# sanazkaviani/3d-latent-diffusion-model

Hardware: AMD Instinct MI355X
Metric: UNet denoising steps/sec (bf16, 1x4x24x24x24 latent; whole job = sum over GPUs) (higher is better)
Workload: dtype bf16

## Files before the change

3d-latent-diffusion-model_amd/_lib.py:

```python
from __future__ import annotations

import ctypes as C
import os
import threading

LDM_MAX_LEVELS = 8
_HERE = os.path.dirname(os.path.abspath(__file__))
LIB_PATH = os.environ.get("LDM3D_LIB") or os.path.join(_HERE, "libldm3d.so")


class UNetCfg(C.Structure):
    _fields_ = [("spatial_dims", C.c_int), ("in_channels", C.c_int), ("out_channels", C.c_int),
                ("num_levels", C.c_int),
                ("channels", C.c_int * LDM_MAX_LEVELS), ("attention_levels", C.c_int * LDM_MAX_LEVELS),
                ("num_head_channels", C.c_int * LDM_MAX_LEVELS), ("num_res_blocks", C.c_int * LDM_MAX_LEVELS),
                ("norm_num_groups", C.c_int), ("norm_eps", C.c_float)]


class VaeCfg(C.Structure):
    _fields_ = [("spatial_dims", C.c_int), ("in_channels", C.c_int), ("out_channels", C.c_int),
                ("latent_channels", C.c_int), ("num_levels", C.c_int),
                ("channels", C.c_int * LDM_MAX_LEVELS), ("num_res_blocks", C.c_int * LDM_MAX_LEVELS),
                ("attention_levels", C.c_int * LDM_MAX_LEVELS),
                ("norm_num_groups", C.c_int), ("norm_eps", C.c_float),
# ... 36 lines not shown
    "ldm_adam_step_ema": (C.c_int, [_P, _P, _P, _P, _P, C.c_int64, C.c_float, C.c_float, C.c_float, C.c_float, C.c_float, C.c_int,
                                    C.c_float, C.c_int, _P, C.c_float, _P]),
    "ldm_model_adam_step_ema": (C.c_int, [_P, _P, _P, _P, _P, _P, C.c_float, C.c_float, C.c_float, C.c_float, C.c_float, C.c_int,
                                          C.c_float, C.c_int, _P, C.c_float, _P]),
    "ldm_model_set_graph_mode": (C.c_int, [_P, C.c_int]),
    "ldm_model_set_precision": (C.c_int, [_P, C.c_int]),
    "ldm_model_get_precision": (C.c_int, [_P]),
    "ldm_model_tap_count": (C.c_int, [_P, C.c_char_p, C.c_int, C.c_int, C.c_int, C.c_int]),
    "ldm_model_tap_elems": (C.c_int64, [_P, C.c_char_p, C.c_int, C.c_int, C.c_int, C.c_int]),
    "ldm_model_tap_info": (C.c_int, [_P, C.c_char_p, C.c_int, C.c_int, C.c_int, C.c_int, C.c_int, C.c_char_p, C.c_int,
                                     C.POINTER(C.c_int), C.POINTER(C.c_int64)]),
    "ldm_model_taps_workspace_bytes": (C.c_size_t, [_P, C.c_char_p, C.c_int, C.c_int, C.c_int, C.c_int, C.c_int]),
    "ldm_unet_forward_taps": (C.c_int, [_P, _P, C.c_int, _P, C.c_int, _P, _P, C.c_int, C.c_int, C.c_int, C.c_int, _P, _P,
                                        _P, C.c_size_t, _P]),
    "ldm_vae_encode_taps": (C.c_int, [_P, _P, _P, _P, _P, _P, C.c_int, C.c_int, C.c_int, C.c_int, _P, _P, _P, C.c_size_t, _P]),
    "ldm_vae_decode_taps": (C.c_int, [_P, _P, _P, C.c_int, C.c_int, C.c_int, C.c_int, _P, _P, _P, C.c_size_t, _P]),
    "ldm_vae_encode_workspace_bytes": (C.c_size_t, [_P, C.c_int, C.c_int, C.c_int, C.c_int]),
    "ldm_vae_decode_workspace_bytes": (C.c_size_t, [_P, C.c_int, C.c_int, C.c_int, C.c_int]),
    "ldm_vae_encode": (C.c_int, [_P, _P, _P, _P, _P, _P, C.c_int, C.c_int, C.c_int, C.c_int, _P, C.c_size_t, _P]),
    "ldm_vae_decode": (C.c_int, [_P, _P, _P, C.c_int, C.c_int, C.c_int, C.c_int, _P, C.c_size_t, _P]),
    "ldm_add_noise": (C.c_int, [_P, _P, _P, _P, _P, C.c_int, C.c_int64, _P]),
    "ldm_scheduler_step": (C.c_int, [_P, _P, _P, _P, _P, C.c_int64, C.c_int, C.c_int, _F, C.c_int, _P]),
    "ldm_add_noise_target": (C.c_int, [_P, _P, _P, _P, _P, _P, C.c_int, C.c_int64, C.c_int, _P]),
    "ldm_scale": (C.c_int, [_P, _P, C.c_int64, C.c_float, _P]),
    "ldm_sampler_create": (C.c_int, [_P, C.c_int, C.c_int, C.c_int, C.c_int, C.c_uint64, C.POINTER(_P)]),
    "ldm_sampler_create_pndm": (C.c_int, [_P, C.c_int, C.c_int, C.POINTER(_P)]),
    "ldm_sampler_state_bytes": (C.c_size_t, [_P, C.c_int64]),
    "ldm_sampler_bind_state": (C.c_int, [_P, _P, C.c_size_t, C.c_int64]),
    "ldm_pndm_step": (C.c_int, [_P] * 9 + [C.c_int64, C.c_int, _F, _P]),
    "ldm_sampler_destroy": (None, [_P]),
    "ldm_sampler_reset": (C.c_int, [_P, _P, C.c_int, _P]),
    "ldm_sampler_step": (C.c_int, [_P, _P, _P, _P, C.c_int64, _P, C.c_int, _P]),
    "ldm_sampler_noise": (C.c_int, [_P, C.c_int, _P, C.c_int64, _P]),
    "ldm_unet_denoise_step": (C.c_int, [_P, _P, _P, C.c_int, _P, C.c_int, _P, _P, C.c_int, C.c_int, C.c_int, C.c_int,
                                        _P, C.c_size_t, _P]),
    "ldm_window_grid_create": (C.c_int, [_P, _P, _P, _P, _P, _P, C.POINTER(_P)]),
    "ldm_window_grid_destroy": (None, [_P]),
    "ldm_window_gather": (C.c_int, [_P, _P, _P, C.c_int, _P]),
    "ldm_window_blend": (C.c_int, [_P, _P, _P, C.c_int, _P]),
    "ldm_unet_denoise_step_windows": (C.c_int, [_P, _P, _P, _P, C.c_int, _P, C.c_int, _P, _P, _P, C.c_int, _P, C.c_size_t, _P]),
    "ldm_op_conv3d": (C.c_int, [_P, C.c_int, _P, C.c_int, _P, _P, _P, C.c_int, _P, C.c_int, _P, _P, _P, C.c_int, _P, _P, _P,
                                C.c_int, C.c_int, C.c_int, C.c_int, C.c_int, C.c_int, C.c_int, C.c_int, C.c_int, C.c_int,
                                C.c_int, C.c_int, _P, C.c_size_t, _P]),
    "ldm_op_weight_flip_transpose": (C.c_int, [_P, _P, C.c_int, C.c_int, C.c_int, C.c_int, _P]),
    "ldm_op_conv3d_wgrad": (C.c_int, [_P, C.c_int, _P, C.c_int, _P, C.c_int, C.c_int, C.c_int, C.c_int, C.c_int, C.c_int,
                                      C.c_int, C.c_int, C.c_int, C.c_int, C.c_int, _P]),
    "ldm_op_group_norm_bwd_scratch_bytes": (C.c_size_t, [C.c_int, C.c_int, C.c_int, C.c_int]),
    "ldm_op_group_norm_bwd": (C.c_int, [_P, _P, C.c_int, _P, C.c_int, _P, _P, C.c_int, C.c_float, C.c_int, _P, _P, _P, _P, _P, _P,
                                        C.c_int, C.c_int, _P, C.c_size_t, _P]),
    "ldm_op_scale_intensity_percentiles_scratch_bytes": (C.c_size_t, [C.c_int]),
    "ldm_op_scale_intensity_percentiles": (C.c_int, [_P, _P, C.c_int, C.c_int64, C.c_float, C.c_float, C.c_float, C.c_float, _P, C.c_size_t, _P]),
    "ldm_op_image_metrics_scratch_bytes": (C.c_size_t, [C.c_int] * 6),
    "ldm_op_image_metrics": (C.c_int, [_P, C.POINTER(C.c_int64), _P, C.POINTER(C.c_int64)] + [C.c_int] * 5 + [_F, C.c_int, C.c_float, C.c_float,
                                       C.c_float, _P, _P, _P, C.c_size_t, _P]),
    "ldm_op_im2col": (C.c_int, [_P, _P] + [C.c_int] * 10 + [_P]),
    "ldm_op_col2im": (C.c_int, [_P, _P] + [C.c_int] * 10 + [_P]),
    "ldm_op_leaky_relu": (C.c_int, [_P, _P, C.c_int64, C.c_float, _P]),
    "ldm_op_leaky_relu_bwd": (C.c_int, [_P, _P, _P, C.c_int64, C.c_float, _P]),
    "ldm_op_pack_ncdhw": (C.c_int, [_P, _P, C.c_int, C.c_int, C.c_int, C.c_int64, _P]),
    "ldm_op_unpack_ndhwc": (C.c_int, [_P, _P, C.c_int, C.c_int, C.c_int, C.c_int64, _P]),
    "ldm_op_conv3d_gn_scratch_bytes": (C.c_size_t, [C.c_int, C.c_int, C.c_int, C.c_int, C.c_int, C.c_int]),
    "ldm_op_conv3d_gn": (C.c_int, [_P, C.c_int, _P, _P, _P, _P, C.c_int, C.c_float, C.c_int, _P, _P, C.c_int, C.c_int, C.c_int, C.c_int,
                                   C.c_int, C.c_int, C.c_int, C.c_int, _P, C.c_size_t, _P]),
    "ldm_op_conv3d_fin_gn_scratch_bytes": (C.c_size_t, [C.c_int, C.c_int, C.c_int, C.c_int, C.c_int, C.c_int]),
    "ldm_op_conv3d_fin_gn": (C.c_int, [_P, C.c_int, _P, _P, _P, C.c_int, _P, _P, _P, C.c_int, C.c_float, C.c_int, _P, _P,
                                       C.c_int, C.c_int, C.c_int, C.c_int, C.c_int, C.c_int, C.c_int, C.c_int, _P, C.c_size_t, _P]),
    "ldm_op_group_norm_scratch_bytes": (C.c_size_t, [C.c_int, C.c_int, C.c_int]),
    "ldm_op_group_norm": (C.c_int, [_P, C.c_int, _P, C.c_int, _P, _P, C.c_int, C.c_float, C.c_int, _P, C.c_int, C.c_int,
                                    _P, C.c_size_t, _P]),
    "ldm_op_attention": (C.c_int, [_P, _P, C.c_int, C.c_int, C.c_int, _P]),
    "ldm_op_attention_hd": (C.c_int, [_P, _P, _P, C.c_int, C.c_int, C.c_int, C.c_int, _P]),
    "ldm_op_attention_bwd_hd": (C.c_int, [_P, _P, _P, _P, _P, _P, C.c_int, C.c_int, C.c_int, C.c_int, _P]),
    "ldm_op_attention_train": (C.c_int, [_P, _P, _P, C.c_int, C.c_int, C.c_int, _P]),
    "ldm_op_attention_bwd": (C.c_int, [_P, _P, _P, _P, _P, _P, C.c_int, C.c_int, C.c_int, _P]),
    "ldm_profile_start": (C.c_int, [C.c_int, C.c_int, C.c_int, C.c_int]),
    "ldm_profile_detail": (C.c_int, [C.POINTER(C.c_double), C.POINTER(C.c_double), C.c_int]),
    "ldm_profile_stop": (C.c_int, [C.POINTER(C.c_double)]),
# ... 109 lines not shown
```

3d-latent-diffusion-model_amd/csrc/conv_thin.h:

```cpp
#pragma once
#include "common.h"

struct ThinParams {
    const bf16_t* x; const bf16_t* w;
    const float* bias; float* out;
    int N, D, H, W, Cin, CoutPad, CoutReal;
    int td, th, tw;
    int x3_c;
};

constexpr int THIN_TD = 4, THIN_TH = 4, THIN_TW = 16;
constexpr int THIN_HD = THIN_TD + 2, THIN_HH = THIN_TH + 2, THIN_HW = THIN_TW + 2;
constexpr int THIN_HV = THIN_HD * THIN_HH * THIN_HW;
constexpr int THIN_CK = 32, THIN_RB = THIN_CK * 2, THIN_NC = THIN_RB / 16;
constexpr int THIN_LDS_X = THIN_HV * THIN_RB, THIN_LDS_W = 27 * 4 * THIN_RB;
constexpr int THIN_LDS = THIN_LDS_X + THIN_LDS_W;

__global__ __launch_bounds__(256) void conv3_thin_kernel(const ThinParams p) {
#if defined(__HIP_DEVICE_COMPILE__)
    extern __shared__ __attribute__((aligned(16))) char smem[];
    char* sx = smem; char* sw = smem + THIN_LDS_X;
    const int tid = threadIdx.x, lane = tid & 63, wave = tid >> 6, fr = lane & 15, fg = lane >> 4;
    int b = blockIdx.x;
    const int bw = b % p.tw; b /= p.tw; const int bh = b % p.th; b /= p.th; const int bd = b % p.td; const int n = b / p.td;
    const int d0 = bd * THIN_TD, h0 = bh * THIN_TH, w0 = bw * THIN_TW;
    const size_t xn = (size_t)n * p.D * p.H * p.W;
    const int xstride = p.x3_c ? 2 * p.x3_c : p.Cin;
    const int wm = fr < 4 ? 2 * fr : fr < 12 ? 2 * (fr - 4) + 1 : 2 * (fr - 8);
    f32x4 acc[4];
#pragma unroll
    for (int t = 0; t < 4; ++t) acc[t] = (f32x4){0.f, 0.f, 0.f, 0.f};
    const u32x4 zero = {0u, 0u, 0u, 0u};
    for (int c0 = 0; c0 < p.Cin; c0 += THIN_CK) {
        __syncthreads();
        const int xc0 = (p.x3_c && c0 >= p.x3_c) ? c0 - p.x3_c : c0;
        constexpr int NIT = (THIN_HV * THIN_NC + 255) / 256;
        u32x4 hv_v[NIT];
#pragma unroll
        for (int k = 0; k < NIT; ++k) {
            const int e = tid + k * 256;
            const int hv = e / THIN_NC, c16 = e % THIN_NC;
            const int wx = hv % THIN_HW, r = hv / THIN_HW, hy = r % THIN_HH, dz = r / THIN_HH;
            const int gd = d0 - 1 + dz, gh = h0 - 1 + hy, gw = w0 - 1 + wx;
            hv_v[k] = zero;
            if (e < THIN_HV * THIN_NC && (unsigned)gd < (unsigned)p.D && (unsigned)gh < (unsigned)p.H && (unsigned)gw < (unsigned)p.W)
                hv_v[k] = *reinterpret_cast<const u32x4*>(p.x + (xn + ((size_t)gd * p.H + gh) * p.W + gw) * xstride + xc0 + c16 * 8);
        }
#pragma unroll
        for (int k = 0; k < NIT; ++k) {
            const int e = tid + k * 256;
            const int hv = e / THIN_NC, c16 = e % THIN_NC;
            if (e < THIN_HV * THIN_NC) *reinterpret_cast<u32x4*>(sx + hv * THIN_RB + ((c16 ^ ((hv >> 2) & (THIN_NC - 1))) << 4)) = hv_v[k];
        }
        for (int e = tid; e < 27 * 4 * THIN_NC; e += 256) {
            const int c16 = e % THIN_NC, row = (e / THIN_NC) & 3, tap = e / (4 * THIN_NC);
            u32x4 v = zero;
            if (row < p.CoutReal) v = *reinterpret_cast<const u32x4*>(p.w + ((size_t)tap * p.CoutPad + row) * p.Cin + c0 + c16 * 8);
            *reinterpret_cast<u32x4*>(sw + (tap * 4 + row) * THIN_RB + ((c16 ^ row) << 4)) = v;
        }
        __syncthreads();
#pragma unroll 1
        for (int tap = 0; tap < 27; ++tap) {
            const int kd = tap / 9, kh = (tap / 3) % 3, kw = tap % 3;
            u32x4 wv = zero;
            if (fr < 4) wv = *reinterpret_cast<const u32x4*>(sw + (tap * 4 + fr) * THIN_RB + ((fg ^ fr) << 4));
            const bf16x8 wf = *reinterpret_cast<const bf16x8*>(&wv);
#pragma unroll
            for (int t = 0; t < 4; ++t) {
                const int hv = ((wave + kd) * THIN_HH + (t + kh)) * THIN_HW + wm + kw;
                const bf16x8 xf = *reinterpret_cast<const bf16x8*>(sx + hv * THIN_RB + ((fg ^ ((hv >> 2) & (THIN_NC - 1))) << 4));
                acc[t] = __builtin_amdgcn_mfma_f32_16x16x32_bf16(wf, xf, acc[t], 0, 0, 0);
            }
        }
    }
    if (fg != 0) return;
    const int gd = d0 + wave, gw = w0 + wm;
    if (gd >= p.D || gw >= p.W) return;
    const size_t dhw = (size_t)p.D * p.H * p.W;
#pragma unroll
    for (int t = 0; t < 4; ++t) {
        const int gh = h0 + t;
        if (gh >= p.H) continue;
        const size_t sp = ((size_t)gd * p.H + gh) * p.W + gw;
#pragma unroll
        for (int r = 0; r < 4; ++r)
            if (r < p.CoutReal) p.out[((size_t)n * p.CoutReal + r) * dhw + sp] = acc[t][r] + (p.bias ? p.bias[r] : 0.f);
    }
#endif
}
```

3d-latent-diffusion-model_amd/csrc/gemm_wg.h:

```cpp
#pragma once
#include "conv_cube.h"
#include "gemm_light.h"

struct WgGnParams {
    const float* slabs;
    const float* gamma; const float* beta;
    int nrb, groups, DHW; float eps;
};

__device__ __forceinline__ void wg_copies_landed_barrier() {
    asm volatile("s_waitcnt vmcnt(0)" ::: "memory");
    __builtin_amdgcn_s_barrier();
    asm volatile("" ::: "memory");
}

template <int MT, int NWV, bool GN>
__global__ __launch_bounds__(64 * NWV) void gemm_wg_kernel(const LightParams p, const int cout_pad, const WgGnParams g) {
#if defined(__HIP_DEVICE_COMPILE__)
    extern __shared__ __attribute__((aligned(16))) char smem[];
    typedef __attribute__((address_space(3))) void* lds_ptr_t;
    constexpr int NT = 2, R = 16 * MT, NW = 32 * NWV;
    const int tid = threadIdx.x, lane = tid & 63, fr = lane & 15, fg = lane >> 4;
    const int wave = __builtin_amdgcn_readfirstlane(tid >> 6);
    const int mtile = blockIdx.x % p.mtiles, ntile = blockIdx.x / p.mtiles;
    const int m0 = mtile * R, n0 = ntile * NW;
    const int nkb = p.K >> 7;
    const unsigned row2 = (unsigned)p.K * 2u;
    const int xbase = nkb * NW * 256;

    constexpr int T = 64 * NWV;
    const int C = p.K;
    int ns0 = 0, ns1 = 0;
    float4 t[16]; float gm[4], bt[4];
    float* const ab = reinterpret_cast<float*>(smem + nkb * (NW + R) * 256);
    double* const csum = reinterpret_cast<double*>(ab + 4 * C);
    float* const gstat = reinterpret_cast<float*>(csum + 2 * C);
    auto slab_loads = [&](const int smp, const int pp) {
        const float* base = g.slabs + ((size_t)smp * g.nrb * C + 2 * pp) * 2;
#pragma unroll
        for (int k = 0; k < 16; ++k) {
            int bb = k; const bool ok = bb < g.nrb; if (!ok) bb = g.nrb - 1;
            t[k] = *reinterpret_cast<const float4*>(base + (size_t)bb * C * 2);
            if (!ok) t[k] = make_float4(0.f, 0.f, 0.f, 0.f);
        }
    };
    if constexpr (GN) {
        ns0 = m0 / g.DHW;
        int ml = m0 + R - 1; if (ml > p.M - 1) ml = p.M - 1;
        ns1 = ml / g.DHW;
        if (tid < (C >> 1)) slab_loads(ns0, tid);
#pragma unroll
        for (int j = 0; j < 4; ++j) {
            const int c = tid + j * T;
            gm[j] = c < C ? g.gamma[c] : 0.f; bt[j] = c < C ? g.beta[c] : 0.f;
        }
    }

    {
        __amdgpu_buffer_rsrc_t rs_w = __builtin_amdgcn_make_buffer_rsrc((void*)p.w, 0, (int)((unsigned)cout_pad * row2), 0x00020000);
        for (int u = wave; u < nkb * (NW / 4); u += NWV) {
            const int kb = u / (NW / 4), lr = 4 * (u % (NW / 4)) + (lane >> 4), f = lr & 15;
            const int co = n0 + (lr & ~31) + 8 * (f >> 2) + 4 * ((lr >> 4) & 1) + (f & 3);
            const unsigned vo = (unsigned)co * row2 + (unsigned)kb * 256u + (unsigned)((lane & 15) ^ f) * 16u;
            __builtin_amdgcn_raw_ptr_buffer_load_lds(rs_w, (lds_ptr_t)(smem + u * 1024), 16, vo, 0, 0, 0);
        }
        __amdgpu_buffer_rsrc_t rs_x = __builtin_amdgcn_make_buffer_rsrc((void*)p.x, 0, (int)((unsigned)p.M * row2), 0x00020000);
        for (int u = wave; u < nkb * (R / 4); u += NWV) {
            const int kb = u / (R / 4), lr = 4 * (u % (R / 4)) + (lane >> 4);
            const unsigned vo = (unsigned)(m0 + lr) * row2 + (unsigned)kb * 256u + (unsigned)((lane & 15) ^ (lr & 15)) * 16u;
            __builtin_amdgcn_raw_ptr_buffer_load_lds(rs_x, (lds_ptr_t)(smem + xbase + u * 1024), 16, vo, 0, 0, 0);
        }
    }
    const int n0w = n0 + 32 * wave;
    const int wrow = (32 * wave + fr) * 256, xrow = xbase + fr * 256;
    f32x4 acc[NT][MT];
#pragma unroll
    for (int a = 0; a < NT; ++a)
#pragma unroll
        for (int b = 0; b < MT; ++b) acc[a][b] = (f32x4){0.f, 0.f, 0.f, 0.f};
    if constexpr (GN) {
        const int cpg = C / g.groups;
        for (int smp = ns0; smp <= ns1; ++smp) {
            for (int pp = tid; pp < (C >> 1); pp += T) {
                if (smp != ns0 || pp != tid) slab_loads(smp, pp);
                double s0 = 0.0, q0 = 0.0, s1 = 0.0, q1 = 0.0;
#pragma unroll
                for (int k = 0; k < 8; ++k) {
                    float4 a = make_float4(0.f, 0.f, 0.f, 0.f);
                    a.x += t[k].x; a.y += t[k].y; a.z += t[k].z; a.w += t[k].w;
                    a.x += t[k + 8].x; a.y += t[k + 8].y; a.z += t[k + 8].z; a.w += t[k + 8].w;
                    s0 += (double)a.x; q0 += (double)a.y; s1 += (double)a.z; q1 += (double)a.w;
                }
                csum[4 * pp] = s0; csum[4 * pp + 1] = q0; csum[4 * pp + 2] = s1; csum[4 * pp + 3] = q1;
            }
            cube_barrier();
            if (tid < g.groups) {
                double s = 0.0, q = 0.0;
                for (int k = 0; k < cpg; ++k) { s += csum[(tid * cpg + k) * 2]; q += csum[(tid * cpg + k) * 2 + 1]; }
                const double cnt = (double)cpg * (double)g.DHW;
                const double mean = s / cnt;
                double var = q / cnt - mean * mean; if (var < 0.0) var = 0.0;
                const float rstd = (float)(1.0 / sqrt(var + (double)g.eps));
                gstat[2 * tid] = (float)mean; gstat[2 * tid + 1] = rstd;
            }
// ... 47 lines not shown
        _Pragma("unroll") for (int mt = 0; mt < MT; ++mt) XF[mt] = *reinterpret_cast<const bf16x8*>(xp_ + mt * 4096); \
    } while (0)
#define GW_MFMA(WF, XF) do {                                                                          \
        _Pragma("unroll") for (int nt = 0; nt < NT; ++nt)                                             \
            _Pragma("unroll") for (int mt = 0; mt < MT; ++mt)                                         \
                acc[nt][mt] = __builtin_amdgcn_mfma_f32_16x16x32_bf16(WF[nt], XF[mt], acc[nt][mt], 0, 0, 0); \
    } while (0)
    GW_LOAD(wa, xa, 0);
    for (int s = 0; s < nsteps; s += 2) {
        GW_LOAD(wb, xb, s + 1);
        GW_MFMA(wa, xa);
        GW_LOAD(wa, xa, s + 2);
        GW_MFMA(wb, xb);
    }
#undef GW_LOAD
#undef GW_MFMA
    light_epilogue<MT, NT>(p, acc, mtile, m0, n0w, fr, fg);
#endif
}

static inline bool gemm_wg_ok(bool single_source, int K, long M) {
    return ldm_knob("LDM_GEMM_WG", 1) != 0 && single_source && K % 128 == 0 && K >= 128 && K <= 512 && M * (long)K * 2 < (1L << 31);
}
static inline int gemm_wg_gn_lds(int K, int groups) { return 32 * K + 8 * groups; }
static inline int gemm_wg_rows(int big) { return big ? 64 : 32; }
static inline int gemm_wg_couts(int big, int K) { return big && K <= 384 ? 128 : 64; }
static inline bool gemm_wg_gn_shape_ok(int K, long DHW, int groups, int nrb, int big) {
    return K >= 256 && groups >= 1 && groups <= 128 && K % groups == 0 && (K / groups) % 2 == 0 && K / groups <= 64 && nrb >= 1 && nrb <= 16 &&
           DHW >= gemm_wg_rows(big) && (gemm_wg_rows(big) + gemm_wg_couts(big, K)) * 2 * K + gemm_wg_gn_lds(K, groups) <= 160 * 1024;
}
static inline bool gemm_wg_gn_ok(int K, long DHW, int groups, int nrb, int big) {
    return ldm_knob("LDM_GEMM_WG_GN", 0) != 0 && gemm_wg_gn_shape_ok(K, DHW, groups, nrb, big);
}
template <int MT, int NWV, bool GN>
static inline hipError_t launch_gemm_wg_t(const LightParams& p, int cout_pad, const WgGnParams& g, hipStream_t s) {
    constexpr int kmax = (16 * MT + 32 * NWV) * 2 * 512 <= 160 * 1024 ? 512 : 384;
    const int lds = (16 * MT + 32 * NWV) * 2 * p.K + (GN ? gemm_wg_gn_lds(p.K, g.groups) : 0);
    if (p.K > kmax || lds > 160 * 1024) return hipErrorInvalidValue;
    static bool attr_tab[32] = {}; bool& attr_set = attr_flag(attr_tab);
    if (!attr_set) {
        hipError_t e = hipFuncSetAttribute(reinterpret_cast<const void*>(&gemm_wg_kernel<MT, NWV, GN>), hipFuncAttributeMaxDynamicSharedMemorySize,
                                           GN ? 160 * 1024 : (16 * MT + 32 * NWV) * 2 * kmax);
        if (e != hipSuccess) return e;
        attr_set = true;
    }
    hipLaunchKernelGGL((gemm_wg_kernel<MT, NWV, GN>), dim3(p.mtiles * ((cout_pad + 32 * NWV - 1) / (32 * NWV))), dim3(64 * NWV), lds, s, p, cout_pad, g);
    return hipGetLastError();
}
static inline hipError_t launch_gemm_wg(const LightParams& p0, int cout_pad, int big, hipStream_t s, const WgGnParams* gn = nullptr) {
    LightParams p = p0;
    const WgGnParams g = gn ? *gn : WgGnParams{};
    if (big) {
        p.mtiles = (p.M + 63) / 64;
        if (p.K <= 384) return gn ? launch_gemm_wg_t<4, 4, true>(p, cout_pad, g, s) : launch_gemm_wg_t<4, 4, false>(p, cout_pad, g, s);
        return gn ? launch_gemm_wg_t<4, 2, true>(p, cout_pad, g, s) : launch_gemm_wg_t<4, 2, false>(p, cout_pad, g, s);
    }
    p.mtiles = (p.M + 31) / 32;
    return gn ? launch_gemm_wg_t<2, 2, true>(p, cout_pad, g, s) : launch_gemm_wg_t<2, 2, false>(p, cout_pad, g, s);
}
static inline hipError_t launch_gemm_1x1(const LightParams& p, int cout_pad, int big, int wg, hipStream_t s) {
    return wg ? launch_gemm_wg(p, cout_pad, big, s) : launch_gemm_light(p, cout_pad, big, s);
}
```

3d-latent-diffusion-model_amd/csrc/ldm3d.hip:

```cpp
#include <hip/hip_runtime.h>
#include <dlfcn.h>
#include <math.h>
#include <stdarg.h>
#include <stdio.h>
#include <stdlib.h>
#include <string.h>

#include <algorithm>
#include <atomic>
#include <map>
#include <memory>
#include <string>
#include <type_traits>
#include <vector>

#include "../../include/ldm3d.h"
#include "attention.h"
#include "conv_igemm.h"
#include "conv_halo.h"
#include "conv_cube.h"
#include "conv_plane.h"
#ifdef LDM_EXPERIMENTS
#include "conv_halo_pp.h"
#include "conv_halo_rw.h"
// ... 99 lines not shown
struct Ref { int base = BASE_NULL; size_t off = 0; };
static inline Ref ws_ref(size_t off) { Ref r; r.base = BASE_WS; r.off = off; return r; }
static inline Ref w_ref(size_t off) { Ref r; r.base = BASE_W; r.off = off; return r; }
static inline Ref io_ref(int i) { Ref r; r.base = BASE_IO0 + i; r.off = 0; return r; }
static inline Ref w32_ref(size_t off) { Ref r; r.base = BASE_W32; r.off = 2 * off; return r; }

struct Act {
    size_t off = 0; int C = 0; int N = 0, D = 0, H = 0, W = 0; bool valid = false;
    size_t stats_off = 0; bool has_stats = false;
    int stats_nrb = 0;
    int esz = 2;
    bool hl = false;
    size_t cs_off = 0; int cs_rows = 0;
    size_t bytes() const { return (size_t)N * D * H * W * C * esz; }
    long rows() const { return (long)N * D * H * W; }
};

enum OpKind { OP_PACK, OP_CONV, OP_FINALIZE, OP_GN_STATS, OP_GN_FINALIZE, OP_GN_PREP, OP_GN_APPLY, OP_ATTN, OP_SINUSOID,
              OP_GEMV, OP_VAE_HEADS, OP_GN_FUSED,
              OP_WT , OP_WT_BATCH, OP_WGRAD, OP_EXPORT , OP_EXPORT_BATCH, OP_COLSUM, OP_GNB, OP_ATTN_BWD, OP_ADD, OP_SUMPOOL, OP_LIN_DX, OP_LIN_DW, OP_VAE_HEADS_BWD,
              OP_GEMM_LIGHT,
              OP_COLSUM_BATCH,
              OP_IM2COL,
              OP_PACK32, OP_CONV32, OP_FIN32, OP_GN_STATS32, OP_GN_APPLY32, OP_ATTN32, OP_GEMV32,
              OP_TAP,
              OP_BUCKET, OP_BUCKET_JOIN,
              OP_UPS_SPLIT32,
              OP_CONV_THIN,
              OP_FIN_GN,
              OP_GEMM_LIGHT32,
              OP_CONV_BLOCK,
              OP_TEMB_ROW };

struct ConvCfg { int wgm, wgn, bk, splitk; int halo = 0, mtps = 0, qps = 0; int slab_lg = 0; int cube = 0; int th = 0, big = 0; int plane = 0; int wg = 0; };

struct ConvRec {
    Ref xa, xb, w; int ca, cb;
    Ref x1a, x1b, w1; int c1a, c1b;
    int N, Din, Hin, Win, Dout, Hout, Wout;
    int k, stride, pad, M;
    int couts, cout_pad, cout_real;
    int nchunk0, nchunk1, mtiles, ntiles;
    bool ups, exact;
    bool phase;
    bool x3;
    bool ep32_ndhwc, ep32_ncdhw;
    Ref bias, bias2, temb, residual; int temb_stride;
    Ref out; int f32_out;
    Ref partial, stats;
    int stats_nrb, stats_rows;
    Ref gamma, beta, gn_out; int gn_groups, gn_silu, gn_lg; float gn_eps;
    Ref gn_stats; int gn_nrb;
};

struct GnRec {
    Ref xa, xb; int ca, cb, N, DHW;
    Ref gamma, beta; int groups; float eps; bool silu;
    Ref stats_a, stats_b; int nrb_a, nrb_b;
    Ref partial; int nslab, rows_per_slab;
    Ref ab, mr;
    Ref out; bool out_hl;
    int rows_per_block, chunks;
    Ref dy, gsum, dgamma_n, dbeta_n;
    Ref cs; bool leaves_colsums;
    Ref acc_a, acc_b, dxa, dxb;
    int dgamma_flat, dbeta_flat;
    bool fp32;
// ... 12 lines not shown
struct LayoutRec {
    Ref a, b, dst;
    int N, c_real, c_stored, D, H, W, DHW;
    bool internal;
    int esz, mode, ups;
};

struct AttnRec {
    Ref qkv, out, lse;
    Ref d_o, delta, dqkv;
    int B, N, C, heads, d; float scale;
    bool x3, fp32;
};

struct LinRec {
    Ref w, bias, x, y;
    Ref dy, x_pre, dx, dW, db, part;
    int B, I, O, x_stride, y_stride, dy_stride;
    int silu, nz; bool fp32;
};

struct ElemRec {
    Ref a, b, out; int n;
    Ref ml, noise, mu, sigma, z;
    Ref dz, g_mu, g_sigma, dy; int c_dz;
    int N, D, H, W, C, L, DHW;
    bool fp32;
};

struct RangeRec { int first, end, count; bool fp32; };

struct Op {
    OpKind kind;
    ConvCfg cc;
    ConvRec cv;
    GnRec gn;
    WgradRec wg;
    LayoutRec lay;
    AttnRec at;
    LinRec lin;
    ElemRec el;
    RangeRec rg;
};

struct Pool {
    struct Blk { size_t off, size; };
    std::vector<Blk> free_list;
    std::map<size_t, size_t> live;
    size_t top = 0, high = 0;
    size_t alloc(size_t bytes) {
        bytes = rup_sz(bytes, 256);
        for (size_t k = 0; k < free_list.size(); ++k)
            if (free_list[k].size >= bytes) {
                size_t off = free_list[k].off;
                if (free_list[k].size == bytes) free_list.erase(free_list.begin() + k);
                else { free_list[k].off += bytes; free_list[k].size -= bytes; }
                live[off] = bytes;
                return off;
            }
        size_t off = top; top += bytes; high = std::max(high, top); live[off] = bytes;
        return off;
    }
    void release(size_t off) {
        auto it = live.find(off); if (it == live.end()) return;
        Blk b{off, it->second}; live.erase(it);
        free_list.push_back(b);
// ... 6 lines not shown
            top = free_list.back().off; free_list.pop_back();
        }
    }
};

struct DevTable {
    void* descs = nullptr; int2* map = nullptr; int nblocks = 0;
    std::vector<char> h_descs, h_map;
    ~DevTable() { if (descs) (void)hipFree(descs); if (map) (void)hipFree(map); }
    template <class D> int upload(const std::vector<D>& d, const std::vector<int2>& m) {
        if (d.empty()) return 0;
        h_descs.assign((const char*)d.data(), (const char*)(d.data() + d.size()));
        h_map.assign((const char*)m.data(), (const char*)(m.data() + m.size()));
        nblocks = (int)m.size();
        return 0;
    }
    int ready() {
        if (descs || h_descs.empty()) return 0;
        if (hipMalloc(&descs, h_descs.size()) != hipSuccess || hipMalloc((void**)&map, h_map.size()) != hipSuccess) return -1;
        if (hipMemcpy(descs, h_descs.data(), h_descs.size(), hipMemcpyHostToDevice) != hipSuccess) return -1;
        if (hipMemcpy(map, h_map.data(), h_map.size(), hipMemcpyHostToDevice) != hipSuccess) return -1;
        return 0;
    }
};

struct TapInfo { std::string name; int dims[5]; size_t off; };

struct Plan {
    std::vector<Op> ops;
    std::vector<TapInfo> taps; size_t tap_elems = 0;
    size_t ws_bytes = 0;
    size_t bwd_begin = 0;
    bool train = false;
    mutable DevTable wt_tab, exp_tab, cs_tab;
};

enum PackKind { PK_CONV_W, PK_VEC_F32, PK_LINEAR_W };
struct ParamDesc {
    std::string name; std::vector<int64_t> shape;
    PackKind kind; size_t dst_off;
    int k = 1, cout = 0, cin = 0, cout_pad = 0, cin_s = 0, row_off = 0;
    int64_t flat_off = 0;
    bool loaded = false;
};

struct ConvW { size_t w_off = 0; size_t b_off = 0; int cout = 0, cout_pad = 0, cin_s = 0, k = 1; bool has = false;
               size_t wp_off = 0;
               size_t x3_off = (size_t)-1;
               size_t x3p_off = (size_t)-1; };
struct GnW { size_t g_off = 0, b_off = 0; int C = 0; };
struct LinW { size_t w_off = 0, b_off = 0; int in = 0, out = 0; };

struct ldm_comm;
struct GradSyncState {
    ldm_comm* comm = nullptr; hipStream_t stream = nullptr;
    std::vector<hipEvent_t> ev;
    size_t used = 0; std::vector<int64_t> elems;
    int wire = 0;
    void* stage = nullptr; size_t stage_bytes = 0;
    int pending = 0;
};
static int grad_sync_begin(GradSyncState& g, hipStream_t s);
static int grad_sync_bucket(GradSyncState& g, float* buf, int64_t count, hipStream_t s);
static int grad_sync_join(GradSyncState& g, hipStream_t s);
struct ldm_model {
    int type = 0;
// ... 141 lines not shown
    int tap_mode = 0;
    void tap(const std::string& name, Act& h, int c_real) {
        if (!tap_mode) return;
        TapInfo t; t.name = name; t.dims[0] = h.N; t.dims[1] = c_real; t.dims[2] = h.D; t.dims[3] = h.H; t.dims[4] = h.W; t.off = plan->tap_elems;
        plan->tap_elems += (size_t)h.N * c_real * h.D * h.H * h.W;
        Op o{}; o.kind = OP_TAP; LayoutRec& l = o.lay; l.a = ws_ref(h.off);
        l.dst.base = BASE_TAPO; l.dst.off = t.off * 4; l.b.base = BASE_TAPI; l.b.off = t.off * 4;
        l.N = h.N; l.c_real = c_real; l.c_stored = h.C; l.DHW = h.D * h.H * h.W; l.esz = h.esz; l.mode = tap_mode;
        plan->ops.push_back(o);
        plan->taps.push_back(t);
        if (tap_mode == 2 && h.has_stats) { pool.release(h.stats_off); h.has_stats = false; }
    }
    void pack(Ref src_a, Ref src_b, const Act& dst, int c_real, bool internal) {
        Op o{}; o.kind = hp ? OP_PACK32 : OP_PACK; LayoutRec& l = o.lay; l.a = src_a; l.b = src_b; l.dst = ws_ref(dst.off);
        l.N = dst.N; l.c_real = c_real; l.c_stored = dst.C; l.DHW = dst.D * dst.H * dst.W; l.internal = internal;
        plan->ops.push_back(o);
    }
    void free_act(Act& a) {
        if (train) return;
        if (a.valid) { pool.release(a.off); if (a.has_stats) pool.release(a.stats_off); }
        a.valid = false; a.has_stats = false;
    }
    bool train = false, recording = false;

    struct ConvArgs {
        Act xa, xb;
        const ConvW* w = nullptr;
        int k = 3, stride = 1, pad = 1, ups = 0;
        int Do = 0, Ho = 0, Wo = 0;
        Act g1a, g1b; const ConvW* w1 = nullptr;
        Ref temb; int temb_stride = 0;
        Act residual;
        bool f32_out = false; Ref out_ref; int cout_real = 0;
        bool want_stats = true;
        Ref w_over; bool no_bias = false; int exact = 0;
        int temb_row = -1;
        int f32_tag = 0;
        const GnW* pre_gn = nullptr; int pre_groups = 0, pre_nrb = 0; float pre_eps = 0.f;
    };
    struct Tape {
        int kind = 0;
        ConvArgs c; Act out; bool leaf_input = false;
        const GnW* g = nullptr; Act xa, xb; size_t ab_off = 0, mr_off = 0; int groups = 0; bool silu = false;
        Act qkv, o; size_t lse_off = 0; int head_ch = 64;
    };
    std::vector<Tape> tape;

    static bool halo_enabled() { return ldm_knob("LDM_CONV_HALO", 1) != 0; }
    static int tall_mode() { return ldm_xknob("LDM_HALO_TALL", 2); }
    static bool light_enabled() { return ldm_knob("LDM_GEMM_LIGHT", 1) != 0; }
    static bool two_wg_enabled() { return ldm_knob("LDM_IGEMM_2WG", 1) != 0; }
    static bool phase_enabled() { return ldm_knob("LDM_CONV_PHASE", 1) != 0; }
    static bool halo_skip_enabled() { static const int v = ldm_knob("LDM_HALO_SKIP", 1); return v != 0; }
    static bool halo_skip_split_enabled() { static const int v = ldm_knob("LDM_HALO_SKIP_SPLIT", 1); return v != 0; }
    static bool cube_enabled() { return ldm_knob("LDM_CONV_CUBE", 1) != 0; }
    static bool cube_ok(int D, int H, int W, int cin0, int c1a, int c1b, int cout_pad) {
        return cube_enabled() && D >= 1 && H >= 1 && W >= 1 && D <= CUBE_EDGE && H <= CUBE_EDGE && W <= CUBE_EDGE && cin0 % 64 == 0 && cin0 >= 128 &&
               c1a % 64 == 0 && c1b % 64 == 0 && cout_pad % 16 == 0;
    }
    static ConvCfg cube_cfg(int cin0) { ConvCfg c{2, 2, 64, cin0 / 64}; c.cube = 1; return c; }
    static bool plane_enabled() { return ldm_knob("LDM_CONV_PLANE", 1) != 0; }
    static int plane_max_cin() { return (int)ldm_knob("LDM_CONV_PLANE_MAX_CIN", 256); }
    static bool plane_ok(int D, int H, int W, int cin0, int c1a, int c1b, int cout_pad) {
        return plane_enabled() && D >= 1 && H >= 1 && W >= 1 && D <= PLANE_EDGE && H <= PLANE_EDGE && W <= PLANE_EDGE &&
               (D > CUBE_EDGE || H > CUBE_EDGE || W > CUBE_EDGE) && cin0 % 64 == 0 && cin0 >= 128 && cin0 <= plane_max_cin() &&
               c1a % 64 == 0 && c1b % 64 == 0 && cout_pad % 16 == 0;
// ... 47 lines not shown
            for (int sk : splits) {
                if (sk > 1 && Q / sk < 3) break;
                const int qps = (Q + sk - 1) / sk, skr = (Q + qps - 1) / qps;
                const long nwg = tiles * skr;
                const double rounds = ceil((double)nwg / 256.0);
                double t = rounds * (3.0 * qps * c_step + 2500.0 + ((steps1 + skr - 1) / skr) * 1.6 * c_step + (steps1 && skr > 1 ? 800.0 : 0.0));
                if (skr > 1) t += 6000.0 + (double)M * cout_pad * 4.0 * skr * 2.0 / 2500.0;
                if (steps1 && skr > 1 && !halo_skip_split_enabled()) continue;
                if (tall_mode() == 2 && cout_pad % 128 == 0) t = 1e31;
                if (tall_mode() == 3 && skr == 1 && best.halo == 1 && best.splitk == 1) t = 0.0;
                if (t < best_t) { best_t = t; best = ConvCfg{4, 1, 64, skr}; best.halo = 2; best.mtps = mtps; best.qps = qps; }
            }
        }
        return best;
    }

    static ConvRec conv_rec(const ConvArgs& a, int k, int stride, int pad, long M, int cout_real) {
        ConvRec c{}; c.N = a.xa.N; c.Din = a.xa.D; c.Hin = a.xa.H; c.Win = a.xa.W; c.Dout = a.Do; c.Hout = a.Ho; c.Wout = a.Wo;
        c.k = k; c.stride = stride; c.pad = pad; c.M = (int)M; c.couts = rup(a.w->cout, 32); c.cout_pad = a.w->cout_pad; c.cout_real = cout_real;
        return c;
    }
    static void conv_epilogue(ConvRec& c, const ConvArgs& a, const Act& out) {
        c.bias = a.no_bias ? Ref() : w_ref(a.w->b_off); c.temb = a.temb; c.temb_stride = a.temb_stride;
        c.residual = a.residual.valid ? ws_ref(a.residual.off) : Ref();
        c.out = a.f32_out ? a.out_ref : ws_ref(out.off); c.f32_out = a.f32_out ? 1 : 0;
    }
    static void conv_sources(ConvRec& c, const ConvArgs& a) {
        c.xa = ws_ref(a.xa.off); c.xb = a.xb.valid ? ws_ref(a.xb.off) : Ref(); c.ca = a.xa.C; c.cb = a.xb.valid ? a.xb.C : 0;
    }
    void record_conv(const ConvArgs& a, const Act& out) { if (recording) { Tape t; t.kind = 0; t.c = a; t.out = out; tape.push_back(t); } }
    static long thin_tiles(const ConvArgs& a) {
        return (long)a.xa.N * ((a.Do + THIN_TD - 1) / THIN_TD) * ((a.Ho + THIN_TH - 1) / THIN_TH) * ((a.Wo + THIN_TW - 1) / THIN_TW);
    }
    void emit_thin(const ConvArgs& a, long M, Ref w, int cout_real, bool x3) {
        Op op{}; op.kind = OP_CONV_THIN;
        ConvRec& c = op.cv; c = conv_rec(a, 3, 1, 1, M, cout_real); conv_epilogue(c, a, Act());
        c.xa = ws_ref(a.xa.off); c.ca = x3 ? 2 * a.xa.C : a.xa.C; c.x3 = x3; c.w = w;
        plan->ops.push_back(op);
    }
    Act emit_light(OpKind kind, const ConvArgs& a, long M, Ref w, int big, bool want_stats) {
        const int N = a.xa.N, rows = big ? 64 : 32;
        Op op{}; op.kind = kind; op.cc.big = big;
        ConvRec& c = op.cv; c = conv_rec(a, a.k, a.stride, a.pad, M, a.w->cout);
        op.cc.wg = kind == OP_GEMM_LIGHT && gemm_wg_ok(!a.xb.valid, a.xa.C + (a.xb.valid ? a.xb.C : 0), M);
        if (a.pre_gn) {
            op.cc.wg = 2; c.gamma = w_ref(a.pre_gn->g_off); c.beta = w_ref(a.pre_gn->b_off); c.gn_groups = a.pre_groups; c.gn_eps = a.pre_eps;
            c.gn_stats = ws_ref(a.xa.stats_off); c.gn_nrb = a.pre_nrb;
        }
        Act out = new_act(N, a.Do, a.Ho, a.Wo, c.couts);
        const long dhwo = (long)a.Do * a.Ho * a.Wo;
        if (want_stats && (N == 1 || dhwo % rows == 0)) {
            out.stats_off = pool.alloc((size_t)((M + rows - 1) / rows) * c.couts * 2 * 4); out.has_stats = true;
            out.stats_nrb = (int)(N == 1 ? (M + rows - 1) / rows : dhwo / rows);
        }
        conv_epilogue(c, a, out); conv_sources(c, a); c.w = w; c.stats = out.has_stats ? ws_ref(out.stats_off) : Ref();
        plan->ops.push_back(op);
        record_conv(a, out);
        return out;
    }
    Act emit_conv_block(const ConvArgs& a, long M, int th, int tiles) {
        const int N = a.xa.N;
        Op op{}; op.kind = OP_CONV_BLOCK; op.cc.th = th;
        ConvRec& c = op.cv; c = conv_rec(a, 3, 1, 1, M, a.w->cout);
        Act out = new_act(N, a.Do, a.Ho, a.Wo, c.couts);
        if (a.want_stats) { out.stats_off = pool.alloc((size_t)N * tiles * c.couts * 2 * 4); out.has_stats = true; out.stats_nrb = tiles; }
        conv_epilogue(c, a, out); conv_sources(c, a);
        c.w = a.w_over.base != BASE_NULL ? a.w_over : w_ref(a.w->w_off); c.stats = out.has_stats ? ws_ref(out.stats_off) : Ref();
        plan->ops.push_back(op);
        record_conv(a, out);
        return out;
// ... 136 lines not shown
        if (sk > 1) { partial_bytes = std::max(partial_bytes, (size_t)sk * M * w.cout_pad * 4); partial_fixups.push_back(plan->ops.size()); }
        plan->ops.push_back(op);
        if (sk > 1) { Op f = op; f.kind = OP_FIN32; fin32_stats(f, out, a, N, a.Do * a.Ho * a.Wo, couts); partial_fixups.push_back(plan->ops.size()); plan->ops.push_back(f); }
        record_conv(a, out);
        return out;
    }

    Act conv(const ConvArgs& a, std::string tag = "") {
        if (hp) return conv32(a, tag);
        const ConvW& w = *a.w;
        const int cin0 = a.xa.C + (a.xb.valid ? a.xb.C : 0);
        int bk = 64;
        if (a.xa.C % 64 || (a.xb.valid && a.xb.C % 64)) bk = 32;
        int cin1 = 0;
        if (a.w1) {
            cin1 = a.g1a.C + (a.g1b.valid ? a.g1b.C : 0);
            if (a.g1a.C % 64 || (a.g1b.valid && a.g1b.C % 64)) bk = 32;
        }
        if (cin0 != w.cin_s || (a.w1 && cin1 != a.w1->cin_s) || cin0 % 32 || cin1 % 32) {
            err = "conv " + tag + ": channel bookkeeping mismatch"; return Act();
        }
        const int N = a.xa.N;
        const long M = (long)N * a.Do * a.Ho * a.Wo;
        {
            const long rows0 = (long)N * a.xa.D * a.xa.H * a.xa.W;
            const long big = std::max(std::max(rows0 * a.xa.C, a.xb.valid ? rows0 * a.xb.C : 0L),
                                      a.w1 ? std::max(M * a.g1a.C, a.g1b.valid ? M * a.g1b.C : 0L) : 0L) * 2;
            if (big >= (1L << 32)) { err = "conv " + tag + ": a source tensor exceeds 4 GiB (split the batch)"; return Act(); }
        }
        {
            static const int thin = ldm_knob("LDM_CONV_THIN", 1);
            static const long thin_min = ldm_knob("LDM_CONV_THIN_MIN", 512L);
            const int cr = a.cout_real ? a.cout_real : w.cout;
            if (thin && a.f32_out && a.k == 3 && a.stride == 1 && a.pad == 1 && !a.ups && !a.exact && !a.xb.valid && !a.w1 &&
                a.temb.base == BASE_NULL && !a.residual.valid && a.w_over.base == BASE_NULL && cr <= 4 && cin0 % 32 == 0 && cin0 <= 128 &&
                a.xa.D == a.Do && a.xa.H == a.Ho && a.xa.W == a.Wo &&
                thin_tiles(a) >= thin_min) {
                emit_thin(a, M, w_ref(w.w_off), cr, false);
                record_conv(a, Act());
                return Act();
            }
        }
        const bool phase = a.ups == 1 && !a.exact && a.k == 3 && a.stride == 1 && a.pad == 1 && !train && !a.xb.valid && !a.w1 &&
                           a.w_over.base == BASE_NULL && w.wp_off != 0 && phase_enabled() &&
                           a.Do == 2 * a.xa.D && a.Ho == 2 * a.xa.H && a.Wo == 2 * a.xa.W;
        if (gemm_light_ok(a.k, a.stride, a.ups, cin0, !a.w1, !a.f32_out && a.temb.base == BASE_NULL) && light_enabled() &&
            a.xa.D == a.Do && a.xa.H == a.Ho && a.xa.W == a.Wo && M * (long)cin0 * 2 < (1L << 31))
            return emit_light(OP_GEMM_LIGHT, a, M, a.w_over.base != BASE_NULL ? a.w_over : w_ref(w.w_off), gemm_light_big(M, w.cout_pad), a.want_stats);
        if (a.pre_gn) { err = "conv " + tag + ": a GroupNorm prologue needs the light GEMM"; return Act(); }
        if (conv_block_enabled() && a.k == 3 && a.stride == 1 && a.pad == 1 && a.ups == 0 && !a.exact && !a.xb.valid && !a.w1 && !a.f32_out &&
            w.cout_pad == 64 && rup(w.cout, 32) == 64 && cin0 <= conv_block_max_cin() &&
            a.xa.D == a.Do && a.xa.H == a.Ho && a.xa.W == a.Wo) {
            const int TH = conv_block_th();
            const int td = (a.Do + BLK_TD - 1) / BLK_TD, th = (a.Ho + TH - 1) / TH, tw = (a.Wo + BLK_TW - 1) / BLK_TW;
            static const long min_blocks = ldm_knob("LDM_CONV_BLOCK_MIN", 512L);
            if ((long)N * td * th * tw >= min_blocks) return emit_conv_block(a, M, TH, td * th * tw);
        }
        if (conv_block128_enabled() && a.k == 3 && a.stride == 1 && a.pad == 1 && a.ups == 0 && !a.exact && !a.xb.valid && !a.w1 && !a.f32_out &&
            w.cout_pad == 128 && rup(w.cout, 32) == 128 && cin0 <= conv_block128_max_cin() && a.xa.D == a.Do && a.xa.H == a.Ho && a.xa.W == a.Wo) {
            const int td = (a.Do + BLK_TD - 1) / BLK_TD, th = (a.Ho + 7) / 8, tw = (a.Wo + BLK_TW - 1) / BLK_TW;
            static const long min_blocks = ldm_knob("LDM_CONV_BLOCK128_MIN", 192L);
            static const long max_blocks = ldm_xknob("LDM_CONV_BLOCK128_MAX", 0L);
            const long tiles128 = (long)N * td * th * tw;
            if (tiles128 >= min_blocks && tiles128 <= (max_blocks > 0 ? max_blocks : (long)device_cus())) return emit_conv_block(a, M, 8, td * th * tw);
        }
        const int taps = phase ? 8 : a.k * a.k * a.k;
        const bool halo_ok = a.k == 3 && a.stride == 1 && a.pad == 1 && a.ups == 0 && !a.exact && !a.xb.valid && (!a.w1 || (halo_skip_enabled() && bk == 64)) &&
                             a.xa.D == a.Do && a.xa.H == a.Ho && a.xa.W == a.Wo;
        int nchunk0 = cin0 / bk, nchunk1 = cin1 / bk;
        int steps0 = taps * nchunk0, steps1 = nchunk1;
// ... 133 lines not shown
            return out;
        }
        if (fused) push_ab(OP_GN_PREP, rec);
        else {
            const int rows_par = std::max(1, 256 / (C / 8));
            static const bool gn32_fold = (ldm_knob("LDM_GN32_FOLD", 1) != 0);
            const bool fold32 = hp && !train && gn32_fold && C / groups <= 64;
            int nslab = std::min((DHW + rows_par - 1) / rows_par, std::max(1, (fold32 ? 256 : 512) / N));
            int rps = (DHW + nslab - 1) / nslab;
            nslab = (DHW + rps - 1) / rps;
            gnpart_bytes = std::max(gnpart_bytes, (size_t)N * nslab * C * 2 * 4);
            rec.nslab = nslab; rec.rows_per_slab = rps;
            gnpart_fixups.push_back(plan->ops.size()); push(hp ? OP_GN_STATS32 : OP_GN_STATS, rec);
            gnpart_fixups.push_back(plan->ops.size());
            if (fold32) { Act out = fold_apply32(); push(OP_GN_APPLY32, rec); return out; }
            push_ab(OP_GN_FINALIZE, rec);
        }
        Act out = new_act(N, xa.D, xa.H, xa.W, C);
        GnRec ap = gn_rec(xa, xb); ap.silu = silu; ap.ab = rec.ab; ap.out = ws_ref(out.off);
        push_ab(hp ? OP_GN_APPLY32 : OP_GN_APPLY, ap);
        record(out);
        return out;
    }

    static bool im2col_enabled() { return ldm_knob("LDM_CONV_IM2COL", 1) != 0; }
    Act conv_in_im2col(const std::string& name, Ref r0, Ref r1, int N, int D, int H, int W, int cin, bool internal) {
        auto it = m->convs.find(name + ".im2col");
        if (train || hp || it == m->convs.end() || !im2col_enabled() || !light_enabled()) return Act();
        const ConvW& wi = it->second;
        Act pm = new_act(N, D, H, W, wi.cin_s);
        Op o{}; o.kind = OP_IM2COL; LayoutRec& l = o.lay; l.a = r0; l.b = r1; l.dst = ws_ref(pm.off);
        l.N = N; l.c_real = cin; l.c_stored = wi.cin_s; l.D = D; l.H = H; l.W = W; l.internal = internal;
        plan->ops.push_back(o);
        ConvArgs a; a.xa = pm; a.w = &wi; a.k = 1; a.pad = 0; a.Do = D; a.Ho = H; a.Wo = W;
        Act out = conv(a, name + ".im2col");
        free_act(pm);
        return out;
    }

    Act conv3(const std::string& name, const Act& x, int stride = 1, int pad = 1, int ups = 0) {
        ConvArgs a; a.xa = x; a.w = &m->convs.at(name); a.k = 3; a.stride = stride; a.pad = pad; a.ups = ups;
        const int Du = x.D << ups, Hu = x.H << ups, Wu = x.W << ups;
        if (stride == 1) { a.Do = Du; a.Ho = Hu; a.Wo = Wu; }
        else if (pad == 1) { a.Do = (Du + 2 - 3) / 2 + 1; a.Ho = (Hu + 2 - 3) / 2 + 1; a.Wo = (Wu + 2 - 3) / 2 + 1; }
        else { a.Do = (Du + 1 - 3) / 2 + 1; a.Ho = (Hu + 1 - 3) / 2 + 1; a.Wo = (Wu + 1 - 3) / 2 + 1; }
        return conv(a, name);
    }

    Act resblock(const std::string& p, const Act& xa, const Act& xb, int cout, int groups, float eps,
                 const std::string& skip_name, bool with_temb, const GnW* next_gn = nullptr) {
        const int cin = xa.C + (xb.valid ? xb.C : 0);
        Act sk;
        if (cin != cout && hp) {
            ConvArgs cs; cs.xa = xa; cs.xb = xb; cs.w = &m->convs.at(p + skip_name); cs.k = 1; cs.pad = 0;
            cs.Do = xa.D; cs.Ho = xa.H; cs.Wo = xa.W; cs.want_stats = false;
            sk = conv(cs, p + skip_name);
            if (!sk.valid) return Act();
        }
        Act h0 = gn_apply(m->gns.at(p + ".norm1"), xa, xb, groups, eps, true, &m->convs.at(p + ".conv1"));
        if (!h0.valid) return Act();
        ConvArgs c1; c1.xa = h0; c1.w = &m->convs.at(p + ".conv1"); c1.Do = xa.D; c1.Ho = xa.H; c1.Wo = xa.W;
        if (with_temb) {
            c1.temb = ws_ref(temb_all_off + (size_t)m->tproj_row.at(p) * 4); c1.temb_stride = tproj_stride;
            c1.temb_row = m->tproj_row.at(p);
        }
        Act h1 = conv(c1, p + ".conv1");
        free_act(h0);
        if (!h1.valid) return Act();
        Act h2;
// ... 389 lines not shown
        const int lvl = L - 1 - i;
        int prev = oc; oc = ch[lvl];
        const int ic = ch[std::max(lvl - 1, 0)];
        const int nres = c.num_res_blocks[lvl] + 1;
        for (int j = 0; j < nres; ++j) {
            const int skip_c = (j == nres - 1) ? ic : oc;
            const int rin = (j == 0) ? prev : oc;
            char p[96]; snprintf(p, sizeof p, "up_blocks.%d.resnets.%d", i, j);
            reg_res(p, rin + skip_c, oc);
            if (c.attention_levels[lvl] && !collect) { snprintf(p, sizeof p, "up_blocks.%d.attentions.%d", i, j); m->reg_attn(p, oc); }
        }
        if (i != L - 1 && !collect) { char p[96]; snprintf(p, sizeof p, "up_blocks.%d.upsampler.postconv", i); m->reg_conv(p, oc, oc, oc, 3, true); }
    }
    if (!collect) { m->reg_gn("out.0", ch[0]); m->reg_conv("out.2", ch[0], ch[0], c.out_channels, 3); }
    };
    walk();
    m->reg_linear("time_embed.0", ch[0], temb);
    m->reg_linear("time_embed.2", temb, temb);
    int rows = 0; for (auto& t : tprojs) rows += t.second;
    m->tproj_rows = rows;
    m->tproj_w_off = m->arena_alloc((size_t)rows * temb * 2);
    m->tproj_b_off = m->arena_alloc((size_t)rows * 4);
    int r = 0;
    for (auto& t : tprojs) {
        m->tproj_row[t.first] = r;
        m->reg_linear_at(t.first + ".time_emb_proj", temb, t.second, m->tproj_w_off + (size_t)r * temb * 2, m->tproj_b_off + (size_t)r * 4);
        r += t.second;
    }
    collect = false;
    walk();
    return 0;
}

static int unet_build(ldm_model* m, int B, int D, int H, int W, Plan* plan, bool train, bool hp = false, int tap_mode = 0, bool temb_table = false) {
    const ldm_unet_cfg& c = m->ucfg;
    const int L = c.num_levels; const int* ch = c.channels;
    const int temb = ch[0] * 4, G = c.norm_num_groups; const float eps = c.norm_eps;
    if (train && tap_mode) return fail(LDM_ERR_UNSUPPORTED, "debug taps are inference-only");
    Builder b; b.m = m; b.plan = plan; b.train = train; b.recording = train; b.hp = hp; b.tap_mode = tap_mode;
    const size_t sin_off = b.pool.alloc((size_t)B * ch[0] * 4);
    const size_t e1_off = b.pool.alloc((size_t)B * temb * 4);
    const size_t e2_off = b.pool.alloc((size_t)B * temb * 4);
    b.tproj_stride = m->tproj_rows;
    b.temb_all_off = b.pool.alloc(((size_t)B * m->tproj_rows + 256) * 4);
    const LinW& l0 = m->lins.at("time_embed.0"); const LinW& l2 = m->lins.at("time_embed.2");
    if (temb_table && !train) {
        Op o{}; o.kind = OP_TEMB_ROW; o.lin.y = ws_ref(b.temb_all_off); o.lin.O = m->tproj_rows; o.lin.B = B; plan->ops.push_back(o);
    } else {
    { Op o{}; o.kind = OP_SINUSOID; o.lin.x = io_ref(2); o.lin.y = ws_ref(sin_off); o.lin.B = B; o.lin.O = ch[0];
      plan->ops.push_back(o); }
    auto gemv = [&](size_t w_off, size_t b_off, size_t x_off, size_t y_off, int I, int O, int xs, int ys, int silu) {
        Op o{}; o.kind = hp ? OP_GEMV32 : OP_GEMV; LinRec& l = o.lin;
        l.w = hp ? w32_ref(w_off) : w_ref(w_off); l.bias = w_ref(b_off); l.x = ws_ref(x_off); l.y = ws_ref(y_off);
        l.I = I; l.O = O; l.x_stride = xs; l.y_stride = ys; l.silu = silu; l.B = B; plan->ops.push_back(o);
    };
    gemv(l0.w_off, l0.b_off, sin_off, e1_off, ch[0], temb, ch[0], temb, 0);
    gemv(l2.w_off, l2.b_off, e1_off, e2_off, temb, temb, temb, temb, 1);
    gemv(m->tproj_w_off, m->tproj_b_off, e2_off, b.temb_all_off, temb, m->tproj_rows, temb, m->tproj_rows, 1);
    }

    const int cin_s = rup(c.in_channels, 32);
    Act h = b.conv_in_im2col("conv_in", io_ref(0), io_ref(1), B, D, H, W, c.in_channels, false);
    if (!h.valid) {
        if (!b.err.empty()) return fail(LDM_ERR_UNSUPPORTED, "%s", b.err.c_str());
        Act xin = b.new_act(B, D, H, W, cin_s);
        b.pack(io_ref(0), io_ref(1), xin, c.in_channels, false);
        h = b.conv3("conv_in", xin);
// ... 47 lines not shown
    for (int i = 0; i < L; ++i) {
        const int lvl = L - 1 - i;
        for (int j = 0; j < c.num_res_blocks[lvl] + 1; ++j) {
            Act s = skips.back(); skips.pop_back();
            snprintf(p, sizeof p, "up_blocks.%d.resnets.%d", i, j);
            char pa[96]; snprintf(pa, sizeof pa, "up_blocks.%d.attentions.%d.norm", i, j);
            Act hn = b.resblock(p, h, s, ch[lvl], G, eps, ".skip_connection", true, c.attention_levels[lvl] ? &m->gns.at(pa) : nullptr);
            b.free_act(h); b.free_act(s);
            if (!hn.valid) return fail(LDM_ERR_UNSUPPORTED, "%s", b.err.c_str());
            b.tap(p, hn, ch[lvl]);
            if (c.attention_levels[lvl]) {
                snprintf(p, sizeof p, "up_blocks.%d.attentions.%d", i, j);
                Act ha = b.attention(p, hn, c.num_head_channels[lvl], G, eps);
                b.free_act(hn);
                if (!ha.valid) return fail(LDM_ERR_UNSUPPORTED, "%s", b.err.c_str());
                hn = ha;
                b.tap(p, hn, ch[lvl]);
            }
            h = hn;
        }
        if (i != L - 1) {
            snprintf(p, sizeof p, "up_blocks.%d.upsampler.postconv", i);
            Act hu = b.conv3(p, h, 1, 1, 1);
            b.free_act(h);
            if (!hu.valid) return fail(LDM_ERR_UNSUPPORTED, "%s", b.err.c_str());
            b.tap(p, hu, ch[lvl]);
            h = hu;
        }
    }
    Act hn = b.gn_apply(m->gns.at("out.0"), h, Act(), G, eps, true, &m->convs.at("out.2"));
    b.free_act(h);
    if (!hn.valid) return fail(LDM_ERR_UNSUPPORTED, "%s", b.err.c_str());
    Builder::ConvArgs oa; oa.xa = hn; oa.w = &m->convs.at("out.2"); oa.Do = D; oa.Ho = H; oa.Wo = W;
    oa.f32_out = true; oa.out_ref = io_ref(3); oa.cout_real = c.out_channels;
    b.conv(oa, "out.2");
    if (!b.err.empty()) return fail(LDM_ERR_UNSUPPORTED, "%s", b.err.c_str());
    if (train) {
        plan->train = true; plan->bwd_begin = plan->ops.size();
        b.recording = false;
        const int rows = m->tproj_rows;
        b.dtemb_off = b.pool.alloc(((size_t)B * rows + 256) * 4);
        { Op o{}; o.kind = OP_WT_BATCH; o.rg.fp32 = hp; plan->ops.push_back(o); }
        const int cos_ = rup(c.out_channels, 32);
        Act dout = b.new_act(B, D, H, W, cos_);
        b.pack(io_ref(0), Ref(), dout, c.out_channels, false);
        b.bucket_hi = b.done_from = m->flat_total;
        b.tail_reserved = m->params[m->pindex.at("conv_in.conv.weight")].flat_off;
        if (!b.backward_all(dout)) return fail(LDM_ERR_UNSUPPORTED, "%s", b.err.c_str());
        b.flush_colsums();
        const Ref dtemb = ws_ref(b.dtemb_off);
        b.dw_off = b.pool.alloc((size_t)rows * temb * 4); b.vec_off = b.pool.alloc((size_t)rows * 4);
        b.emit_lin_dw(dtemb, ws_ref(e2_off), ws_ref(b.dw_off), ws_ref(b.vec_off), B, temb, rows, rows, temb, 1);
        for (const ParamDesc& d : m->params) {
            if (d.kind == PK_LINEAR_W && d.dst_off >= m->tproj_w_off && d.dst_off < m->tproj_w_off + (size_t)rows * temb * 2)
                b.emit_export(b.dw_off, 1, rows, temb, (int)((d.dst_off - m->tproj_w_off) / ((size_t)temb * 2)), 0, d.cout, d.cin, d.flat_off);
            if (d.kind == PK_VEC_F32 && d.dst_off >= m->tproj_b_off && d.dst_off < m->tproj_b_off + (size_t)rows * 4)
                b.emit_export(b.vec_off, 1, 1, 0, 0, (int)((d.dst_off - m->tproj_b_off) / 4), 1, d.cout, d.flat_off);
        }
        const size_t de2 = b.pool.alloc((size_t)B * temb * 4), de1 = b.pool.alloc((size_t)B * temb * 4);
        b.emit_lin_dx(hp ? w32_ref(m->tproj_w_off) : w_ref(m->tproj_w_off), dtemb, ws_ref(e2_off), ws_ref(de2), B, temb, rows, rows, temb, 1);
        auto P = [&](const char* n) { return m->params[m->pindex.at(n)].flat_off; };
        b.emit_lin_dw(ws_ref(de2), ws_ref(e1_off), Builder::grad_ref(P("time_embed.2.weight")), Builder::grad_ref(P("time_embed.2.bias")),
                      B, temb, temb, temb, temb, 1);
        b.emit_lin_dx(hp ? w32_ref(l2.w_off) : w_ref(l2.w_off), ws_ref(de2), ws_ref(e1_off), ws_ref(de1), B, temb, temb, temb, temb, 1);
        b.emit_lin_dw(ws_ref(de1), ws_ref(sin_off), Builder::grad_ref(P("time_embed.0.weight")), Builder::grad_ref(P("time_embed.0.bias")),
                      B, ch[0], temb, temb, ch[0], 0);
        if (!b.err.empty()) return fail(LDM_ERR_UNSUPPORTED, "%s", b.err.c_str());
// ... 611 lines not shown
    p.CoutS = c.couts; p.CoutPad = c.cout_pad; p.CoutReal = c.cout_real; p.nchunk = c.nchunk0; p.steps = c.k * c.k * c.k * c.nchunk0;
    p.splitk = o.cc.splitk; p.steps_per_split = (p.steps + p.splitk - 1) / p.splitk; p.mtiles = c.mtiles; p.ntiles = c.ntiles;
    p.bias = (const float*)rp(bs, c.bias); p.temb = (const float*)rp(bs, c.temb); p.temb_stride = c.temb_stride; p.residual = (const float*)rp(bs, c.residual);
    if (c.f32_out) p.out_ncdhw = (float*)rp(bs, c.out); else p.out = (float*)rp(bs, c.out);
    p.partial = (float*)rp(bs, c.partial);
    if (c.stats_nrb > 0) { p.stats = (float*)rp(bs, c.stats); p.stats_nrb = c.stats_nrb; p.stats_rows = c.stats_rows; }
    return p;
}
static FinalizeParams finalize_params(const ConvParams& p) {
    FinalizeParams f{}; f.partial = p.partial; f.splitk = p.splitk; f.M = p.M; f.CoutPad = p.CoutPad; f.CoutS = p.CoutS; f.CoutReal = p.CoutReal;
    f.DHWo = p.Dout * p.Hout * p.Wout; f.bias = p.bias; f.bias2 = p.bias2; f.temb = p.temb; f.temb_stride = p.temb_stride; f.residual = p.residual;
    f.out = p.out; f.out_f32 = p.out_f32; f.stats = p.stats;
    return f;
}
template <class P> static P wgrad_params(const WgradRec& w, const Bases& bs) {
    P p{}; p.dy = (decltype(p.dy))rp(bs, w.dy); p.cdy = w.cdy; p.x = (decltype(p.x))rp(bs, w.x); p.cx = w.cx;
    p.dw = (float*)rp(bs, w.dw); p.Cout = w.Cout; p.Cin = w.Cin; p.dw_ld = w.dw_ld; p.dw_ci_off = w.dw_ci_off;
    p.N = w.N; p.Din = w.Din; p.Hin = w.Hin; p.Win = w.Win; p.Dout = w.Dout; p.Hout = w.Hout; p.Wout = w.Wout;
    p.ksize = w.ksize; p.stride = w.stride; p.pad = w.pad; p.ups = w.ups; p.M = w.M;
    p.co_tiles = (p.Cout + 127) / 128; p.ci_tiles = (p.Cin + 127) / 128; p.ksplit = w.ksplit;
    p.slab_stride = (long)w.ksize * w.ksize * w.ksize * w.rows_total * w.dw_ld;
    return p;
}
template <class P> static P attn_params(const AttnRec& a, const Bases& bs) {
    P p{}; p.qkv = (decltype(p.qkv))rp(bs, a.qkv); p.out = (decltype(p.out))rp(bs, a.out); p.lse = (float*)rp(bs, a.lse);
    p.B = a.B; p.N = a.N; p.C = a.C; p.heads = a.heads; p.d = a.d; p.scale = a.scale;
    return p;
}
template <class P> static P attn_bwd_params(const AttnRec& a, const Bases& bs) {
    P p{}; p.qkv = (decltype(p.qkv))rp(bs, a.qkv); p.o = (decltype(p.o))rp(bs, a.out); p.d_o = (decltype(p.d_o))rp(bs, a.d_o);
    p.lse = (const float*)rp(bs, a.lse); p.delta = (float*)rp(bs, a.delta); p.dqkv = (decltype(p.dqkv))rp(bs, a.dqkv);
    p.B = a.B; p.N = a.N; p.C = a.C; p.d = a.d; p.heads = a.heads; p.scale = a.scale;
    return p;
}

struct PlanTrace { bool on = false; std::string path; PlanTrace() { const char* e = getenv("LDM_PLAN_TRACE"); if (e && *e) { on = true; path = e; } } };
static PlanTrace g_plan_trace;
struct LaneCtx { GradSyncState* sync = nullptr; };

static int run_plan(const Plan& plan, const Bases& bs, const int* rt, hipStream_t s, size_t begin = 0, size_t end = (size_t)-1,
                    LaneCtx lanes = LaneCtx()) {
    if (end > plan.ops.size()) end = plan.ops.size();
    const char* trace_path = g_plan_trace.on ? g_plan_trace.path.c_str() : nullptr;
    std::vector<hipEvent_t> tev;
    if (trace_path) { tev.resize(end - begin + 1); for (auto& e : tev) HIP_TRY(hipEventCreate(&e)); }
    struct TraceDone {
        const Plan& plan; size_t begin, end; std::vector<hipEvent_t>& ev; hipStream_t s; const char* path;
        ~TraceDone() {
            if (ev.empty()) return;
            (void)hipEventRecord(ev.back(), s); (void)hipEventSynchronize(ev.back());
            FILE* f = fopen(path, "a");
            for (size_t oi = begin; oi < end && f; ++oi) {
                const Op& o = plan.ops[oi]; float ms = 0.f; (void)hipEventElapsedTime(&ms, ev[oi - begin], ev[oi - begin + 1]);
                fprintf(f, "%zu,%zu,%d,%.3f", plan.ops.size(), oi, (int)o.kind, ms * 1e3f);
                const ConvRec& c = o.cv;
                if (o.kind == OP_CONV || o.kind == OP_FINALIZE)
                    fprintf(f, ",M=%d k=%d s=%d ups=%d cin=%d+%d(x%d) cin1=%d couts=%d cfg=%dx%dx%d splitk=%d halo=%d mtps=%d qps=%d cube=%d", c.M, c.k, c.stride,
                            c.ups | c.exact << 1 | c.phase << 2 | c.x3 << 3 | c.ep32_ndhwc << 4 | c.ep32_ncdhw << 5, c.ca, c.cb, c.nchunk0, c.c1a + c.c1b, c.couts,
                            o.cc.wgm, o.cc.wgn, o.cc.bk, o.cc.splitk, o.cc.plane ? 6 : o.cc.halo, o.cc.mtps, o.cc.qps, o.cc.cube);
                else {
                    const GnRec& g = o.gn; const WgradRec& w = o.wg; const LayoutRec& l = o.lay; const AttnRec& at = o.at;
                    const LinRec& li = o.lin; const ElemRec& el = o.el; const RangeRec& r = o.rg;
                    int v[6] = {};
                    auto six = [&](int a, int b, int c2, int d, int e, int h) { v[0] = a; v[1] = b; v[2] = c2; v[3] = d; v[4] = e; v[5] = h; };
                    switch (o.kind) {
                        case OP_FIN_GN: six(c.gn_groups, c.gn_silu, c.gn_lg, c.c1b, c.N, c.Din); break;
// ... 10 lines not shown
                        case OP_COLSUM: six(g.N, g.nslab, g.ca, g.over_n, g.count, g.out_stride); break;
                        case OP_GNB: six(g.ca, g.cb, g.groups, g.DHW, g.N, g.silu); break;
                        case OP_WGRAD: six(w.cdy, w.cx, w.Cout, w.Cin, w.dw_ld, w.dw_ci_off); break;
                        case OP_PACK: case OP_PACK32: six(l.N, l.c_real, l.c_stored, l.DHW, l.internal, 0); break;
                        case OP_IM2COL: six(l.N, l.c_real, l.c_stored, l.D, l.H, l.W); break;
                        case OP_UPS_SPLIT32: six(l.N, l.c_stored, l.D, l.H, l.W, l.ups); break;
                        case OP_TAP: six(l.N, l.c_real, l.c_stored, l.DHW, l.esz, l.mode); break;
                        case OP_ATTN: case OP_ATTN32: six(at.B, at.N, at.C, at.heads, at.d, at.x3); break;
                        case OP_ATTN_BWD: six(at.B, at.N, at.C, at.d, at.fp32, 0); break;
                        case OP_SINUSOID: six(li.B, li.O, 0, 0, 0, 0); break;
                        case OP_TEMB_ROW: six(li.O, li.B, 0, 0, 0, 0); break;
                        case OP_GEMV: case OP_GEMV32: six(li.I, li.O, li.x_stride, li.y_stride, li.silu, li.B); break;
                        case OP_LIN_DX: case OP_LIN_DW: six(li.B, li.I, li.O, li.dy_stride, li.x_stride, li.silu); break;
                        case OP_VAE_HEADS: six(el.N, el.L, el.DHW, 0, 0, 0); break;
                        case OP_VAE_HEADS_BWD: six(el.N, el.L, el.C, el.DHW, el.c_dz, el.fp32); break;
                        case OP_ADD: six(el.n, el.fp32, 0, 0, 0, 0); break;
                        case OP_SUMPOOL: six(el.N, el.D, el.H, el.W, el.C, el.fp32); break;
                        case OP_WT_BATCH: six(r.fp32, 0, 0, 0, 0, 0); break;
                        case OP_COLSUM_BATCH: case OP_EXPORT_BATCH: six(r.first, r.end, 0, 0, 0, 0); break;
                        case OP_BUCKET: six(r.first, r.count, 0, 0, 0, 0); break;
                        case OP_BUCKET_JOIN: case OP_WT: case OP_EXPORT: case OP_CONV: case OP_FINALIZE: break;
                    }
                    fprintf(f, ",i=%d %d %d %d %d %d", v[0], v[1], v[2], v[3], v[4], v[5]);
                }
                fprintf(f, "\n");
            }
            if (f) fclose(f);
            for (auto e : ev) (void)hipEventDestroy(e);
        }
    } trace_done{plan, begin, end, tev, s, trace_path};
    for (size_t oi = begin; oi < end; ++oi) {
        const Op& o = plan.ops[oi];
        if (trace_path) HIP_TRY(hipEventRecord(tev[oi - begin], s));
        switch (o.kind) {
            case OP_PACK: case OP_PACK32: case OP_IM2COL: {
                const LayoutRec& l = o.lay;
                int cx = rt[0], cc = rt[1];
                if (l.internal) { cx = l.c_real; cc = 0; }
                if (cx + cc != l.c_real) return fail(LDM_ERR_BAD_ARG, "x_channels + cond_channels = %d, model expects %d", cx + cc, l.c_real);
                const float* xa = (const float*)rp(bs, l.a); const float* xb = (const float*)rp(bs, l.b);
                const long total = (long)l.N * l.DHW * l.c_stored;
                if (o.kind == OP_PACK)
                    hipLaunchKernelGGL(pack2_ncdhw_kernel, dim3(grid_for(total)), dim3(256), 0, s, xa, cx, xb, cc, (bf16_t*)rp(bs, l.dst), l.N, l.c_stored, l.DHW);
                else if (o.kind == OP_PACK32)
                    hipLaunchKernelGGL(pack2_ncdhw_f32_kernel, dim3(grid_for(total)), dim3(256), 0, s, xa, cx, xb, cc, (float*)rp(bs, l.dst), l.N, l.c_stored, l.DHW);
                else
                    hipLaunchKernelGGL(pack_im2col_kernel, dim3(grid_for((long)l.N * l.D * l.H * l.W * (l.c_stored / 8), 256, 16384)), dim3(256), 0, s, xa, cx,
                                       xb, cc, (bf16_t*)rp(bs, l.dst), l.N, l.D, l.H, l.W, l.c_stored);
                break; }
            case OP_CONV_THIN: {
                const ConvRec& c = o.cv;
                ThinParams q{}; q.x = (const bf16_t*)rp(bs, c.xa); q.w = (const bf16_t*)rp(bs, c.w); q.bias = (const float*)rp(bs, c.bias);
                q.out = (float*)rp(bs, c.out); q.N = c.N; q.D = c.Din; q.H = c.Hin; q.W = c.Win; q.CoutPad = c.cout_pad; q.CoutReal = c.cout_real;
                if (c.x3) { q.x3_c = c.ca / 2; q.Cin = 3 * q.x3_c; } else q.Cin = c.ca;
                if (!q.w) return fail(LDM_ERR_NOT_LOADED, "the weight arena is empty");
                q.td = (q.D + THIN_TD - 1) / THIN_TD; q.th = (q.H + THIN_TH - 1) / THIN_TH; q.tw = (q.W + THIN_TW - 1) / THIN_TW;
                static bool attr_tab[32] = {}; bool& attr_set = attr_flag(attr_tab);
                if (!attr_set) { HIP_TRY(hipFuncSetAttribute(reinterpret_cast<const void*>(&conv3_thin_kernel), hipFuncAttributeMaxDynamicSharedMemorySize, THIN_LDS)); attr_set = true; }
                hipLaunchKernelGGL(conv3_thin_kernel, dim3((unsigned)((long)q.N * q.td * q.th * q.tw)), dim3(256), THIN_LDS, s, q);
                break; }
            case OP_CONV_BLOCK: {
                const ConvRec& c = o.cv;
                BlockParams q{}; q.x = (const bf16_t*)rp(bs, c.xa); q.w = (const bf16_t*)rp(bs, c.w); q.bias = (const float*)rp(bs, c.bias);
                q.temb = (const float*)rp(bs, c.temb); q.temb_stride = c.temb_stride; q.residual = (const bf16_t*)rp(bs, c.residual); q.out = (bf16_t*)rp(bs, c.out);
                q.stats = (float*)rp(bs, c.stats); q.N = c.N; q.D = c.Dout; q.H = c.Hout; q.W = c.Wout; q.Cin = c.ca;
                if (!q.w) return fail(LDM_ERR_NOT_LOADED, "the weight arena is empty");
                if (c.couts == 128) HIP_TRY(launch_conv_block128(q, s)); else HIP_TRY(launch_conv_block(q, o.cc.th, s));
                break; }
            case OP_UPS_SPLIT32: {
                const LayoutRec& l = o.lay;
                hipLaunchKernelGGL(upsample_split_f32_kernel, dim3(grid_for(((long)l.N * l.D * l.H * l.W << (3 * l.ups)) * (l.c_stored / 4), 256, 4096)), dim3(256), 0, s,
                                   (const float*)rp(bs, l.a), (bf16_t*)rp(bs, l.dst), l.N, l.c_stored, l.D, l.H, l.W, l.ups);
                break; }
            case OP_CONV32: case OP_FIN32: {
                const Conv32Params p = conv32_params(o, bs);
                if (!p.w) return fail(LDM_ERR_NOT_LOADED, "fp32 precision: the fp32 weight arena is empty (re-upload the parameters after ldm_model_set_precision)");
                if (o.kind == OP_CONV32) launch_conv32(p, o.cc.bk == 32, o.cc.wgn * 64, s);
                else launch_fin32(p, s);
                break; }
            case OP_GEMM_LIGHT32: {
                const ConvRec& c = o.cv;
                LightX3Params p{};
                p.x = (const float*)rp(bs, c.xa); p.xb = (const float*)rp(bs, c.xb); p.ca = c.ca;
                p.w = (const float*)rp(bs, c.w);
                if (!p.w) return fail(LDM_ERR_NOT_LOADED, "fp32 precision: the fp32 weight arena is empty (re-upload the parameters after ldm_model_set_precision)");
                p.bias = (const float*)rp(bs, c.bias); p.residual = (const float*)rp(bs, c.residual);
                p.out = (float*)rp(bs, c.out); p.stats = (float*)rp(bs, c.stats);
                p.M = c.M; p.K = c.ca + c.cb; p.CoutS = c.couts;
                HIP_TRY(launch_gemm_light_x3(p, c.cout_pad, o.cc.big, s));
                break; }
            case OP_GN_STATS32: {
                const GnRec& g = o.gn;
// ... 32 lines not shown
                                        (float*)rp(bs, l.y), l.I, l.O, l.x_stride, l.y_stride, l.silu);
                break; }
            case OP_TAP: {
                const LayoutRec& l = o.lay;
                float* dst = (float*)rp(bs, l.dst); const float* src = (const float*)rp(bs, l.b);
                const long total = (long)l.N * l.c_real * l.DHW;
                if (dst) {
                    if (l.esz == 4) hipLaunchKernelGGL(tap_export_kernel<float>, dim3(grid_for(total)), dim3(256), 0, s, (const float*)rp(bs, l.a), dst, l.N, l.c_real, l.c_stored, l.DHW);
                    else hipLaunchKernelGGL(tap_export_kernel<bf16_t>, dim3(grid_for(total)), dim3(256), 0, s, (const bf16_t*)rp(bs, l.a), dst, l.N, l.c_real, l.c_stored, l.DHW);
                }
                if (src && l.mode == 2) {
                    const long tot2 = (long)l.N * l.DHW * l.c_stored;
                    if (l.esz == 4) hipLaunchKernelGGL(pack2_ncdhw_f32_kernel, dim3(grid_for(tot2)), dim3(256), 0, s, src, l.c_real, (const float*)nullptr, 0, (float*)rp(bs, l.a), l.N, l.c_stored, l.DHW);
                    else hipLaunchKernelGGL(pack2_ncdhw_kernel, dim3(grid_for(tot2)), dim3(256), 0, s, src, l.c_real, (const float*)nullptr, 0, (bf16_t*)rp(bs, l.a), l.N, l.c_stored, l.DHW);
                }
                break; }
            case OP_FIN_GN: {
                const ConvRec& c = o.cv;
                FinGnParams q{}; q.f = finalize_params(conv_params(o, bs));
                q.gamma = (const float*)rp(bs, c.gamma); q.beta = (const float*)rp(bs, c.beta); q.y = (bf16_t*)rp(bs, c.gn_out);
                q.groups = c.gn_groups; q.silu = c.gn_silu; q.lg = c.gn_lg; q.eps = c.gn_eps;
                HIP_TRY(launch_fin_gn(q, c.N, wt_stores(), s));
                break; }
            case OP_CONV: case OP_FINALIZE: {
                const ConvParams p = conv_params(o, bs);
                if (o.kind == OP_CONV) { LDM_TRY(launch_conv(p, o.cc, s)); }
                else launch_finalize(finalize_params(p), wt_stores(), s);
                break; }
            case OP_GEMM_LIGHT: {
                const ConvRec& c = o.cv;
                LightParams p{}; p.x = (const bf16_t*)rp(bs, c.xa); p.w = (const bf16_t*)rp(bs, c.w); p.bias = (const float*)rp(bs, c.bias);
                p.residual = (const bf16_t*)rp(bs, c.residual); p.out = (bf16_t*)rp(bs, c.out); p.stats = (float*)rp(bs, c.stats);
                p.M = c.M; p.K = c.ca + c.cb; p.CoutS = c.couts; p.xb = (const bf16_t*)rp(bs, c.xb); p.ca = c.ca;
                if (o.cc.wg == 2) {
                    WgGnParams g{}; g.slabs = (const float*)rp(bs, c.gn_stats); g.gamma = (const float*)rp(bs, c.gamma); g.beta = (const float*)rp(bs, c.beta);
                    g.nrb = c.gn_nrb; g.groups = c.gn_groups; g.DHW = c.Dout * c.Hout * c.Wout; g.eps = c.gn_eps;
                    HIP_TRY(launch_gemm_wg(p, c.cout_pad, o.cc.big, s, &g));
                } else
                    HIP_TRY(launch_gemm_1x1(p, c.cout_pad, o.cc.big, o.cc.wg, s));
                break; }
            case OP_GN_STATS: {
                const GnRec& g = o.gn;
                GnStatsParams p{}; p.xa = (const bf16_t*)rp(bs, g.xa); p.xb = (const bf16_t*)rp(bs, g.xb); p.ca = g.ca; p.cb = g.cb;
                p.DHW = g.DHW; p.nslab = g.nslab; p.rows_per_slab = g.rows_per_slab; p.partial = (float*)rp(bs, g.partial);
                hipLaunchKernelGGL(gn_stats_kernel, dim3(g.nslab, g.N), dim3(256), 0, s, p);
                break; }
            case OP_GN_FINALIZE: {
                const GnRec& g = o.gn;
                GnFinalizeParams p{}; p.partial = (const float*)rp(bs, g.partial); p.nslab = g.nslab; p.C = p.Creal = g.ca + g.cb; p.groups = g.groups;
                p.DHW = g.DHW; p.eps = g.eps; p.gamma = (const float*)rp(bs, g.gamma); p.beta = (const float*)rp(bs, g.beta);
                p.ab = (float*)rp(bs, g.ab); p.mr = (float*)rp(bs, g.mr);
                hipLaunchKernelGGL(gn_finalize_kernel, dim3(g.groups, g.N), dim3(256), 0, s, p);
                break; }
            case OP_GN_PREP: {
                const GnRec& g = o.gn;
                GnPrepParams p{}; p.sa = (const float*)rp(bs, g.stats_a); p.sb = (const float*)rp(bs, g.stats_b); p.ca = g.ca; p.cb = g.cb;
                p.nrb_a = g.nrb_a; p.nrb_b = g.nrb_b; p.groups = g.groups; p.DHW = g.DHW; p.eps = g.eps;
                p.gamma = (const float*)rp(bs, g.gamma); p.beta = (const float*)rp(bs, g.beta); p.ab = (float*)rp(bs, g.ab); p.mr = (float*)rp(bs, g.mr);
                hipLaunchKernelGGL(gn_prep_kernel, dim3(g.groups, g.N), dim3(256), 0, s, p);
                break; }
            case OP_GN_FUSED: {
                const GnRec& g = o.gn;
                GnFusedParams p{}; p.xa = (const bf16_t*)rp(bs, g.xa); p.xb = (const bf16_t*)rp(bs, g.xb); p.ca = g.ca; p.cb = g.cb;
                p.sa = (const float*)rp(bs, g.stats_a); p.sb = (const float*)rp(bs, g.stats_b); p.nrb_a = g.nrb_a; p.nrb_b = g.nrb_b;
                p.groups = g.groups; p.DHW = g.DHW; p.N = g.N; p.silu = g.silu; p.rows_per_block = g.rows_per_block; p.eps = g.eps;
                p.gamma = (const float*)rp(bs, g.gamma); p.beta = (const float*)rp(bs, g.beta); p.out = (bf16_t*)rp(bs, g.out);
                p.ab = (float*)rp(bs, g.ab); p.mr = (float*)rp(bs, g.mr); p.xcd_rows = xcd_rows_mode();
// ... 280 lines not shown
}

static int ensure_derived(ldm_model* m, hipStream_t s) {
    if (!m->derived_dirty) return 0;
    for (const auto& iw : m->im2col_ws)
        hipLaunchKernelGGL(im2col_weights_kernel, dim3((unsigned)((iw.cout_pad * iw.Kp + 255) / 256)), dim3(256), 0, s,
                           (const bf16_t*)(m->arena + iw.w_off), (bf16_t*)(m->arena + iw.wi_off), iw.cout_pad, iw.cin_s, iw.cin, iw.Kp);
    for (const auto& pw : m->phase_ws) {
        const long vecs = (long)pw.cout_pad * pw.cin_s / 8;
        hipLaunchKernelGGL(phase_weights_kernel, dim3((unsigned)((vecs + 255) / 256), 64), dim3(256), 0, s,
                           (const bf16_t*)(m->arena + pw.w_off), (bf16_t*)(m->arena + pw.wp_off), pw.cout_pad, pw.cin_s);
    }
    if (m->precision == 1 && m->arena32)
        for (const auto& xw : m->x3p_ws)
            hipLaunchKernelGGL(x3_phase_weights_kernel, dim3((unsigned)(((long)xw.cout_pad * xw.cin_s / 4 + 255) / 256), 64), dim3(256), 0, s,
                               (const float*)(m->arena32 + 2 * xw.w_off), (bf16_t*)(m->arena32 + 2 * m->arena_bytes + xw.x3p_off), xw.cout_pad, xw.cin_s);
    if (m->precision == 1 && m->arena32)
        for (const auto& xw : m->x3_ws)
            hipLaunchKernelGGL(x3_weights_kernel, dim3(grid_for(xw.rows * (xw.cin_s / 4), 256, 2048)), dim3(256), 0, s,
                               (const float*)(m->arena32 + 2 * xw.w_off), (bf16_t*)(m->arena32 + 2 * m->arena_bytes + xw.x3_off), xw.rows, xw.cin_s);
    HIP_TRY(hipGetLastError());
    m->derived_dirty = false;
    return 0;
}

static int get_plan(ldm_model* m, const char* kind, int B, int D, int H, int W, std::shared_ptr<Plan>* out, int tap_mode = 0) {
    if (B < 1 || D < 1 || H < 1 || W < 1 || D > 255 * 8 || H > 255 * 8 || W > 255 * 8) return fail(LDM_ERR_BAD_ARG, "bad shape");
    const bool train = kind[0] == 't';
    const bool hp = m->precision == 1;
    char key[96]; snprintf(key, sizeof key, "%s:%d:%d:%d:%d:p%d:t%d", kind, B, D, H, W, hp ? 1 : 0, tap_mode);
    auto it = m->plans.find(key);
    if (it != m->plans.end()) { *out = it->second; return 0; }
    std::shared_ptr<Plan> p(new Plan());
    if (m->type == 0) LDM_TRY(unet_build(m, B, D, H, W, p.get(), train, hp, tap_mode, strcmp(kind, "unet_tab") == 0));
    else if (train) LDM_TRY(vae_build_train(m, B, D, H, W, p.get(), hp));
    else if (kind[0] == 'e') LDM_TRY(vae_build_encode(m, B, D, H, W, p.get(), hp, tap_mode));
    else LDM_TRY(vae_build_decode(m, B, D, H, W, p.get(), hp, tap_mode));
    m->plans[key] = p; *out = p;
    return 0;
}

static int check_ready(ldm_model* m, const void* ws, size_t ws_bytes, const Plan& p) {
    if (m->loaded_count != (int)m->params.size()) {
        for (auto& d : m->params) if (!d.loaded)
            return fail(LDM_ERR_NOT_LOADED, "parameter '%s' (and %d others) not uploaded", d.name.c_str(),
                        (int)m->params.size() - m->loaded_count - 1);
    }
    if (!ws || ws_bytes < p.ws_bytes) return fail(LDM_ERR_WORKSPACE, "workspace too small: need %zu bytes, got %zu", p.ws_bytes, ws_bytes);
    if (((uintptr_t)ws) & 255) return fail(LDM_ERR_BAD_ARG, "workspace must be 256-byte aligned");
    if (p.wt_tab.ready() || p.exp_tab.ready() || p.cs_tab.ready()) return fail(LDM_ERR_HIP, "descriptor table upload failed");
    return 0;
}

size_t ldm_unet_workspace_bytes(ldm_model* m, int B, int D, int H, int W) {
    if (!m || m->type != 0) { fail(LDM_ERR_BAD_ARG, "not a UNet handle"); return 0; }
    std::shared_ptr<Plan> p; if (get_plan(m, "unet", B, D, H, W, &p)) return 0;
    return p->ws_bytes;
}

static std::atomic<uint64_t> g_sampler_uid{0};
struct ldm_sampler {
    float* coef = nullptr; SamplerState* st = nullptr; int n_steps = 0, kind = 0, clip = 1, pred = PRED_EPSILON; unsigned seed_lo = 0, seed_hi = 0;
    uint64_t uid = ++g_sampler_uid;
    float* state = nullptr; int64_t state_n = 0;
    std::vector<float> ts;
};
enum { SAMPLER_DDPM = 0, SAMPLER_DDIM = 1, SAMPLER_PNDM = 2 };
extern "C++" template <bool SAMPLE = true, class Launch>
static void with_pred(int pred, Launch&& launch) {
    if constexpr (SAMPLE) if (pred == PRED_SAMPLE) return launch(std::integral_constant<int, PRED_SAMPLE>{});
    if (pred == PRED_V) return launch(std::integral_constant<int, PRED_V>{});
    launch(std::integral_constant<int, PRED_EPSILON>{});
}
static int pndm_check_state(const ldm_sampler* sp, int64_t n) {
    if (sp->kind != SAMPLER_PNDM) return 0;
    if (!sp->state) return fail(LDM_ERR_BAD_ARG, "PNDM sampler without a state buffer: call ldm_sampler_bind_state first");
    if (sp->state_n != n) return fail(LDM_ERR_BAD_ARG, "PNDM sampler: the state buffer is bound for %lld elements, the step has %lld",
                                      (long long)sp->state_n, (long long)n);
    return 0;
}
static int sampler_launch(ldm_sampler* sp, const float* eps, float* x, float* x0_out, int64_t n, float* tbuf, int B, hipStream_t s) {
    if (sp->kind == SAMPLER_PNDM) {
        if (x0_out) return fail(LDM_ERR_BAD_ARG, "PNDM has no x0_hat: x0_out must be NULL");
        LDM_TRY(pndm_check_state(sp, n));
        PndmParams p{}; p.coef = sp->coef; p.st = sp->st; p.n_steps = sp->n_steps; p.m = eps; p.x = x; p.state = sp->state; p.n = (long)n;
        p.tbuf = tbuf; p.B = B;
        const dim3 grid(grid_for((n + 3) / 4, 256, 1024));
        with_pred<false>(sp->pred, [&](auto P) { hipLaunchKernelGGL(pndm_sampler_step_kernel<P()>, grid, dim3(256), 0, s, p); });
        return 0;
    }
    SamplerParams p{}; p.coef = sp->coef; p.st = sp->st; p.n_steps = sp->n_steps; p.kind = sp->kind; p.clip = sp->clip;
    p.seed_lo = sp->seed_lo; p.seed_hi = sp->seed_hi; p.eps = eps; p.x = x; p.x0_out = x0_out; p.n = (long)n; p.tbuf = tbuf; p.B = B;
    const dim3 grid(grid_for((n + 3) / 4, 256, 1024));
    with_pred(sp->pred, [&](auto P) { hipLaunchKernelGGL(sampler_step_kernel<P()>, grid, dim3(256), 0, s, p); });
    return 0;
}

static bool temb_table_enabled() { static const int v = ldm_knob("LDM_TEMB_TABLE", 1); return v != 0; }
static int ensure_temb_table(ldm_model* m, const ldm_sampler* sp, hipStream_t s) {
    if (m->temb_tab_valid && m->temb_tab_prec == m->precision && m->temb_tab_ts == sp->ts) return 0;
    const int n = sp->n_steps, rows = m->tproj_rows, c0 = m->ucfg.channels[0], temb = 4 * c0;
    const bool hp = m->precision == 1;
    if (hp && !m->arena32) return fail(LDM_ERR_NOT_LOADED, "fp32 precision: the fp32 weight arena is empty");
    const size_t need = (size_t)n * rows * 4;
    if (need > m->temb_tab_cap) {
        HIP_TRY(hipDeviceSynchronize());
        for (auto& g : m->graphs) if (g.exec) (void)hipGraphExecDestroy(g.exec);
        m->graphs.clear();
        if (m->temb_tab) (void)hipFree(m->temb_tab);
        m->temb_tab = nullptr; m->temb_tab_cap = 0;
        HIP_TRY(hipMalloc((void**)&m->temb_tab, need));
        m->temb_tab_cap = need;
    }
    float* tmp = nullptr;
    HIP_TRY(hipMalloc((void**)&tmp, (size_t)n * (1 + c0 + 2 * temb) * 4));
    float* d_t = tmp; float* d_sin = tmp + n; float* d_e1 = d_sin + (size_t)n * c0; float* d_e2 = d_e1 + (size_t)n * temb;
    hipError_t e = hipMemcpyAsync(d_t, sp->ts.data(), (size_t)n * 4, hipMemcpyHostToDevice, s);
    if (e == hipSuccess) {
        const LinW& l0 = m->lins.at("time_embed.0"); const LinW& l2 = m->lins.at("time_embed.2");
        hipLaunchKernelGGL(temb_sinusoid_kernel, dim3(grid_for((long)n * c0)), dim3(256), 0, s, (const float*)d_t, d_sin, n, c0);
        auto gemv = [&](size_t w_off, size_t b_off, const float* xin, float* y, int I, int O, int silu) {
            if (hp) hipLaunchKernelGGL(gemv_f32_kernel, dim3((O + 3) / 4, n), dim3(256), 0, s, (const float*)(m->arena32 + 2 * w_off),
                                       (const float*)(m->arena + b_off), xin, y, I, O, I, O, silu);
            else hipLaunchKernelGGL(gemv_bf16_kernel, dim3((O + 3) / 4, n), dim3(256), 0, s, (const bf16_t*)(m->arena + w_off),
                                    (const float*)(m->arena + b_off), xin, y, I, O, I, O, silu);
// ... 25 lines not shown
        if (g.plan == probe.plan && g.plan2 == probe.plan2 && !memcmp(g.ptr, probe.ptr, sizeof g.ptr) && g.rt[0] == probe.rt[0] &&
            g.rt[1] == probe.rt[1] && g.sampler_uid == probe.sampler_uid && g.grid_uid == probe.grid_uid && g.chunk == probe.chunk &&
            g.sampler_state == probe.sampler_state) { ge = &g; break; }
    if (!ge) {
        if (m->graphs.size() >= 16) {
            if (m->graphs.front().exec) (void)hipGraphExecDestroy(m->graphs.front().exec);
            m->graphs.erase(m->graphs.begin());
        }
        ldm_model::GraphEntry g = probe; g.seen = 0; g.exec = nullptr;
        m->graphs.push_back(g); ge = &m->graphs.back();
    }
    if (ge->exec) { HIP_TRY(hipGraphLaunch(ge->exec, stream)); return 0; }
    if (ge->seen++ == 0) return run_all(stream);
    hipGraph_t graph = nullptr;
    if (!m->cap_stream) HIP_TRY(hipStreamCreateWithFlags(&m->cap_stream, hipStreamNonBlocking));
    HIP_TRY(hipStreamBeginCapture(m->cap_stream, hipStreamCaptureModeThreadLocal));
    const int rc = run_all(m->cap_stream);
    const hipError_t ec = hipStreamEndCapture(m->cap_stream, &graph);
    if (rc) { if (graph) (void)hipGraphDestroy(graph); return rc; }
    if (ec != hipSuccess || !graph) return fail(LDM_ERR_HIP, "stream capture failed: %s", hipGetErrorString(ec));
    HIP_TRY(hipGraphInstantiate(&ge->exec, graph, nullptr, nullptr, 0));
    (void)hipGraphDestroy(graph);
    HIP_TRY(hipGraphLaunch(ge->exec, stream));
    return 0;
}

static int unet_forward_impl(ldm_model* m, const float* x, int x_channels, const float* cond, int cond_channels,
                             const float* timesteps, float* out, int B, int D, int H, int W,
                             void* workspace, size_t workspace_bytes, void* stream, ldm_sampler* sp, float* x_inout) {
    if (!m || m->type != 0) return fail(LDM_ERR_BAD_ARG, "not a UNet handle");
    if (!x || !timesteps || !out) return fail(LDM_ERR_BAD_ARG, "null tensor argument");
    if (!cond) cond_channels = 0;
    const bool tab = sp != nullptr && temb_table_enabled() && m->tproj_rows % 4 == 0;
    std::shared_ptr<Plan> p; LDM_TRY(get_plan(m, tab ? "unet_tab" : "unet", B, D, H, W, &p));
    LDM_TRY(check_ready(m, workspace, workspace_bytes, *p));
    if (tab) LDM_TRY(ensure_temb_table(m, sp, (hipStream_t)stream));
    Bases bs{}; bs.p[BASE_WS] = (char*)workspace; bs.p[BASE_W] = m->arena; bs.p[BASE_W32] = m->arena32;
    bs.p[BASE_IO0] = (char*)x; bs.p[BASE_IO1] = (char*)cond; bs.p[BASE_IO2] = (char*)timesteps; bs.p[BASE_IO3] = (char*)out;
    if (tab) { bs.p[BASE_TTAB] = (char*)m->temb_tab; bs.p[BASE_SST] = (char*)sp->st; bs.sampler_steps = sp->n_steps; }
    const int rt[2] = {x_channels, cond_channels};
    LDM_TRY(ensure_derived(m, (hipStream_t)stream));
    LaneCtx lanes;
    const int64_t n_out = (int64_t)B * m->ucfg.out_channels * D * H * W;
    auto run_all = [&](hipStream_t s) -> int {
        LDM_TRY(run_plan(*p, bs, rt, s, 0, (size_t)-1, lanes));
        if (sp) LDM_TRY(sampler_launch(sp, out, x_inout, nullptr, n_out, (float*)timesteps, B, s));
        return 0;
    };
    if (!m->graph_mode || g_prof.on || g_plan_trace.on) return run_all((hipStream_t)stream);
    ldm_model::GraphEntry probe{}; probe.plan = p.get();
    const void* key[8] = {x, cond, timesteps, out, workspace, stream, sp, x_inout};
    memcpy(probe.ptr, key, sizeof key); probe.rt[0] = rt[0]; probe.rt[1] = rt[1]; probe.sampler_uid = sp ? sp->uid : 0;
    probe.sampler_state = sp ? sp->state : nullptr;
    return graph_run(m, probe, sp, (hipStream_t)stream, run_all);
}

int ldm_unet_forward(ldm_model* m, const float* x, int x_channels, const float* cond, int cond_channels,
                     const float* timesteps, float* out, int B, int D, int H, int W,
                     void* workspace, size_t workspace_bytes, void* stream) {
    return unet_forward_impl(m, x, x_channels, cond, cond_channels, timesteps, out, B, D, H, W, workspace, workspace_bytes, stream, nullptr, nullptr);
}

static int sampler_alloc(const float* coef_host, int row_len, int n_steps, std::unique_ptr<ldm_sampler>* out) {
    std::unique_ptr<ldm_sampler> sp(new ldm_sampler());
    const size_t bytes = (size_t)n_steps * row_len * 4;
    HIP_TRY(hipMalloc((void**)&sp->coef, bytes));
    HIP_TRY(hipMemcpy(sp->coef, coef_host, bytes, hipMemcpyHostToDevice));
    HIP_TRY(hipMalloc((void**)&sp->st, 256));
    HIP_TRY(hipMemset(sp->st, 0, 256));
    HIP_TRY(hipDeviceSynchronize());
    sp->n_steps = n_steps;
    sp->ts.resize(n_steps); for (int k = 0; k < n_steps; ++k) sp->ts[k] = coef_host[(size_t)k * row_len + 5];
    *out = std::move(sp);
    return 0;
}
int ldm_sampler_create(const float* coef_host, int n_steps, int kind, int pred, int clip, uint64_t seed, ldm_sampler** out) {
    if (!coef_host || n_steps < 1 || kind < 0 || kind > 1 || !out) return fail(LDM_ERR_BAD_ARG, "bad argument");
    if (pred < PRED_EPSILON || pred > PRED_V) return fail(LDM_ERR_BAD_ARG, "unknown prediction type %d (0 epsilon, 1 sample, 2 v_prediction)", pred);
    std::unique_ptr<ldm_sampler> sp; LDM_TRY(sampler_alloc(coef_host, 8, n_steps, &sp));
// ... 24 lines not shown
    sp->kind = SAMPLER_PNDM; sp->pred = pred; sp->clip = 0;
    *out = sp.release();
    return 0;
}
size_t ldm_sampler_state_bytes(const ldm_sampler* sp, int64_t n) {
    if (!sp || n < 0) { fail(LDM_ERR_BAD_ARG, "bad argument"); return 0; }
    return sp->kind == SAMPLER_PNDM ? (size_t)n * 6 * sizeof(float) : 0;
}
int ldm_sampler_bind_state(ldm_sampler* sp, void* state, size_t bytes, int64_t n) {
    if (!sp || !state || n < 0) return fail(LDM_ERR_BAD_ARG, "bad argument");
    if (sp->kind != SAMPLER_PNDM) return fail(LDM_ERR_BAD_ARG, "only a PNDM sampler takes a state buffer");
    if ((uintptr_t)state % sizeof(float)) return fail(LDM_ERR_BAD_ARG, "state buffer not aligned to 4 bytes");
    const size_t need = ldm_sampler_state_bytes(sp, n);
    if (bytes < need) return fail(LDM_ERR_BAD_ARG, "state buffer of %zu bytes, %zu needed for %lld elements", bytes, need, (long long)n);
    sp->state = (float*)state; sp->state_n = n;
    return 0;
}
void ldm_sampler_destroy(ldm_sampler* sp) {
    if (!sp) return;
    if (sp->coef) (void)hipFree(sp->coef);
    if (sp->st) (void)hipFree(sp->st);
    delete sp;
}
int ldm_sampler_reset(ldm_sampler* sp, float* tbuf, int B, void* stream) {
    if (!sp || !tbuf || B < 1) return fail(LDM_ERR_BAD_ARG, "bad argument");
    hipLaunchKernelGGL(sampler_reset_kernel, dim3(1), dim3(64), 0, (hipStream_t)stream, sp->st, (const float*)sp->coef, tbuf, B);
    HIP_TRY(hipGetLastError());
    return 0;
}
int ldm_sampler_step(ldm_sampler* sp, const float* eps, float* x, float* x0_out, int64_t n, float* tbuf, int B, void* stream) {
    if (!sp || !eps || !x || !tbuf || n < 0 || B < 1) return fail(LDM_ERR_BAD_ARG, "bad argument");
    if (sp->kind == SAMPLER_PNDM && eps == x) return fail(LDM_ERR_BAD_ARG, "PNDM: the model output may not alias x");
    LDM_TRY(sampler_launch(sp, eps, x, x0_out, n, tbuf, B, (hipStream_t)stream));
    HIP_TRY(hipGetLastError());
    return 0;
}
int ldm_sampler_noise(const ldm_sampler* sp, int step, float* out, int64_t n, void* stream) {
    if (!sp || !out || n < 0 || step < 0) return fail(LDM_ERR_BAD_ARG, "bad argument");
    hipLaunchKernelGGL(sampler_noise_kernel, dim3(grid_for((n + 3) / 4, 256, 1024)), dim3(256), 0, (hipStream_t)stream, out, (long)n, step, sp->seed_lo, sp->seed_hi);
    HIP_TRY(hipGetLastError());
    return 0;
}
int ldm_unet_denoise_step(ldm_model* m, ldm_sampler* sp, float* x, int x_channels, const float* cond, int cond_channels,
                          float* tbuf, float* eps_scratch, int B, int D, int H, int W,
                          void* workspace, size_t workspace_bytes, void* stream) {
    if (!sp) return fail(LDM_ERR_BAD_ARG, "null sampler");
    if (m && m->type == 0 && x_channels != m->ucfg.out_channels) return fail(LDM_ERR_BAD_ARG, "x must have the UNet's out_channels (%d)", m->ucfg.out_channels);
    LDM_TRY(pndm_check_state(sp, (int64_t)B * x_channels * D * H * W));
    return unet_forward_impl(m, x, x_channels, cond, cond_channels, tbuf, eps_scratch, B, D, H, W, workspace, workspace_bytes, stream, sp, x);
}

static std::atomic<uint64_t> g_grid_uid{0};
struct ldm_window_grid {
    int dims[3] = {0, 0, 0}, roi[3] = {0, 0, 0}, n[3] = {0, 0, 0};
    char* dev = nullptr;
    WinGeom geom{};
    uint64_t uid = ++g_grid_uid;
    int64_t n_windows() const { return (int64_t)n[0] * n[1] * n[2]; }
    int64_t roi_vox() const { return (int64_t)roi[0] * roi[1] * roi[2]; }
    int64_t vox() const { return (int64_t)dims[0] * dims[1] * dims[2]; }
};

int ldm_window_grid_create(const int* dims, const int* roi, const int* n, const int* starts, const float* weights, const int* cover,
                           ldm_window_grid** out) {
    if (!dims || !roi || !n || !starts || !weights || !cover || !out) return fail(LDM_ERR_BAD_ARG, "null argument");
    std::unique_ptr<ldm_window_grid> g(new ldm_window_grid());
// ... 584 lines not shown
}
int ldm_profile_stop(double out[5]) {
    if (!out) return fail(LDM_ERR_BAD_ARG, "null out");
    g_prof.on = false;
    double ms = 0.0, fl = 0.0;
    for (size_t k = 0; k + 1 < g_prof.used + 1 && k < g_prof.used; k += 2) {
        HIP_TRY(hipEventSynchronize(g_prof.ev[k + 1]));
        float t = 0.f; HIP_TRY(hipEventElapsedTime(&t, g_prof.ev[k], g_prof.ev[k + 1]));
        ms += t; fl += g_prof.flops[k / 2];
    }
    out[0] = (double)(g_prof.used / 2); out[1] = ms; out[2] = fl; out[3] = (double)g_prof.launches_all; out[4] = g_prof.flops_all;
    for (auto e : g_prof.ev) (void)hipEventDestroy(e);
    g_prof.ev.clear(); g_prof.used = 0; g_prof.flops.clear();
    return 0;
}
int ldm_model_plan_conv_cfgs(ldm_model* m, const char* kind, int B, int D, int H, int W, int* cfgs, int max_convs) {
    if (!m || !kind) return fail(LDM_ERR_BAD_ARG, "null argument");
    std::shared_ptr<Plan> p; LDM_TRY(get_plan(m, kind, B, D, H, W, &p));
    int n = 0;
    for (const Op& o : p->ops) if (o.kind == OP_CONV) {
        if (cfgs && n < max_convs) { cfgs[4 * n] = o.cc.wgm; cfgs[4 * n + 1] = o.cc.wgn; cfgs[4 * n + 2] = o.cc.bk | ((o.cc.cube ? 5 : o.cc.plane ? 6 : o.cc.halo) << 8); cfgs[4 * n + 3] = o.cc.splitk; }
        ++n;
    } else if (o.kind == OP_CONV_BLOCK) {
        if (cfgs && n < max_convs) { cfgs[4 * n] = 4; cfgs[4 * n + 1] = o.cv.couts == 128 ? 2 : 1; cfgs[4 * n + 2] = 32 | ((o.cv.couts == 128 ? 4 : 3) << 8); cfgs[4 * n + 3] = 1; }
        ++n;
    }
    return n;
}

int ldm_model_plan_launches(ldm_model* m, const char* kind, int B, int D, int H, int W) {
    if (!m || !kind) return fail(LDM_ERR_BAD_ARG, "null argument");
    std::shared_ptr<Plan> p; LDM_TRY(get_plan(m, kind, B, D, H, W, &p));
    int n = 0;
    for (const Op& o : p->ops) if (o.kind != OP_TAP) ++n;
    return n;
}

static char* g_zero_page = nullptr;
static int ensure_zero_page() {
    if (g_zero_page) return 0;
    HIP_TRY(hipMalloc((void**)&g_zero_page, 8192));
    HIP_TRY(hipMemset(g_zero_page, 0, 8192));
    HIP_TRY(hipDeviceSynchronize());
    return 0;
}

int ldm_op_conv3d_block128(const void* x, int cin, const void* w, const float* bias, const float* temb, int temb_stride, const void* residual,
                           void* out, float* stats, int N, int D, int H, int W, void* stream) {
    if (!x || !w || !out || N < 1 || D < 1 || H < 1 || W < 1 || cin < 32 || cin % 32) return fail(LDM_ERR_BAD_ARG, "bad argument");
    if ((long)N * D * H * W * cin * 2 >= (1L << 32)) return fail(LDM_ERR_BAD_ARG, "the input tensor exceeds 4 GiB (split the batch)");
    BlockParams q{}; q.x = (const bf16_t*)x; q.w = (const bf16_t*)w; q.bias = bias; q.temb = temb; q.temb_stride = temb_stride;
    q.residual = (const bf16_t*)residual; q.out = (bf16_t*)out; q.stats = stats; q.N = N; q.D = D; q.H = H; q.W = W; q.Cin = cin;
    HIP_TRY(launch_conv_block128(q, (hipStream_t)stream));
    return 0;
}
int ldm_debug_conv_block_slots(int slots) {
#ifdef LDM_EXPERIMENTS
    const int old = g_block_slots; g_block_slots = slots < 0 ? 0 : slots; return old;
#else
    (void)slots; return -1;
#endif
}
int ldm_op_conv3d_block_stats_rows(int D, int H, int W, int th) {
    if (th != 4 && th != 8) return 0;
    return ((D + BLK_TD - 1) / BLK_TD) * ((H + th - 1) / th) * ((W + BLK_TW - 1) / BLK_TW);
}
int ldm_op_conv3d_block(const void* x, int cin, const void* w, const float* bias, const float* temb, int temb_stride, const void* residual,
                        void* out, float* stats, int N, int D, int H, int W, int th, void* stream) {
    if (!x || !w || !out || N < 1 || D < 1 || H < 1 || W < 1 || cin < 32 || cin % 32 || (th != 4 && th != 8)) return fail(LDM_ERR_BAD_ARG, "bad argument");
    if ((long)N * D * H * W * cin * 2 >= (1L << 32)) return fail(LDM_ERR_BAD_ARG, "the input tensor exceeds 4 GiB (split the batch)");
    BlockParams q{}; q.x = (const bf16_t*)x; q.w = (const bf16_t*)w; q.bias = bias; q.temb = temb; q.temb_stride = temb_stride;
    q.residual = (const bf16_t*)residual; q.out = (bf16_t*)out; q.stats = stats; q.N = N; q.D = D; q.H = H; q.W = W; q.Cin = cin;
    HIP_TRY(launch_conv_block(q, th, (hipStream_t)stream));
    return 0;
}

static int op_conv3d_impl(const void* xa, int ca, const void* xb, int cb, const void* w, const float* bias,
                          const void* x1a, int c1a, const void* x1b, int c1b, const void* w1, const float* bias2,
                          const float* temb, int temb_stride, const void* residual, void* out_bf16, float* out_f32,
                          int N, int Din, int Hin, int Win, int ksize, int stride, int pad, int ups,
                          int cout, int cout_pad, int wgn, int splitk, void* scratch, size_t scratch_bytes, void* stream,
                          float* stats, int* stats_nrb, FinGnParams* fg = nullptr) {
    if (!xa || !w || (!out_bf16 && !out_f32 && !fg)) return fail(LDM_ERR_BAD_ARG, "null tensor argument");
    if (!xb) cb = 0;
    if (!x1a) { c1a = 0; c1b = 0; }
    if (!x1b) c1b = 0;
    const int cin0 = ca + cb, cin1 = c1a + c1b;
    const int cmax = (ksize == 1 && stride == 1 && pad == 0 && ups == 0) ? 65536 : 4096;
    if (ca % 32 || cb % 32 || c1a % 32 || c1b % 32 || cout_pad % 64 || cout > cout_pad || cin0 > cmax || cin1 > 4096)
        return fail(LDM_ERR_BAD_ARG, "channel counts must be multiples of 32 (cout_pad of 64), at most %d per row", cmax);
    if (ksize != 1 && ksize != 3) return fail(LDM_ERR_UNSUPPORTED, "ksize must be 1 or 3");
    int exact = 0;
    if (ups == 2) { ups = 1; exact = 1; }
    if (ups < 0 || ups > 1 || stride < 1 || stride > 2) return fail(LDM_ERR_UNSUPPORTED, "stride 1|2, ups 0|1|2");
    LDM_TRY(ensure_zero_page());
    int bk = 64;
    if (ca % 64 || cb % 64 || c1a % 64 || c1b % 64) bk = 32;
    const int Du = Din << ups, Hu = Hin << ups, Wu = Win << ups;
    const int pad_total = (stride == 2 && pad == 0 && ksize == 3) ? 1 : 2 * pad;
    const int Do = (Du + pad_total - ksize) / stride + 1, Ho = (Hu + pad_total - ksize) / stride + 1,
              Wo = (Wu + pad_total - ksize) / stride + 1;
    const long M = (long)N * Do * Ho * Wo;
    if (M >= (1L << 31) || M < 1) return fail(LDM_ERR_BAD_ARG, "bad output size");
    if (!stats && !wgn && !splitk && out_bf16 && !out_f32 && gemm_light_ok(ksize, stride, ups, cin0, cin1 == 0, !temb && !bias2) &&
        Builder::light_enabled() && M * (long)cin0 * 2 < (1L << 31)) {
        LightParams lp{}; lp.x = (const bf16_t*)xa; lp.w = (const bf16_t*)w; lp.bias = bias; lp.residual = (const bf16_t*)residual;
// ... 236 lines not shown
    hipLaunchKernelGGL(pack2_ncdhw_f32_kernel, dim3(grid_for((long)N * DHW * Cs)), dim3(256), 0, (hipStream_t)stream, x, C, (const float*)nullptr, 0, out, N, Cs, (int)DHW);
    HIP_TRY(hipGetLastError());
    return 0;
}
int ldm_op_unpack_ndhwc_f32(const float* act, float* out, int N, int C, int Cs, int64_t DHW, void* stream) {
    if (!act || !out || N < 1 || C < 1 || C > Cs || DHW < 1 || DHW >= (1L << 31)) return fail(LDM_ERR_BAD_ARG, "bad argument");
    hipLaunchKernelGGL(unpack_ndhwc_kernel<float>, dim3(grid_for((long)N * C * DHW)), dim3(256), 0, (hipStream_t)stream, act, out, N, C, Cs, (int)DHW);
    HIP_TRY(hipGetLastError());
    return 0;
}
int ldm_op_gemm_f32(const float* x, int K, const float* w, const float* bias, float* out, int64_t M, int cout, int cout_pad, int couts, void* stream) {
    if (!x || !w || !out || M < 1 || M >= (1L << 31) || K < 16 || K % 16 || cout < 1 || cout_pad % 64 || cout_pad < cout || couts % 4 || couts < cout || couts > cout_pad)
        return fail(LDM_ERR_BAD_ARG, "bad argument");
    Conv32Params p{}; p.xa = x; p.ca = K; p.w = w; p.N = 1; p.Din = p.Dout = (int)M; p.Hin = p.Win = p.Hout = p.Wout = 1;
    p.ksize = 1; p.stride = 1; p.pad = 0; p.M = (int)M; p.CoutS = couts; p.CoutPad = cout_pad; p.CoutReal = cout;
    p.nchunk = K / 16; p.steps = p.nchunk; p.splitk = 1; p.steps_per_split = p.steps; p.mtiles = (int)((M + 127) / 128);
    p.bias = bias; p.out = out;
    const int bn = cout_pad % 128 == 0 ? 128 : 64;
    p.ntiles = cout_pad / bn;
    launch_conv32(p, false, bn, (hipStream_t)stream);
    HIP_TRY(hipGetLastError());
    return 0;
}
int ldm_op_linear_f32x3(const float* xa, int ca, const float* xb, int cb, const float* w, const float* bias, const float* residual, float* out,
                        float* stats, int64_t M, int cout_pad, int couts, int big, void* stream) {
    if (!xa || !w || !out || M < 1 || ca < 32 || ca % 32 || cb < 0 || cb % 32 || (cb > 0 && !xb) || cout_pad < 32 || cout_pad % 32 || couts < 32 || couts % 32 ||
        couts > cout_pad || M * (int64_t)std::max(ca + cb, cout_pad) * 4 >= (1L << 31) || (big == 1 && cout_pad % 64))
        return fail(LDM_ERR_BAD_ARG, "bad argument");
    LightX3Params p{}; p.x = xa; p.xb = cb > 0 ? xb : nullptr; p.ca = ca; p.w = w; p.bias = bias; p.residual = residual; p.out = out; p.stats = stats;
    p.M = (int)M; p.K = ca + cb; p.CoutS = couts;
    HIP_TRY(launch_gemm_light_x3(p, cout_pad, big < 0 ? gemm_light_x3_big(M, cout_pad) : big, (hipStream_t)stream));
    return 0;
}
int ldm_op_linear_bf16(const void* xa, int ca, const void* xb, int cb, const void* w, const float* bias, const void* residual, void* out,
                       float* stats, int64_t M, int cout_pad, int couts, int big, int kernel,
                       const float* gn_slabs, int gn_nrb, int gn_dhw, const float* gamma, const float* beta, int groups, float eps, int fold,
                       void* scratch, void* stream) {
    const int K = ca + (xb ? cb : 0);
    if (!xa || !w || !out || M < 1 || ca < 32 || ca % 32 || cb < 0 || cb % 32 || (cb > 0 && !xb) || cout_pad < 32 || cout_pad % 32 || couts < 32 || couts % 32 ||
        couts > cout_pad || M * (int64_t)std::max(K, cout_pad) * 2 >= (1L << 31) || (big == 1 && cout_pad % 64) || kernel < -1 || kernel > 1 ||
        !(K % 128 == 0 || K < 128) || K > 2048)
        return fail(LDM_ERR_BAD_ARG, "bad argument");
    const bool one = !xb || cb == 0;
    const bool wg_shape = one && K % 128 == 0 && K >= 128 && K <= 512;
    if (kernel == 1 && !wg_shape) return fail(LDM_ERR_UNSUPPORTED, "gemm_wg_kernel takes one source and K = 128 .. 512 in steps of 128");
    LightParams p{}; p.x = (const bf16_t*)xa; p.xb = one ? nullptr : (const bf16_t*)xb; p.ca = one ? K : ca; p.w = (const bf16_t*)w; p.bias = bias;
    p.residual = (const bf16_t*)residual; p.out = (bf16_t*)out; p.stats = stats; p.M = (int)M; p.K = K; p.CoutS = couts;
    if (big < 0) big = cout_pad % 64 == 0 ? gemm_light_big(M, cout_pad) : 0;
    const int wg = kernel < 0 ? gemm_wg_ok(one, K, M) : kernel;
    if (gn_slabs) {
        if (!one || !gamma || !beta || groups < 1 || K % groups || K % 8 || K / groups > 64 || gn_nrb < 1 || gn_nrb > 512 || gn_dhw < 1 || M % gn_dhw || fold < 0 || fold > 1 ||
            (!fold && !scratch))
            return fail(LDM_ERR_BAD_ARG, "bad GroupNorm argument");
        if (fold) {
            if (!wg || !wg_shape || !gemm_wg_gn_shape_ok(K, gn_dhw, groups, gn_nrb, big))
                return fail(LDM_ERR_UNSUPPORTED, "the GroupNorm prologue needs gemm_wg_kernel, K >= 256, at most 16 slab rows, even groups of at most 64 channels");
            WgGnParams g{}; g.slabs = gn_slabs; g.gamma = gamma; g.beta = beta; g.nrb = gn_nrb; g.groups = groups; g.DHW = gn_dhw; g.eps = eps;
            HIP_TRY(launch_gemm_wg(p, cout_pad, big, (hipStream_t)stream, &g));
            return 0;
        }
        const int N = (int)(M / gn_dhw), slices = (K + 63) / 64;
        int chunks = std::max(1, std::min(512 / (slices * N), (gn_dhw + 31) / 32));
        const int rpb = rup((gn_dhw + chunks - 1) / chunks, 32);
        chunks = (gn_dhw + rpb - 1) / rpb;
        GnFusedParams g{}; g.xa = (const bf16_t*)xa; g.ca = K; g.sa = gn_slabs; g.nrb_a = gn_nrb; g.groups = groups; g.DHW = gn_dhw; g.N = N;
        g.rows_per_block = rpb; g.eps = eps; g.gamma = gamma; g.beta = beta; g.out = (bf16_t*)scratch;
// ... 830 lines not shown
```

3d-latent-diffusion-model_amd/csrc/norm_elem.h:

```cpp
#pragma once
#include "common.h"

struct GnStatsParams {
    const bf16_t* xa; const bf16_t* xb; int ca, cb;
    int DHW; int nslab; int rows_per_slab;
    float* partial;
};

__global__ __launch_bounds__(256) void gn_stats_kernel(const GnStatsParams p) {
    __shared__ float red[256 * 16];
    const int C = p.ca + p.cb;
    const int cvec = C / 8;
    const int n = blockIdx.y, slab = blockIdx.x;
    const int r0 = slab * p.rows_per_slab;
    int r1 = r0 + p.rows_per_slab; if (r1 > p.DHW) r1 = p.DHW;
    float s[8], q[8];
#pragma unroll
    for (int k = 0; k < 8; ++k) { s[k] = 0.f; q[k] = 0.f; }
    const int tid = threadIdx.x;
    const int rows_par = 256 / cvec > 0 ? 256 / cvec : 1;
    if (cvec <= 256) {
        const int cv = tid % cvec, rl = tid / cvec;
        if (rl < rows_par) {
            const int c = cv * 8;
// ... 439 lines not shown
__global__ __launch_bounds__(256) void add_noise_target_kernel(const float* __restrict__ x0, const float* __restrict__ eps,
                                                               const float* __restrict__ sa, const float* __restrict__ sb,
                                                               float* __restrict__ noisy, float* __restrict__ target, long per_sample, int B) {
#pragma clang fp contract(off)
    const long n = per_sample * B;
    for (long i = (long)blockIdx.x * blockDim.x + threadIdx.x; i < n; i += (long)gridDim.x * blockDim.x) {
        const int b = (int)(i / per_sample);
        const float a = sa[b], s = sb[b], xv = x0[i], ev = eps[i];
        if (noisy) noisy[i] = __fmaf_rn(a, xv, s * ev);
        if constexpr (PRED == PRED_EPSILON) target[i] = ev;
        else if constexpr (PRED == PRED_SAMPLE) target[i] = xv;
        else target[i] = __fmaf_rn(a, ev, -(s * xv));
    }
}

__global__ __launch_bounds__(256) void vae_heads_kernel(const float* __restrict__ ml, const float* __restrict__ eps,
                                                        float* __restrict__ mu, float* __restrict__ sigma,
                                                        float* __restrict__ z, int N, int L, int DHW) {
    const long total = (long)N * L * DHW;
    for (long i = (long)blockIdx.x * blockDim.x + threadIdx.x; i < total; i += (long)gridDim.x * blockDim.x) {
        const int n = (int)(i / ((long)L * DHW));
        const long r = i - (long)n * L * DHW;
        const float m = ml[(size_t)n * 2 * L * DHW + r];
        float lv = ml[(size_t)n * 2 * L * DHW + (long)L * DHW + r];
        lv = fminf(fmaxf(lv, -30.f), 20.f);
        const float sg = expf(0.5f * lv);
        if (mu) mu[i] = m;
        if (sigma) sigma[i] = sg;
        if (z) z[i] = m + sg * (eps ? eps[i] : 0.f);
    }
}

struct SamplerState { int k; unsigned done; };
struct SamplerParams {
    const float* coef; SamplerState* st; int n_steps; int kind;
    int clip; unsigned seed_lo, seed_hi;
    const float* eps; float* x; float* x0_out; long n;
    float* tbuf; int B;
};
__device__ __forceinline__ void philox4x32_10(unsigned c0, unsigned c1, unsigned c2, unsigned c3, unsigned k0, unsigned k1, unsigned out[4]) {
#pragma unroll
    for (int r = 0; r < 10; ++r) {
        const unsigned hi0 = __umulhi(0xD2511F53u, c0), lo0 = 0xD2511F53u * c0;
        const unsigned hi1 = __umulhi(0xCD9E8D57u, c2), lo1 = 0xCD9E8D57u * c2;
        const unsigned n0 = hi1 ^ c1 ^ k0, n2 = hi0 ^ c3 ^ k1;
        c0 = n0; c1 = lo1; c2 = n2; c3 = lo0;
        k0 += 0x9E3779B9u; k1 += 0xBB67AE85u;
    }
    out[0] = c0; out[1] = c1; out[2] = c2; out[3] = c3;
}
__device__ __forceinline__ float4 sampler_normal4(unsigned long long quad, unsigned step, unsigned seed_lo, unsigned seed_hi) {
    unsigned r[4];
    philox4x32_10((unsigned)quad, (unsigned)(quad >> 32), step, 0x5eedu, seed_lo, seed_hi, r);
    const float u0 = ((float)(r[0] >> 8) + 1.0f) * (1.0f / 16777216.0f), u1 = (float)(r[1] >> 8) * (1.0f / 16777216.0f);
    const float u2 = ((float)(r[2] >> 8) + 1.0f) * (1.0f / 16777216.0f), u3 = (float)(r[3] >> 8) * (1.0f / 16777216.0f);
    const float ra = sqrtf(-2.0f * logf(u0)), rb = sqrtf(-2.0f * logf(u2));
    float sa, ca, sb, cb;
    sincosf(6.283185307179586f * u1, &sa, &ca); sincosf(6.283185307179586f * u3, &sb, &cb);
    return make_float4(ra * ca, ra * sa, rb * cb, rb * sb);
}
__global__ __launch_bounds__(256) void sampler_noise_kernel(float* __restrict__ out, long n, int step, unsigned seed_lo, unsigned seed_hi) {
    const long nq = (n + 3) / 4;
    for (long q = (long)blockIdx.x * blockDim.x + threadIdx.x; q < nq; q += (long)gridDim.x * blockDim.x) {
        const float4 z = sampler_normal4((unsigned long long)q, (unsigned)step, seed_lo, seed_hi);
        const float zz[4] = {z.x, z.y, z.z, z.w};
        for (int e = 0; e < 4; ++e) if (4 * q + e < n) out[4 * q + e] = zz[e];
    }
}
struct SamplerCoef { float inv_sqrt_a, sqrt_b, c0, c1, sigma, sqrt_a, inv_sqrt_b; };
template <int PRED>
__device__ __forceinline__ SamplerCoef sampler_coef(const float* coef, int k, int n_steps) {
// ... 17 lines not shown
        eh = __fmaf_rn(c.sqrt_a, ee, c.sqrt_b * xe);
    }
    if (clip) x0 = fminf(fmaxf(x0, -1.f), 1.f);
    float pv = c.c0 * x0 + c.c1 * (kind == 0 ? xe : eh);
    if (c.sigma != 0.f) pv = __fmaf_rn(c.sigma, z, pv);
    *x0_out = x0;
    return pv;
}
__device__ __forceinline__ void sampler_advance(SamplerState* st, const float* coef, int n_steps, int k, float* tbuf, int B, int stride = 8) {
    __shared__ int s_last;
    __syncthreads();
    if (threadIdx.x == 0) s_last = (atomicAdd(&st->done, 1u) == gridDim.x - 1) ? 1 : 0;
    __syncthreads();
    if (s_last && threadIdx.x == 0) {
        st->done = 0;
        const int kn = k < n_steps ? k + 1 : k;
        st->k = kn;
        const float tn = coef[(size_t)(kn < n_steps ? kn : n_steps - 1) * stride + 5];
        for (int b = 0; b < B; ++b) tbuf[b] = tn;
    }
}
template <int PRED>
__global__ __launch_bounds__(256) void sampler_step_kernel(const SamplerParams p) {
    KSTAMP_BEGIN(9);
    const int k = p.st->k;
    const bool live = k < p.n_steps;
    const SamplerCoef c = sampler_coef<PRED>(p.coef, k, p.n_steps);
    const long nq = (p.n + 3) / 4;
    if (live)
    for (long q = (long)blockIdx.x * blockDim.x + threadIdx.x; q < nq; q += (long)gridDim.x * blockDim.x) {
        float4 z = make_float4(0.f, 0.f, 0.f, 0.f);
        if (c.sigma != 0.f) z = sampler_normal4((unsigned long long)q, (unsigned)k, p.seed_lo, p.seed_hi);
        const float zz[4] = {z.x, z.y, z.z, z.w};
#pragma unroll
        for (int e = 0; e < 4; ++e) {
            const long i = 4 * q + e;
            if (i >= p.n) break;
            float x0;
            p.x[i] = sampler_update<PRED>(c, p.kind, p.clip, p.x[i], p.eps[i], zz[e], &x0);
            if (p.x0_out) p.x0_out[i] = x0;
        }
    }
    sampler_advance(p.st, p.coef, p.n_steps, k, p.tbuf, p.B);
}
template <int PRED>
__global__ __launch_bounds__(256) void scheduler_step_kernel(const float* __restrict__ m, const float* __restrict__ x,
                                                             const float* __restrict__ z, float* __restrict__ prev,
                                                             float* __restrict__ x0_out, long n, const SamplerCoef c, int kind, int clip) {
    for (long i = (long)blockIdx.x * blockDim.x + threadIdx.x; i < n; i += (long)gridDim.x * blockDim.x) {
        float x0;
        prev[i] = sampler_update<PRED>(c, kind, clip, x[i], m[i], z ? z[i] : 0.f, &x0);
        if (x0_out) x0_out[i] = x0;
    }
}
__global__ void sampler_reset_kernel(SamplerState* st, const float* coef, float* tbuf, int B) {
    if (threadIdx.x == 0 && blockIdx.x == 0) { st->k = 0; st->done = 0; for (int b = 0; b < B; ++b) tbuf[b] = coef[5]; }
}
enum { PNDM_ROW = 16, PNDM_PUSH = 1, PNDM_SAVE = 2, PNDM_USE_SAVED = 4, PNDM_ACC_SET = 8, PNDM_ACC_ADD = 16 };
struct PndmCoef { float cx, ce, sqrt_a, sqrt_b, wm, w1, w2, w3, wacc, am; int flags, head; };
__host__ __device__ __forceinline__ PndmCoef pndm_coef(const float* c) {
    return PndmCoef{c[0], c[1], c[2], c[3], c[6], c[7], c[8], c[9], c[10], c[11], (int)c[4], (int)c[12]};
}
template <int PRED>
__device__ __forceinline__ float pndm_update(const PndmCoef& c, float xs, float m, float h1, float h2, float h3, float acc, float* acc_out) {
#pragma clang fp contract(off)
    static_assert(PRED == PRED_EPSILON || PRED == PRED_V, "PNDM: epsilon or v_prediction");
    float e = c.wm * m;
    if (c.w1 != 0.f) e = __fmaf_rn(c.w1, h1, e);
    if (c.w2 != 0.f) e = __fmaf_rn(c.w2, h2, e);
    if (c.w3 != 0.f) e = __fmaf_rn(c.w3, h3, e);
    if (c.wacc != 0.f) e = __fmaf_rn(c.wacc, acc, e);
    if (c.flags & PNDM_ACC_SET) acc = c.am * m;
// ... 2 lines not shown
    if constexpr (PRED == PRED_V) e = __fmaf_rn(c.sqrt_a, e, c.sqrt_b * xs);
    return __fmaf_rn(c.cx, xs, c.ce * e);
}
struct PndmSlots { const float *h1, *h2, *h3, *saved_in, *acc_in; float *push, *save, *acc_out; };
__device__ __forceinline__ PndmSlots pndm_slots(const PndmCoef& c, float* state, long n) {
    PndmSlots s{};
    if (c.w1 != 0.f) s.h1 = state + (long)((c.head - 1) & 3) * n;
    if (c.w2 != 0.f) s.h2 = state + (long)((c.head - 2) & 3) * n;
    if (c.w3 != 0.f) s.h3 = state + (long)((c.head - 3) & 3) * n;
    if (c.flags & PNDM_USE_SAVED) s.saved_in = state + 4 * n;
    if (c.wacc != 0.f || (c.flags & PNDM_ACC_ADD)) s.acc_in = state + 5 * n;
    if (c.flags & PNDM_PUSH) s.push = state + (long)(c.head & 3) * n;
    if (c.flags & PNDM_SAVE) s.save = state + 4 * n;
    if (c.flags & (PNDM_ACC_SET | PNDM_ACC_ADD)) s.acc_out = state + 5 * n;
    return s;
}
template <int PRED>
__device__ __forceinline__ float pndm_element(const PndmCoef& c, const PndmSlots& s, float* __restrict__ x, float m, long i) {
    const float xe = x[i];
    const float xs = s.saved_in ? s.saved_in[i] : xe;
    float acc;
    const float xn = pndm_update<PRED>(c, xs, m, s.h1 ? s.h1[i] : 0.f, s.h2 ? s.h2[i] : 0.f, s.h3 ? s.h3[i] : 0.f,
                                       s.acc_in ? s.acc_in[i] : 0.f, &acc);
    if (s.push) s.push[i] = m;
    if (s.save) s.save[i] = xe;
    if (s.acc_out) s.acc_out[i] = acc;
    x[i] = xn;
    return xn;
}
struct PndmParams {
    const float* coef; SamplerState* st; int n_steps;
    const float* m; float* x; float* state; long n;
    float* tbuf; int B;
};
template <int PRED>
__global__ __launch_bounds__(256) void pndm_sampler_step_kernel(const PndmParams p) {
    const int k = p.st->k;
    if (k < p.n_steps) {
        const PndmCoef c = pndm_coef(p.coef + (size_t)k * PNDM_ROW);
        const PndmSlots s = pndm_slots(c, p.state, p.n);
        const long nq = (p.n + 3) / 4;
        for (long q = (long)blockIdx.x * blockDim.x + threadIdx.x; q < nq; q += (long)gridDim.x * blockDim.x) {
#pragma unroll
            for (int e = 0; e < 4; ++e) {
                const long i = 4 * q + e;
                if (i >= p.n) break;
                pndm_element<PRED>(c, s, p.x, p.m[i], i);
            }
        }
    }
    sampler_advance(p.st, p.coef, p.n_steps, k, p.tbuf, p.B, PNDM_ROW);
}
template <int PRED>
__global__ __launch_bounds__(256) void pndm_step_kernel(const float* __restrict__ m, const float* __restrict__ x, const float* __restrict__ h1,
                                                        const float* __restrict__ h2, const float* __restrict__ h3,
                                                        const float* __restrict__ saved, const float* acc_in, float* acc_out,
                                                        float* __restrict__ prev, long n, const PndmCoef c) {
    for (long i = (long)blockIdx.x * blockDim.x + threadIdx.x; i < n; i += (long)gridDim.x * blockDim.x) {
        float acc;
        prev[i] = pndm_update<PRED>(c, saved ? saved[i] : x[i], m[i], h1 ? h1[i] : 0.f, h2 ? h2[i] : 0.f, h3 ? h3[i] : 0.f,
                                    acc_in ? acc_in[i] : 0.f, &acc);
        if (acc_out) acc_out[i] = acc;
    }
}
__global__ __launch_bounds__(256) void temb_row_kernel(const float* __restrict__ tab, const SamplerState* __restrict__ st,
                                                       float* __restrict__ out, int rows, int stride, int n_steps) {
    KSTAMP_BEGIN(1);
    int k = st->k; if (k >= n_steps) k = n_steps - 1; if (k < 0) k = 0;
    const int q = blockIdx.x * blockDim.x + threadIdx.x;
    KSTAMP(1);
    if (4 * q < rows)
        *reinterpret_cast<float4*>(out + (size_t)blockIdx.y * stride + 4 * q) = *reinterpret_cast<const float4*>(tab + (size_t)k * rows + 4 * q);
    KSTAMP_DRAIN(2);
}

template <class T> __device__ __forceinline__ float el_ld(const T* p);
template <> __device__ __forceinline__ float el_ld<bf16_t>(const bf16_t* p) { return bf2f(*p); }
template <> __device__ __forceinline__ float el_ld<float>(const float* p) { return *p; }
template <class T> __device__ __forceinline__ void el_st(T* p, float v);
template <> __device__ __forceinline__ void el_st<bf16_t>(bf16_t* p, float v) { *p = f2bf(v); }
// ... 978 lines not shown
```

include/ldm3d.h:

```cpp
#ifndef LDM3D_H
#define LDM3D_H
#include <stddef.h>
#include <stdint.h>

#ifdef __cplusplus
extern "C" {
#endif

#define LDM_MAX_LEVELS 8
#define LDM_ABI_VERSION 1

typedef enum {
    LDM_OK = 0,
    LDM_ERR_BAD_ARG = -1,
    LDM_ERR_UNSUPPORTED = -2,
    LDM_ERR_HIP = -3,
    LDM_ERR_NOT_LOADED = -4,
    LDM_ERR_WORKSPACE = -5,
    LDM_ERR_RCCL = -6
} ldm_status;

typedef struct {
    int spatial_dims;
    int in_channels, out_channels;
// ... 90 lines not shown

size_t ldm_vae_encode_workspace_bytes(ldm_model* m, int B, int D, int H, int W);
size_t ldm_vae_decode_workspace_bytes(ldm_model* m, int B, int d, int h, int w);
int ldm_vae_encode(ldm_model* m, const float* x, const float* eps, float* z_mu, float* z_sigma, float* z,
                   int B, int D, int H, int W, void* workspace, size_t workspace_bytes, void* stream);
int ldm_vae_decode(ldm_model* m, const float* z, float* out, int B, int d, int h, int w,
                   void* workspace, size_t workspace_bytes, void* stream);

int ldm_add_noise(const float* x0, const float* eps, const float* sqrt_a, const float* sqrt_b, float* out,
                  int B, int64_t per_sample, void* stream);
int ldm_scale(const float* x, float* y, int64_t n, float s, void* stream);
int ldm_scheduler_step(const float* model_out, const float* x, const float* noise, float* prev, float* x0_out, int64_t n, int kind, int pred,
                       const float* row, int clip, void* stream);
int ldm_add_noise_target(const float* x0, const float* eps, const float* sqrt_a, const float* sqrt_b, float* noisy, float* target,
                         int B, int64_t per_sample, int pred, void* stream);

typedef struct ldm_sampler ldm_sampler;
int ldm_sampler_create(const float* coef_host, int n_steps, int kind , int pred, int clip, uint64_t seed, ldm_sampler** out);
#define LDM_PNDM_ROW 16
#define LDM_PNDM_PUSH 1
#define LDM_PNDM_SAVE 2
#define LDM_PNDM_USE_SAVED 4
#define LDM_PNDM_ACC_SET 8
#define LDM_PNDM_ACC_ADD 16
int ldm_sampler_create_pndm(const float* coef_host, int n_steps, int pred, ldm_sampler** out);
size_t ldm_sampler_state_bytes(const ldm_sampler* sp, int64_t n);
int ldm_sampler_bind_state(ldm_sampler* sp, void* state, size_t bytes, int64_t n);
int ldm_pndm_step(const float* m, const float* x, const float* h1, const float* h2, const float* h3, const float* saved,
                  const float* acc_in, float* acc_out, float* prev, int64_t n, int pred, const float* row, void* stream);
void ldm_sampler_destroy(ldm_sampler* sp);
int ldm_sampler_reset(ldm_sampler* sp, float* tbuf, int B, void* stream);
int ldm_sampler_step(ldm_sampler* sp, const float* eps, float* x, float* x0_out, int64_t n, float* tbuf, int B, void* stream);
int ldm_sampler_noise(const ldm_sampler* sp, int step, float* out, int64_t n, void* stream);
int ldm_unet_denoise_step(ldm_model* m, ldm_sampler* sp, float* x, int x_channels, const float* cond, int cond_channels,
                          float* tbuf, float* eps_scratch, int B, int D, int H, int W,
                          void* workspace, size_t workspace_bytes, void* stream);

typedef struct ldm_window_grid ldm_window_grid;
int ldm_window_grid_create(const int* dims, const int* roi, const int* n, const int* starts, const float* weights, const int* cover,
                           ldm_window_grid** out);
void ldm_window_grid_destroy(ldm_window_grid* grid);
int ldm_window_gather(const ldm_window_grid* grid, const float* src, float* dst, int C, void* stream);
int ldm_window_blend(const ldm_window_grid* grid, const float* src, float* dst, int C, void* stream);
int ldm_unet_denoise_step_windows(ldm_model* m, ldm_sampler* sp, const ldm_window_grid* grid, float* x, int x_channels,
                                  const float* cond_w, int cond_channels, float* xw, float* eps_w, float* tbuf, int chunk,
                                  void* workspace, size_t workspace_bytes, void* stream);

int ldm_op_conv3d(const void* xa, int ca, const void* xb, int cb, const void* w, const float* bias,
                  const void* x1a, int c1a, const void* x1b, int c1b, const void* w1, const float* bias2,
                  const float* temb, int temb_stride, const void* residual, void* out_bf16, float* out_f32,
                  int N, int Din, int Hin, int Win, int ksize, int stride, int pad, int ups,
                  int cout, int cout_pad, int wgn, int splitk, void* scratch, size_t scratch_bytes, void* stream);
int ldm_op_conv3d_block_stats_rows(int D, int H, int W, int th);
int ldm_op_conv3d_block128(const void* x, int cin, const void* w, const float* bias, const float* temb, int temb_stride, const void* residual,
                           void* out, float* stats, int N, int D, int H, int W, void* stream);
int ldm_debug_conv_block_slots(int slots);
int ldm_op_conv3d_block(const void* x, int cin, const void* w, const float* bias, const float* temb, int temb_stride, const void* residual,
                        void* out, float* stats, int N, int D, int H, int W, int th, void* stream);
int ldm_op_weight_flip_transpose(const void* w, void* wt, int ksize, int cout, int cout_pad, int cin, void* stream);
int ldm_op_conv3d_wgrad(const void* dy, int cdy, const void* x, int cx, float* dw, int cout, int cin,
                        int N, int Din, int Hin, int Win, int ksize, int stride, int pad, int ups, int ksplit, void* stream);
size_t ldm_op_group_norm_bwd_scratch_bytes(int N, int C, int DHW, int groups);
int ldm_op_group_norm_bwd(const void* dy, const void* xa, int ca, const void* xb, int cb, const float* gamma, const float* beta,
                          int groups, float eps, int silu, const void* acc_a, const void* acc_b, void* dxa, void* dxb,
                          float* dgamma, float* dbeta, int N, int DHW, void* scratch, size_t scratch_bytes, void* stream);
size_t ldm_op_scale_intensity_percentiles_scratch_bytes(int B);
int ldm_op_scale_intensity_percentiles(const float* x, float* out, int B, int64_t n, float lower, float upper, float b_min, float b_max,
                                       void* scratch, size_t scratch_bytes, void* stream);
size_t ldm_op_image_metrics_scratch_bytes(int B, int C, int D, int H, int W, int win);
int ldm_op_image_metrics(const float* x, const int64_t* x_strides, const float* y, const int64_t* y_strides, int B, int C, int D, int H, int W,
                         const float* weights, int win, float data_range, float k1, float k2, float* out, float* ssim_map,
                         void* scratch, size_t scratch_bytes, void* stream);
int ldm_op_im2col(const void* x, void* col, int N, int D, int H, int W, int Cs, int C, int k, int stride, int pad, int Kp, void* stream);
int ldm_op_col2im(const void* dcol, void* dx, int N, int D, int H, int W, int Cs, int C, int k, int stride, int pad, int Kp, void* stream);
int ldm_op_leaky_relu(const void* x, void* y, int64_t n, float slope, void* stream);
int ldm_op_leaky_relu_bwd(const void* x, const void* dy, void* dx, int64_t n, float slope, void* stream);
int ldm_op_pack_ncdhw(const float* x, void* out_bf16_ndhwc, int N, int C, int Cs, int64_t DHW, void* stream);
int ldm_op_unpack_ndhwc(const void* act_bf16_ndhwc, float* out, int N, int C, int Cs, int64_t DHW, void* stream);
int ldm_op_pack_ncdhw_f32(const float* x, float* out_f32_ndhwc, int N, int C, int Cs, int64_t DHW, void* stream);
int ldm_op_unpack_ndhwc_f32(const float* act_f32_ndhwc, float* out, int N, int C, int Cs, int64_t DHW, void* stream);
int ldm_op_im2col_f32(const float* x, float* col, int N, int D, int H, int W, int Cs, int C, int k, int stride, int pad, int Kp, void* stream);
int ldm_op_col2im_f32(const float* dcol, float* dx, int N, int D, int H, int W, int Cs, int C, int k, int stride, int pad, int Kp, void* stream);
int ldm_op_leaky_relu_f32(const float* x, float* y, int64_t n, float slope, void* stream);
int ldm_op_leaky_relu_bwd_f32(const float* x, const float* dy, float* dx, int64_t n, float slope, void* stream);
int ldm_op_gemm_f32(const float* x, int K, const float* w, const float* bias, float* out, int64_t M, int cout, int cout_pad, int couts, void* stream);
int ldm_op_gemm_wgrad_f32(const float* dy, int cdy, const float* x, int K, float* dw, int cout, int64_t M, int ksplit, void* stream);
int ldm_op_linear_f32x3(const float* xa, int ca, const float* xb, int cb, const float* w, const float* bias, const float* residual, float* out,
                        float* stats, int64_t M, int cout_pad, int couts, int big, void* stream);
int ldm_op_linear_bf16(const void* xa, int ca, const void* xb, int cb, const void* w, const float* bias, const void* residual, void* out,
                       float* stats, int64_t M, int cout_pad, int couts, int big, int kernel,
                       const float* gn_slabs, int gn_nrb, int gn_dhw, const float* gamma, const float* beta, int groups, float eps, int fold,
                       void* scratch, void* stream);
size_t ldm_op_group_norm_f32_scratch_bytes(int N, int C, int DHW, int groups);
int ldm_op_group_norm_f32(const float* x, int C, const float* gamma, const float* beta, int groups, float eps, int act, float* out,
                          int N, int DHW, void* scratch, size_t scratch_bytes, void* stream);
int ldm_op_group_norm_bwd_f32(const float* dy, const float* x, int C, const float* gamma, const float* beta, int groups, float eps, int act,
                              float* dx, float* dgamma, float* dbeta, int N, int DHW, void* scratch, size_t scratch_bytes, void* stream);
int ldm_op_conv3d_f32_stats_blocks(int N, int dhwo, int couts, int* rows);
int ldm_op_conv3d_f32(const float* xa, int ca, const float* xb, int cb, const float* w, const float* bias, const float* temb, int temb_stride,
                      const float* residual, float* out, int couts, float* out_ncdhw, float* stats, int N, int Din, int Hin, int Win,
                      int ksize, int stride, int pad, int ups, int cout, int cout_pad, int form, int bn, int splitk,
                      void* scratch, size_t scratch_bytes, void* stream);
size_t ldm_op_weight_flip_transpose_f32_ws_bytes(int ksize, int cout, int ci_cnt);
int ldm_op_weight_flip_transpose_f32(const float* w, float* wt, int ksize, int cout, int cout_pad, int cin, int ci_off, int ci_cnt,
                                     void* desc_ws, size_t desc_ws_bytes, void* stream);
int ldm_op_conv3d_wgrad_f32(const float* dy, int cdy, const float* x, int cx, float* dw, int cout, int cin, int dw_ld, int dw_ci_off,
                            int N, int Din, int Hin, int Win, int ksize, int stride, int pad, int ups, int ksplit, void* stream);
int ldm_op_attention_f32(const float* qkv, float* out, float* lse, int B, int N, int C, int head_dim, int x3, void* stream);
int ldm_op_attention_bwd_f32(const float* qkv, const float* o, const float* d_o, const float* lse, float* delta_scratch, float* dqkv,
                             int B, int N, int C, int head_dim, void* stream);
int ldm_op_group_norm_bwd2_f32(const float* dy, const float* xa, int ca, const float* xb, int cb, const float* gamma, const float* beta,
                               int groups, float eps, int act, const float* acc_a, const float* acc_b, float* dxa, float* dxb,
                               float* dgamma, float* dbeta, int N, int DHW, void* scratch, size_t scratch_bytes, void* stream);
int ldm_op_upsample_bwd_f32(const float* dy, float* dx, int N, int D, int H, int W, int C, void* stream);
size_t ldm_op_group_norm_bwd_saved_scratch_bytes(int N, int C, int DHW, int groups);
int ldm_op_group_norm_bwd_fold_chunks(int N, int C, int groups, int DHW);
int ldm_op_group_norm_bwd_saved(const void* dy, const void* xa, int ca, const void* xb, int cb, const float* ab, const float* mr,
                                const float* gamma, int groups, int act, const void* acc_a, const void* acc_b, void* dxa, void* dxb,
                                float* dgamma, float* dbeta, float* cs, int N, int DHW, int form, void* scratch, size_t scratch_bytes,
                                void* stream);
size_t ldm_op_colsum_finalize_ws_bytes(const int64_t* desc, int k);
// ... 68 lines not shown
```

Measured before the change: 531.9.

## Split-K thin output conv into sampler step and fuse conv_in im2col with temb

The final thin output convolution can be split along input channels into per-chunk partial buffers. The sampler/PNDM step kernel then sums those partials plus bias in a fixed order, which removes the separate reduction and gives the small conv more blocks. A separate path fuses the conv_in im2col packing into the GEMM prologue and lets spare blocks copy the timestep-embedding row, removing extra launches. This costs partial-buffer memory traffic and extra kernel complexity; the im2col fusion sits behind a knob that is off by default.

```diff
diff --git a/3d-latent-diffusion-model_amd/_lib.py b/3d-latent-diffusion-model_amd/_lib.py
--- a/3d-latent-diffusion-model_amd/_lib.py
+++ b/3d-latent-diffusion-model_amd/_lib.py
@@ -92,6 +92,7 @@
     "ldm_sampler_reset": (C.c_int, [_P, _P, C.c_int, _P]),
     "ldm_sampler_step": (C.c_int, [_P, _P, _P, _P, C.c_int64, _P, C.c_int, _P]),
     "ldm_sampler_noise": (C.c_int, [_P, C.c_int, _P, C.c_int64, _P]),
+    "ldm_op_sampler_step_parts": (C.c_int, [_P, _P, C.c_int, C.c_int64, _P, C.c_int, C.c_int, _P, _P, C.c_int64, _P, C.c_int, _P]),
     "ldm_unet_denoise_step": (C.c_int, [_P, _P, _P, C.c_int, _P, C.c_int, _P, _P, C.c_int, C.c_int, C.c_int, C.c_int,
                                         _P, C.c_size_t, _P]),
     "ldm_window_grid_create": (C.c_int, [_P, _P, _P, _P, _P, _P, C.POINTER(_P)]),
@@ -103,6 +104,8 @@
                                 C.c_int, C.c_int, C.c_int, C.c_int, C.c_int, C.c_int, C.c_int, C.c_int, C.c_int, C.c_int,
                                 C.c_int, C.c_int, _P, C.c_size_t, _P]),
     "ldm_op_weight_flip_transpose": (C.c_int, [_P, _P, C.c_int, C.c_int, C.c_int, C.c_int, _P]),
+    "ldm_op_conv_in_im2col": (C.c_int, [_P, C.c_int, _P, C.c_int, _P, _P, _P, _P] + [C.c_int] * 9 + [_P, _P, _P, _P, C.c_int, C.c_int, _P]),
+    "ldm_op_conv3d_thin": (C.c_int, [_P, C.c_int, _P, _P, _P, C.c_int, C.c_int, C.c_int, C.c_int, C.c_int, C.c_int, C.c_int, _P]),
     "ldm_op_conv3d_wgrad": (C.c_int, [_P, C.c_int, _P, C.c_int, _P, C.c_int, C.c_int, C.c_int, C.c_int, C.c_int, C.c_int,
                                       C.c_int, C.c_int, C.c_int, C.c_int, C.c_int, _P]),
     "ldm_op_group_norm_bwd_scratch_bytes": (C.c_size_t, [C.c_int, C.c_int, C.c_int, C.c_int]),
diff --git a/3d-latent-diffusion-model_amd/csrc/conv_thin.h b/3d-latent-diffusion-model_amd/csrc/conv_thin.h
--- a/3d-latent-diffusion-model_amd/csrc/conv_thin.h
+++ b/3d-latent-diffusion-model_amd/csrc/conv_thin.h
@@ -16,8 +16,10 @@
 constexpr int THIN_LDS_X = THIN_HV * THIN_RB, THIN_LDS_W = 27 * 4 * THIN_RB;
 constexpr int THIN_LDS = THIN_LDS_X + THIN_LDS_W;
 
+template <bool SPLIT>
 __global__ __launch_bounds__(256) void conv3_thin_kernel(const ThinParams p) {
 #if defined(__HIP_DEVICE_COMPILE__)
+    KSTAMP_BEGIN(11);
     extern __shared__ __attribute__((aligned(16))) char smem[];
     char* sx = smem; char* sw = smem + THIN_LDS_X;
     const int tid = threadIdx.x, lane = tid & 63, wave = tid >> 6, fr = lane & 15, fg = lane >> 4;
@@ -31,7 +33,8 @@
 #pragma unroll
     for (int t = 0; t < 4; ++t) acc[t] = (f32x4){0.f, 0.f, 0.f, 0.f};
     const u32x4 zero = {0u, 0u, 0u, 0u};
-    for (int c0 = 0; c0 < p.Cin; c0 += THIN_CK) {
+    const int c_begin = SPLIT ? (int)blockIdx.y * THIN_CK : 0, c_end = SPLIT ? c_begin + THIN_CK : p.Cin;
+    for (int c0 = c_begin; c0 < c_end; c0 += THIN_CK) {
         __syncthreads();
         const int xc0 = (p.x3_c && c0 >= p.x3_c) ? c0 - p.x3_c : c0;
         constexpr int NIT = (THIN_HV * THIN_NC + 255) / 256;
@@ -59,6 +62,7 @@
             *reinterpret_cast<u32x4*>(sw + (tap * 4 + row) * THIN_RB + ((c16 ^ row) << 4)) = v;
         }
         __syncthreads();
+        KSTAMP(1);
 #pragma unroll 1
         for (int tap = 0; tap < 27; ++tap) {
             const int kd = tap / 9, kh = (tap / 3) % 3, kw = tap % 3;
@@ -73,10 +77,12 @@
             }
         }
     }
+    KSTAMP(2);
     if (fg != 0) return;
     const int gd = d0 + wave, gw = w0 + wm;
     if (gd >= p.D || gw >= p.W) return;
     const size_t dhw = (size_t)p.D * p.H * p.W;
+    float* const out = SPLIT ? p.out + (size_t)blockIdx.y * p.N * p.CoutReal * dhw : p.out;
 #pragma unroll
     for (int t = 0; t < 4; ++t) {
         const int gh = h0 + t;
@@ -84,7 +90,8 @@
         const size_t sp = ((size_t)gd * p.H + gh) * p.W + gw;
 #pragma unroll
         for (int r = 0; r < 4; ++r)
-            if (r < p.CoutReal) p.out[((size_t)n * p.CoutReal + r) * dhw + sp] = acc[t][r] + (p.bias ? p.bias[r] : 0.f);
+            if (r < p.CoutReal) out[((size_t)n * p.CoutReal + r) * dhw + sp] = SPLIT ? acc[t][r] : acc[t][r] + (p.bias ? p.bias[r] : 0.f);
     }
+    KSTAMP_DRAIN(3);
 #endif
 }
diff --git a/3d-latent-diffusion-model_amd/csrc/gemm_wg.h b/3d-latent-diffusion-model_amd/csrc/gemm_wg.h
--- a/3d-latent-diffusion-model_amd/csrc/gemm_wg.h
+++ b/3d-latent-diffusion-model_amd/csrc/gemm_wg.h
@@ -8,20 +8,41 @@
     int nrb, groups, DHW; float eps;
 };
 
+struct SamplerState;
+struct WgI2cParams {
+    const float* x; const float* cond; int cx, cc;
+    int D, H, W;
+    const float* tab; const SamplerState* st; float* temb_out; int rows, n_steps, temb_blocks;
+};
+template <bool I2C> struct WgPrologue { typedef WgGnParams type; };
+template <> struct WgPrologue<true> { typedef WgI2cParams type; };
+
 __device__ __forceinline__ void wg_copies_landed_barrier() {
     asm volatile("s_waitcnt vmcnt(0)" ::: "memory");
     __builtin_amdgcn_s_barrier();
     asm volatile("" ::: "memory");
 }
 
-template <int MT, int NWV, bool GN>
-__global__ __launch_bounds__(64 * NWV) void gemm_wg_kernel(const LightParams p, const int cout_pad, const WgGnParams g) {
+template <int MT, int NWV, bool GN, bool I2C = false>
+__global__ __launch_bounds__(64 * NWV) void gemm_wg_kernel(const LightParams p, const int cout_pad, const typename WgPrologue<I2C>::type g) {
 #if defined(__HIP_DEVICE_COMPILE__)
+    static_assert(!(GN && I2C), "one prologue");
     extern __shared__ __attribute__((aligned(16))) char smem[];
     typedef __attribute__((address_space(3))) void* lds_ptr_t;
     constexpr int NT = 2, R = 16 * MT, NW = 32 * NWV;
     const int tid = threadIdx.x, lane = tid & 63, fr = lane & 15, fg = lane >> 4;
     const int wave = __builtin_amdgcn_readfirstlane(tid >> 6);
+    if constexpr (I2C) {
+        const int gemm_blocks = p.mtiles * ((cout_pad + NW - 1) / NW);
+        if ((int)blockIdx.x >= gemm_blocks) {
+            const int rb = (int)blockIdx.x - gemm_blocks, b = rb / g.temb_blocks;
+            int k = g.st->k; if (k >= g.n_steps) k = g.n_steps - 1; if (k < 0) k = 0;
+            const int q = (rb - b * g.temb_blocks) * (64 * NWV) + tid;
+            if (4 * q < g.rows)
+                *reinterpret_cast<float4*>(g.temb_out + (size_t)b * g.rows + 4 * q) = *reinterpret_cast<const float4*>(g.tab + (size_t)k * g.rows + 4 * q);
+            return;
+        }
+    }
     const int mtile = blockIdx.x % p.mtiles, ntile = blockIdx.x / p.mtiles;
     const int m0 = mtile * R, n0 = ntile * NW;
     const int nkb = p.K >> 7;
@@ -36,12 +57,14 @@
     double* const csum = reinterpret_cast<double*>(ab + 4 * C);
     float* const gstat = reinterpret_cast<float*>(csum + 2 * C);
     auto slab_loads = [&](const int smp, const int pp) {
+        if constexpr (GN) {
         const float* base = g.slabs + ((size_t)smp * g.nrb * C + 2 * pp) * 2;
 #pragma unroll
         for (int k = 0; k < 16; ++k) {
             int bb = k; const bool ok = bb < g.nrb; if (!ok) bb = g.nrb - 1;
             t[k] = *reinterpret_cast<const float4*>(base + (size_t)bb * C * 2);
             if (!ok) t[k] = make_float4(0.f, 0.f, 0.f, 0.f);
+        }
         }
     };
     if constexpr (GN) {
@@ -64,12 +87,46 @@
             const unsigned vo = (unsigned)co * row2 + (unsigned)kb * 256u + (unsigned)((lane & 15) ^ f) * 16u;
             __builtin_amdgcn_raw_ptr_buffer_load_lds(rs_w, (lds_ptr_t)(smem + u * 1024), 16, vo, 0, 0, 0);
         }
+        if constexpr (!I2C) {
         __amdgpu_buffer_rsrc_t rs_x = __builtin_amdgcn_make_buffer_rsrc((void*)p.x, 0, (int)((unsigned)p.M * row2), 0x00020000);
         for (int u = wave; u < nkb * (R / 4); u += NWV) {
             const int kb = u / (R / 4), lr = 4 * (u % (R / 4)) + (lane >> 4);
             const unsigned vo = (unsigned)(m0 + lr) * row2 + (unsigned)kb * 256u + (unsigned)((lane & 15) ^ (lr & 15)) * 16u;
             __builtin_amdgcn_raw_ptr_buffer_load_lds(rs_x, (lds_ptr_t)(smem + xbase + u * 1024), 16, vo, 0, 0, 0);
         }
+        }
+    }
+    if constexpr (I2C) {
+        const int cin = g.cx + g.cc, HW = g.H * g.W, DHW = g.D * HW, kreal = 27 * cin;
+        for (int q = tid; q < nkb * 16 * R; q += 64 * NWV) {
+            const int lr = q % R, vq = q / R;
+            const int m = m0 + lr;
+            u32x4 o = {0u, 0u, 0u, 0u};
+            if (m < p.M) {
+                const int n = m / DHW, sp = m - n * DHW;
+                const int d = sp / HW, r = sp - d * HW, h = r / g.W, w = r - h * g.W;
+                float v[8];
+#pragma unroll
+                for (int e = 0; e < 8; ++e) {
+                    const int k = vq * 8 + e;
+                    float val = 0.f;
+                    if (k < kreal) {
+                        const int tap = k / cin, c = k - tap * cin;
+                        const int kd = tap / 9, kh = (tap - kd * 9) / 3, kw = tap - kd * 9 - kh * 3;
+                        const int id = d + kd - 1, ih = h + kh - 1, iw = w + kw - 1;
+                        if ((unsigned)id < (unsigned)g.D && (unsigned)ih < (unsigned)g.H && (unsigned)iw < (unsigned)g.W) {
+                            const int spi = (id * g.H + ih) * g.W + iw;
+                            val = c < g.cx ? g.x[((size_t)n * g.cx + c) * DHW + spi] : g.cond[((size_t)n * g.cc + (c - g.cx)) * DHW + spi];
+                        }
+                    }
+                    v[e] = val;
+                }
+#pragma unroll
+                for (int j = 0; j < 4; ++j) o[j] = pack2bf(v[2 * j], v[2 * j + 1]);
+            }
+            *reinterpret_cast<u32x4*>(smem + xbase + (vq >> 4) * (R * 256) + lr * 256 + (((vq & 15) ^ (lr & 15)) << 4)) = o;
+        }
+        asm volatile("s_waitcnt lgkmcnt(0)" ::: "memory");
     }
     const int n0w = n0 + 32 * wave;
     const int wrow = (32 * wave + fr) * 256, xrow = xbase + fr * 256;
@@ -183,6 +240,30 @@
 static inline bool gemm_wg_gn_ok(int K, long DHW, int groups, int nrb, int big) {
     return ldm_knob("LDM_GEMM_WG_GN", 0) != 0 && gemm_wg_gn_shape_ok(K, DHW, groups, nrb, big);
 }
+static inline bool gemm_wg_i2c_ok(int Kp, long M) { return ldm_knob("LDM_IM2COL_FUSED", 0) != 0 && (Kp == 128 || Kp == 256) && M * (long)Kp * 2 < (1L << 31); }
+template <int MT, int NWV>
+static inline hipError_t launch_gemm_wg_i2c_t(const LightParams& p, int cout_pad, const WgI2cParams& g, int B, hipStream_t s) {
+    const int lds = (16 * MT + 32 * NWV) * 2 * p.K;
+    if (p.K > 256) return hipErrorInvalidValue;
+    static bool attr_tab[32] = {}; bool& attr_set = attr_flag(attr_tab);
+    if (!attr_set) {
+        hipError_t e = hipFuncSetAttribute(reinterpret_cast<const void*>(&gemm_wg_kernel<MT, NWV, false, true>), hipFuncAttributeMaxDynamicSharedMemorySize,
+                                           (16 * MT + 32 * NWV) * 2 * 256);
+        if (e != hipSuccess) return e;
+        attr_set = true;
+    }
+    const int blocks = p.mtiles * ((cout_pad + 32 * NWV - 1) / (32 * NWV)) + g.temb_blocks * B;
+    hipLaunchKernelGGL((gemm_wg_kernel<MT, NWV, false, true>), dim3(blocks), dim3(64 * NWV), lds, s, p, cout_pad, g);
+    return hipGetLastError();
+}
+static inline hipError_t launch_gemm_wg_i2c(const LightParams& p0, int cout_pad, int big, WgI2cParams g, int B, hipStream_t s) {
+    LightParams p = p0;
+    const int threads = big ? 256 : 128;
+    if (g.temb_blocks) g.temb_blocks = (g.rows / 4 + threads - 1) / threads;
+    if (big) { p.mtiles = (p.M + 63) / 64; return launch_gemm_wg_i2c_t<4, 4>(p, cout_pad, g, B, s); }
+    p.mtiles = (p.M + 31) / 32;
+    return launch_gemm_wg_i2c_t<2, 2>(p, cout_pad, g, B, s);
+}
 template <int MT, int NWV, bool GN>
 static inline hipError_t launch_gemm_wg_t(const LightParams& p, int cout_pad, const WgGnParams& g, hipStream_t s) {
     constexpr int kmax = (16 * MT + 32 * NWV) * 2 * 512 <= 160 * 1024 ? 512 : 384;
diff --git a/3d-latent-diffusion-model_amd/csrc/ldm3d.hip b/3d-latent-diffusion-model_amd/csrc/ldm3d.hip
--- a/3d-latent-diffusion-model_amd/csrc/ldm3d.hip
+++ b/3d-latent-diffusion-model_amd/csrc/ldm3d.hip
@@ -155,7 +155,7 @@
               OP_CONV_BLOCK,
               OP_TEMB_ROW };
 
-struct ConvCfg { int wgm, wgn, bk, splitk; int halo = 0, mtps = 0, qps = 0; int slab_lg = 0; int cube = 0; int th = 0, big = 0; int plane = 0; int wg = 0; };
+struct ConvCfg { int wgm, wgn, bk, splitk; int halo = 0, mtps = 0, qps = 0; int slab_lg = 0; int cube = 0; int th = 0, big = 0; int plane = 0; int wg = 0; int thin_split = 0; int i2c = 0, temb_ride = 0; };
 
 struct ConvRec {
     Ref xa, xb, w; int ca, cb;
@@ -234,6 +234,7 @@
 
 struct Op {
     OpKind kind;
+    int carried;
     ConvCfg cc;
     ConvRec cv;
     GnRec gn;
@@ -306,6 +307,7 @@
     size_t ws_bytes = 0;
     size_t bwd_begin = 0;
     bool train = false;
+    long eps_split_op = -1;
     mutable DevTable wt_tab, exp_tab, cs_tab;
 };
 
@@ -513,6 +515,7 @@
         Ref temb; int temb_stride = 0;
         Act residual;
         bool f32_out = false; Ref out_ref; int cout_real = 0;
+        bool eps_split = false;
         bool want_stats = true;
         Ref w_over; bool no_bias = false; int exact = 0;
         int temb_row = -1;
@@ -626,10 +629,15 @@
     static long thin_tiles(const ConvArgs& a) {
         return (long)a.xa.N * ((a.Do + THIN_TD - 1) / THIN_TD) * ((a.Ho + THIN_TH - 1) / THIN_TH) * ((a.Wo + THIN_TW - 1) / THIN_TW);
     }
-    void emit_thin(const ConvArgs& a, long M, Ref w, int cout_real, bool x3) {
+    void emit_thin(const ConvArgs& a, long M, Ref w, int cout_real, bool x3, bool split = false) {
         Op op{}; op.kind = OP_CONV_THIN;
         ConvRec& c = op.cv; c = conv_rec(a, 3, 1, 1, M, cout_real); conv_epilogue(c, a, Act());
         c.xa = ws_ref(a.xa.off); c.ca = x3 ? 2 * a.xa.C : a.xa.C; c.x3 = x3; c.w = w;
+        if (split) {
+            op.cc.thin_split = a.xa.C / THIN_CK;
+            partial_bytes = std::max(partial_bytes, (size_t)op.cc.thin_split * M * cout_real * 4); partial_fixups.push_back(plan->ops.size());
+            plan->eps_split_op = (long)plan->ops.size();
+        }
         plan->ops.push_back(op);
     }
     Act emit_light(OpKind kind, const ConvArgs& a, long M, Ref w, int big, bool want_stats) {
@@ -832,10 +840,18 @@
             static const int thin = ldm_knob("LDM_CONV_THIN", 1);
             static const long thin_min = ldm_knob("LDM_CONV_THIN_MIN", 512L);
             const int cr = a.cout_real ? a.cout_real : w.cout;
-            if (thin && a.f32_out && a.k == 3 && a.stride == 1 && a.pad == 1 && !a.ups && !a.exact && !a.xb.valid && !a.w1 &&
-                a.temb.base == BASE_NULL && !a.residual.valid && a.w_over.base == BASE_NULL && cr <= 4 && cin0 % 32 == 0 && cin0 <= 128 &&
-                a.xa.D == a.Do && a.xa.H == a.Ho && a.xa.W == a.Wo &&
-                thin_tiles(a) >= thin_min) {
+            const bool thin_ok = thin && a.f32_out && a.k == 3 && a.stride == 1 && a.pad == 1 && !a.ups && !a.exact && !a.xb.valid && !a.w1 &&
+                a.temb.base == BASE_NULL && !a.residual.valid && a.w_over.base == BASE_NULL && cr <= 4 && cin0 % 32 == 0 &&
+                a.xa.D == a.Do && a.xa.H == a.Ho && a.xa.W == a.Wo;
+            if (thin_ok && !train && ldm_knob("LDM_CONV_THIN_SPLIT", 1) != 0 &&
+                thin_tiles(a) * (cin0 / THIN_CK) >= ldm_knob("LDM_CONV_THIN_SPLIT_MIN", 256L)) {
+                if (a.eps_split) {
+                    emit_thin(a, M, w_ref(w.w_off), cr, false, true);
+                    return Act();
+                }
+                partial_bytes = std::max(partial_bytes, (size_t)(cin0 / THIN_CK) * M * cr * 4);
+            }
+            if (thin_ok && cin0 <= 128 && thin_tiles(a) >= thin_min) {
                 emit_thin(a, M, w_ref(w.w_off), cr, false);
                 record_conv(a, Act());
                 return Act();
@@ -1035,9 +1051,20 @@
         Op o{}; o.kind = OP_IM2COL; LayoutRec& l = o.lay; l.a = r0; l.b = r1; l.dst = ws_ref(pm.off);
         l.N = N; l.c_real = cin; l.c_stored = wi.cin_s; l.D = D; l.H = H; l.W = W; l.internal = internal;
         plan->ops.push_back(o);
+        const size_t im2col_op = plan->ops.size() - 1;
         ConvArgs a; a.xa = pm; a.w = &wi; a.k = 1; a.pad = 0; a.Do = D; a.Ho = H; a.Wo = W;
         Act out = conv(a, name + ".im2col");
         free_act(pm);
+        if (out.valid && plan->ops.size() == im2col_op + 2 && plan->ops.back().kind == OP_GEMM_LIGHT && plan->ops.back().cc.wg != 2 &&
+            gemm_wg_i2c_ok(wi.cin_s, (long)N * D * H * W)) {
+            Op& gemm = plan->ops.back();
+            gemm.cc.wg = 3; gemm.cc.i2c = (int)im2col_op + 1; plan->ops[im2col_op].carried = (int)im2col_op + 2;
+            if (ldm_knob("LDM_TEMB_RIDE", 1) != 0)
+                for (size_t k = 0; k < im2col_op; ++k)
+                    if (plan->ops[k].kind == OP_TEMB_ROW && plan->ops[k].lin.O % 4 == 0) {
+                        gemm.cc.temb_ride = (int)k + 1; plan->ops[k].carried = (int)im2col_op + 2;
+                    }
+        }
         return out;
     }
 
@@ -1493,7 +1520,8 @@
     return 0;
 }
 
-static int unet_build(ldm_model* m, int B, int D, int H, int W, Plan* plan, bool train, bool hp = false, int tap_mode = 0, bool temb_table = false) {
+static int unet_build(ldm_model* m, int B, int D, int H, int W, Plan* plan, bool train, bool hp = false, int tap_mode = 0, bool temb_table = false,
+                      bool step = false) {
     const ldm_unet_cfg& c = m->ucfg;
     const int L = c.num_levels; const int* ch = c.channels;
     const int temb = ch[0] * 4, G = c.norm_num_groups; const float eps = c.norm_eps;
@@ -1607,7 +1635,7 @@
     b.free_act(h);
     if (!hn.valid) return fail(LDM_ERR_UNSUPPORTED, "%s", b.err.c_str());
     Builder::ConvArgs oa; oa.xa = hn; oa.w = &m->convs.at("out.2"); oa.Do = D; oa.Ho = H; oa.Wo = W;
-    oa.f32_out = true; oa.out_ref = io_ref(3); oa.cout_real = c.out_channels;
+    oa.f32_out = true; oa.out_ref = io_ref(3); oa.cout_real = c.out_channels; oa.eps_split = step && !tap_mode;
     b.conv(oa, "out.2");
     if (!b.err.empty()) return fail(LDM_ERR_UNSUPPORTED, "%s", b.err.c_str());
     if (train) {
@@ -2285,6 +2313,21 @@
     p.lse = (const float*)rp(bs, a.lse); p.delta = (float*)rp(bs, a.delta); p.dqkv = (decltype(p.dqkv))rp(bs, a.dqkv);
     p.B = a.B; p.N = a.N; p.C = a.C; p.d = a.d; p.heads = a.heads; p.scale = a.scale;
     return p;
+}
+
+static hipError_t launch_conv_thin(ThinParams q, bool split, hipStream_t s) {
+    q.td = (q.D + THIN_TD - 1) / THIN_TD; q.th = (q.H + THIN_TH - 1) / THIN_TH; q.tw = (q.W + THIN_TW - 1) / THIN_TW;
+    static bool attr_tab[32] = {}; bool& attr_set = attr_flag(attr_tab);
+    if (!attr_set) {
+        hipError_t e = hipFuncSetAttribute(reinterpret_cast<const void*>(&conv3_thin_kernel<false>), hipFuncAttributeMaxDynamicSharedMemorySize, THIN_LDS);
+        if (e == hipSuccess) e = hipFuncSetAttribute(reinterpret_cast<const void*>(&conv3_thin_kernel<true>), hipFuncAttributeMaxDynamicSharedMemorySize, THIN_LDS);
+        if (e != hipSuccess) return e;
+        attr_set = true;
+    }
+    const unsigned blocks = (unsigned)((long)q.N * q.td * q.th * q.tw);
+    if (split) hipLaunchKernelGGL(conv3_thin_kernel<true>, dim3(blocks, (unsigned)(q.Cin / THIN_CK)), dim3(256), THIN_LDS, s, q);
+    else hipLaunchKernelGGL(conv3_thin_kernel<false>, dim3(blocks), dim3(256), THIN_LDS, s, q);
+    return hipSuccess;
 }
 
 struct PlanTrace { bool on = false; std::string path; PlanTrace() { const char* e = getenv("LDM_PLAN_TRACE"); if (e && *e) { on = true; path = e; } } };
@@ -2361,6 +2404,7 @@
     for (size_t oi = begin; oi < end; ++oi) {
         const Op& o = plan.ops[oi];
         if (trace_path) HIP_TRY(hipEventRecord(tev[oi - begin], s));
+        if (o.carried) continue;
         switch (o.kind) {
             case OP_PACK: case OP_PACK32: case OP_IM2COL: {
                 const LayoutRec& l = o.lay;
@@ -2383,10 +2427,8 @@
                 q.out = (float*)rp(bs, c.out); q.N = c.N; q.D = c.Din; q.H = c.Hin; q.W = c.Win; q.CoutPad = c.cout_pad; q.CoutReal = c.cout_real;
                 if (c.x3) { q.x3_c = c.ca / 2; q.Cin = 3 * q.x3_c; } else q.Cin = c.ca;
                 if (!q.w) return fail(LDM_ERR_NOT_LOADED, "the weight arena is empty");
-                q.td = (q.D + THIN_TD - 1) / THIN_TD; q.th = (q.H + THIN_TH - 1) / THIN_TH; q.tw = (q.W + THIN_TW - 1) / THIN_TW;
-                static bool attr_tab[32] = {}; bool& attr_set = attr_flag(attr_tab);
-                if (!attr_set) { HIP_TRY(hipFuncSetAttribute(reinterpret_cast<const void*>(&conv3_thin_kernel), hipFuncAttributeMaxDynamicSharedMemorySize, THIN_LDS)); attr_set = true; }
-                hipLaunchKernelGGL(conv3_thin_kernel, dim3((unsigned)((long)q.N * q.td * q.th * q.tw)), dim3(256), THIN_LDS, s, q);
+                if (o.cc.thin_split) q.out = (float*)rp(bs, c.partial);
+                HIP_TRY(launch_conv_thin(q, o.cc.thin_split != 0, s));
                 break; }
             case OP_CONV_BLOCK: {
                 const ConvRec& c = o.cv;
@@ -2485,7 +2527,21 @@
                 LightParams p{}; p.x = (const bf16_t*)rp(bs, c.xa); p.w = (const bf16_t*)rp(bs, c.w); p.bias = (const float*)rp(bs, c.bias);
                 p.residual = (const bf16_t*)rp(bs, c.residual); p.out = (bf16_t*)rp(bs, c.out); p.stats = (float*)rp(bs, c.stats);
                 p.M = c.M; p.K = c.ca + c.cb; p.CoutS = c.couts; p.xb = (const bf16_t*)rp(bs, c.xb); p.ca = c.ca;
-                if (o.cc.wg == 2) {
+                if (o.cc.wg == 3) {
+                    const LayoutRec& l = plan.ops[o.cc.i2c - 1].lay;
+                    int cx = rt[0], cc = rt[1];
+                    if (l.internal) { cx = l.c_real; cc = 0; }
+                    if (cx + cc != l.c_real) return fail(LDM_ERR_BAD_ARG, "x_channels + cond_channels = %d, model expects %d", cx + cc, l.c_real);
+                    WgI2cParams g{}; g.x = (const float*)rp(bs, l.a); g.cond = (const float*)rp(bs, l.b); g.cx = cx; g.cc = cc; g.D = l.D; g.H = l.H; g.W = l.W;
+                    int B = 0;
+                    if (o.cc.temb_ride) {
+                        const LinRec& t = plan.ops[o.cc.temb_ride - 1].lin;
+                        g.tab = (const float*)bs.p[BASE_TTAB]; g.st = (const SamplerState*)bs.p[BASE_SST]; g.n_steps = bs.sampler_steps;
+                        if (!g.tab || !g.st || g.n_steps < 1) return fail(LDM_ERR_BAD_ARG, "denoise-step plan without a sampler / time-embedding table");
+                        g.temb_out = (float*)rp(bs, t.y); g.rows = t.O; g.temb_blocks = 1; B = t.B;
+                    }
+                    HIP_TRY(launch_gemm_wg_i2c(p, c.cout_pad, o.cc.big, g, B, s));
+                } else if (o.cc.wg == 2) {
                     WgGnParams g{}; g.slabs = (const float*)rp(bs, c.gn_stats); g.gamma = (const float*)rp(bs, c.gamma); g.beta = (const float*)rp(bs, c.beta);
                     g.nrb = c.gn_nrb; g.groups = c.gn_groups; g.DHW = c.Dout * c.Hout * c.Wout; g.eps = c.gn_eps;
                     HIP_TRY(launch_gemm_wg(p, c.cout_pad, o.cc.big, s, &g));
@@ -2832,7 +2888,7 @@
     auto it = m->plans.find(key);
     if (it != m->plans.end()) { *out = it->second; return 0; }
     std::shared_ptr<Plan> p(new Plan());
-    if (m->type == 0) LDM_TRY(unet_build(m, B, D, H, W, p.get(), train, hp, tap_mode, strcmp(kind, "unet_tab") == 0));
+    if (m->type == 0) LDM_TRY(unet_build(m, B, D, H, W, p.get(), train, hp, tap_mode, !strncmp(kind, "unet_tab", 8), strstr(kind, "_step") != nullptr));
     else if (train) LDM_TRY(vae_build_train(m, B, D, H, W, p.get(), hp));
     else if (kind[0] == 'e') LDM_TRY(vae_build_encode(m, B, D, H, W, p.get(), hp, tap_mode));
     else LDM_TRY(vae_build_decode(m, B, D, H, W, p.get(), hp, tap_mode));
@@ -2879,18 +2935,20 @@
                                       (long long)sp->state_n, (long long)n);
     return 0;
 }
-static int sampler_launch(ldm_sampler* sp, const float* eps, float* x, float* x0_out, int64_t n, float* tbuf, int B, hipStream_t s) {
+static int sampler_launch(ldm_sampler* sp, const float* eps, float* x, float* x0_out, int64_t n, float* tbuf, int B, hipStream_t s,
+                          const EpsParts* parts = nullptr) {
     if (sp->kind == SAMPLER_PNDM) {
         if (x0_out) return fail(LDM_ERR_BAD_ARG, "PNDM has no x0_hat: x0_out must be NULL");
         LDM_TRY(pndm_check_state(sp, n));
         PndmParams p{}; p.coef = sp->coef; p.st = sp->st; p.n_steps = sp->n_steps; p.m = eps; p.x = x; p.state = sp->state; p.n = (long)n;
-        p.tbuf = tbuf; p.B = B;
+        p.tbuf = tbuf; p.B = B; if (parts) p.parts = *parts;
         const dim3 grid(grid_for((n + 3) / 4, 256, 1024));
         with_pred<false>(sp->pred, [&](auto P) { hipLaunchKernelGGL(pndm_sampler_step_kernel<P()>, grid, dim3(256), 0, s, p); });
         return 0;
     }
     SamplerParams p{}; p.coef = sp->coef; p.st = sp->st; p.n_steps = sp->n_steps; p.kind = sp->kind; p.clip = sp->clip;
     p.seed_lo = sp->seed_lo; p.seed_hi = sp->seed_hi; p.eps = eps; p.x = x; p.x0_out = x0_out; p.n = (long)n; p.tbuf = tbuf; p.B = B;
+    if (parts) p.parts = *parts;
     const dim3 grid(grid_for((n + 3) / 4, 256, 1024));
     with_pred(sp->pred, [&](auto P) { hipLaunchKernelGGL(sampler_step_kernel<P()>, grid, dim3(256), 0, s, p); });
     return 0;
@@ -2982,7 +3040,7 @@
     if (!x || !timesteps || !out) return fail(LDM_ERR_BAD_ARG, "null tensor argument");
     if (!cond) cond_channels = 0;
     const bool tab = sp != nullptr && temb_table_enabled() && m->tproj_rows % 4 == 0;
-    std::shared_ptr<Plan> p; LDM_TRY(get_plan(m, tab ? "unet_tab" : "unet", B, D, H, W, &p));
+    std::shared_ptr<Plan> p; LDM_TRY(get_plan(m, sp ? (tab ? "unet_tab_step" : "unet_step") : "unet", B, D, H, W, &p));
     LDM_TRY(check_ready(m, workspace, workspace_bytes, *p));
     if (tab) LDM_TRY(ensure_temb_table(m, sp, (hipStream_t)stream));
     Bases bs{}; bs.p[BASE_WS] = (char*)workspace; bs.p[BASE_W] = m->arena; bs.p[BASE_W32] = m->arena32;
@@ -2992,9 +3050,16 @@
     LDM_TRY(ensure_derived(m, (hipStream_t)stream));
     LaneCtx lanes;
     const int64_t n_out = (int64_t)B * m->ucfg.out_channels * D * H * W;
+    EpsParts parts{};
+    if (sp && p->eps_split_op >= 0) {
+        const Op& o = p->ops[(size_t)p->eps_split_op]; const ConvRec& c = o.cv;
+        parts.partial = (const float*)rp(bs, c.partial); parts.bias = (const float*)rp(bs, c.bias); parts.chunks = o.cc.thin_split;
+        parts.cout = c.cout_real; parts.dhw = c.Din * c.Hin * c.Win; parts.stride = (long)c.N * c.cout_real * parts.dhw;
+        if (!parts.bias) return fail(LDM_ERR_UNSUPPORTED, "split out conv without a bias");
+    }
     auto run_all = [&](hipStream_t s) -> int {
         LDM_TRY(run_plan(*p, bs, rt, s, 0, (size_t)-1, lanes));
-        if (sp) LDM_TRY(sampler_launch(sp, out, x_inout, nullptr, n_out, (float*)timesteps, B, s));
+        if (sp) LDM_TRY(sampler_launch(sp, out, x_inout, nullptr, n_out, (float*)timesteps, B, s, &parts));
         return 0;
     };
     if (!m->graph_mode || g_prof.on || g_plan_trace.on) return run_all((hipStream_t)stream);
@@ -3085,6 +3150,15 @@
     if (!sp || !eps || !x || !tbuf || n < 0 || B < 1) return fail(LDM_ERR_BAD_ARG, "bad argument");
     if (sp->kind == SAMPLER_PNDM && eps == x) return fail(LDM_ERR_BAD_ARG, "PNDM: the model output may not alias x");
     LDM_TRY(sampler_launch(sp, eps, x, x0_out, n, tbuf, B, (hipStream_t)stream));
+    HIP_TRY(hipGetLastError());
+    return 0;
+}
+int ldm_op_sampler_step_parts(ldm_sampler* sp, const float* partial, int chunks, int64_t stride, const float* bias, int cout, int dhw,
+                              float* x, float* x0_out, int64_t n, float* tbuf, int B, void* stream) {
+    if (!sp || !partial || !bias || !x || !tbuf || n < 0 || B < 1 || chunks < 1 || cout < 1 || dhw < 1 || stride < n || n % ((int64_t)cout * dhw))
+        return fail(LDM_ERR_BAD_ARG, "bad argument");
+    EpsParts parts{}; parts.partial = partial; parts.bias = bias; parts.stride = (long)stride; parts.chunks = chunks; parts.cout = cout; parts.dhw = dhw;
+    LDM_TRY(sampler_launch(sp, nullptr, x, x0_out, n, tbuf, B, (hipStream_t)stream, &parts));
     HIP_TRY(hipGetLastError());
     return 0;
 }
@@ -3735,7 +3809,7 @@
     if (!m || !kind) return fail(LDM_ERR_BAD_ARG, "null argument");
     std::shared_ptr<Plan> p; LDM_TRY(get_plan(m, kind, B, D, H, W, &p));
     int n = 0;
-    for (const Op& o : p->ops) if (o.kind != OP_TAP) ++n;
+    for (const Op& o : p->ops) if (o.kind != OP_TAP && !o.carried) ++n;
     return n;
 }
 
@@ -3775,6 +3849,18 @@
     BlockParams q{}; q.x = (const bf16_t*)x; q.w = (const bf16_t*)w; q.bias = bias; q.temb = temb; q.temb_stride = temb_stride;
     q.residual = (const bf16_t*)residual; q.out = (bf16_t*)out; q.stats = stats; q.N = N; q.D = D; q.H = H; q.W = W; q.Cin = cin;
     HIP_TRY(launch_conv_block(q, th, (hipStream_t)stream));
+    return 0;
+}
+
+int ldm_op_conv3d_thin(const void* x, int cin, const void* w, const float* bias, float* out, int cout_pad, int cout_real,
+                       int N, int D, int H, int W, int split, void* stream) {
+    if (!x || !w || !out || N < 1 || D < 1 || H < 1 || W < 1 || cin < 32 || cin % 32 || cout_real < 1 || cout_real > 4 || cout_pad < cout_real)
+        return fail(LDM_ERR_BAD_ARG, "bad argument");
+    if ((long)N * D * H * W * cin * 2 >= (1L << 32)) return fail(LDM_ERR_BAD_ARG, "the input tensor exceeds 4 GiB (split the batch)");
+    ThinParams q{}; q.x = (const bf16_t*)x; q.w = (const bf16_t*)w; q.bias = bias; q.out = out; q.N = N; q.D = D; q.H = H; q.W = W;
+    q.Cin = cin; q.CoutPad = cout_pad; q.CoutReal = cout_real;
+    HIP_TRY(launch_conv_thin(q, split != 0, (hipStream_t)stream));
+    HIP_TRY(hipGetLastError());
     return 0;
 }
 
@@ -4077,6 +4163,29 @@
     HIP_TRY(launch_gemm_light_x3(p, cout_pad, big < 0 ? gemm_light_x3_big(M, cout_pad) : big, (hipStream_t)stream));
     return 0;
 }
+int ldm_op_conv_in_im2col(const float* x, int cx, const float* cond, int cc, const void* w2, const float* bias, void* out, float* stats,
+                          int N, int D, int H, int W, int Kp, int cout_pad, int couts, int big, int fused, void* patch,
+                          const ldm_sampler* sp, const float* tab, float* temb_out, int rows, int B, void* stream) {
+    if (!cond) cc = 0;
+    const int64_t M = (int64_t)N * D * H * W;
+    if (!x || !w2 || !out || N < 1 || D < 1 || H < 1 || W < 1 || cx < 1 || cc < 0 || (Kp != 128 && Kp != 256) || 27 * (cx + cc) > Kp || cout_pad < 32 ||
+        cout_pad % 32 || couts < 32 || couts % 32 || couts > cout_pad || (big && cout_pad % 64) || M * (int64_t)std::max(Kp, cout_pad) * 2 >= (1L << 31) ||
+        (!fused && !patch) || (sp && (!fused || !tab || !temb_out || rows < 4 || rows % 4 || B < 1)))
+        return fail(LDM_ERR_BAD_ARG, "bad argument");
+    LightParams p{}; p.w = (const bf16_t*)w2; p.bias = bias; p.out = (bf16_t*)out; p.stats = stats; p.M = (int)M; p.K = Kp; p.ca = Kp; p.CoutS = couts;
+    if (!fused) {
+        hipLaunchKernelGGL(pack_im2col_kernel, dim3(grid_for(M * (Kp / 8), 256, 16384)), dim3(256), 0, (hipStream_t)stream, x, cx, cond, cc,
+                           (bf16_t*)patch, N, D, H, W, Kp);
+        p.x = (const bf16_t*)patch;
+        HIP_TRY(launch_gemm_wg(p, cout_pad, big, (hipStream_t)stream));
+        return 0;
+    }
+    WgI2cParams g{}; g.x = x; g.cond = cond; g.cx = cx; g.cc = cc; g.D = D; g.H = H; g.W = W;
+    if (sp) { g.tab = tab; g.st = sp->st; g.n_steps = sp->n_steps; g.temb_out = temb_out; g.rows = rows; g.temb_blocks = 1; }
+    HIP_TRY(launch_gemm_wg_i2c(p, cout_pad, big, g, sp ? B : 0, (hipStream_t)stream));
+    return 0;
+}
+
 int ldm_op_linear_bf16(const void* xa, int ca, const void* xb, int cb, const void* w, const float* bias, const void* residual, void* out,
                        float* stats, int64_t M, int cout_pad, int couts, int big, int kernel,
                        const float* gn_slabs, int gn_nrb, int gn_dhw, const float* gamma, const float* beta, int groups, float eps, int fold,
diff --git a/3d-latent-diffusion-model_amd/csrc/norm_elem.h b/3d-latent-diffusion-model_amd/csrc/norm_elem.h
--- a/3d-latent-diffusion-model_amd/csrc/norm_elem.h
+++ b/3d-latent-diffusion-model_amd/csrc/norm_elem.h
@@ -495,11 +495,48 @@
 }
 
 struct SamplerState { int k; unsigned done; };
+struct EpsParts { const float* partial; const float* bias; long stride; int chunks, cout, dhw; };
+__device__ __forceinline__ void eps_quad(const float* plain, const EpsParts& e, long q, long n, float out[4]) {
+#pragma clang fp reassociate(off) contract(off)
+    const long i0 = 4 * q;
+    if (e.chunks == 0) {
+#pragma unroll
+        for (int j = 0; j < 4; ++j) out[j] = i0 + j < n ? plain[i0 + j] : 0.f;
+        return;
+    }
+    const bool vec = i0 + 3 < n && (e.stride & 3) == 0 && (reinterpret_cast<uintptr_t>(e.partial) & 15) == 0;
+    auto load4 = [&](int k, float t[4]) {
+        const float* src = e.partial + (size_t)k * e.stride + i0;
+        if (vec) { const float4 v = *reinterpret_cast<const float4*>(src); t[0] = v.x; t[1] = v.y; t[2] = v.z; t[3] = v.w; }
+        else {
+#pragma unroll
+            for (int j = 0; j < 4; ++j) t[j] = i0 + j < n ? src[j] : 0.f;
+        }
+    };
+    load4(0, out);
+    for (int k0 = 1; k0 < e.chunks; k0 += 8) {
+        float t[8][4];
+#pragma unroll
+        for (int j = 0; j < 8; ++j) if (k0 + j < e.chunks) load4(k0 + j, t[j]);
+#pragma unroll
+        for (int j = 0; j < 8; ++j)
+            if (k0 + j < e.chunks) {
+#pragma unroll
+                for (int l = 0; l < 4; ++l) out[l] = __fadd_rn(out[l], t[j][l]);
+            }
+    }
+#pragma unroll
+    for (int j = 0; j < 4; ++j) {
+        const long i = i0 + j;
+        if (i < n) out[j] = __fadd_rn(out[j], e.bias[(i >> 32) == 0 ? ((unsigned)i / (unsigned)e.dhw) % (unsigned)e.cout : (i / e.dhw) % e.cout]);
+    }
+}
 struct SamplerParams {
     const float* coef; SamplerState* st; int n_steps; int kind;
     int clip; unsigned seed_lo, seed_hi;
     const float* eps; float* x; float* x0_out; long n;
     float* tbuf; int B;
+    EpsParts parts;
 };
 __device__ __forceinline__ void philox4x32_10(unsigned c0, unsigned c1, unsigned c2, unsigned c3, unsigned k0, unsigned k1, unsigned out[4]) {
 #pragma unroll
@@ -583,12 +620,13 @@
         float4 z = make_float4(0.f, 0.f, 0.f, 0.f);
         if (c.sigma != 0.f) z = sampler_normal4((unsigned long long)q, (unsigned)k, p.seed_lo, p.seed_hi);
         const float zz[4] = {z.x, z.y, z.z, z.w};
+        float ee[4]; eps_quad(p.eps, p.parts, q, p.n, ee);
 #pragma unroll
         for (int e = 0; e < 4; ++e) {
             const long i = 4 * q + e;
             if (i >= p.n) break;
             float x0;
-            p.x[i] = sampler_update<PRED>(c, p.kind, p.clip, p.x[i], p.eps[i], zz[e], &x0);
+            p.x[i] = sampler_update<PRED>(c, p.kind, p.clip, p.x[i], ee[e], zz[e], &x0);
             if (p.x0_out) p.x0_out[i] = x0;
         }
     }
@@ -657,6 +695,7 @@
     const float* coef; SamplerState* st; int n_steps;
     const float* m; float* x; float* state; long n;
     float* tbuf; int B;
+    EpsParts parts;
 };
 template <int PRED>
 __global__ __launch_bounds__(256) void pndm_sampler_step_kernel(const PndmParams p) {
@@ -666,11 +705,12 @@
         const PndmSlots s = pndm_slots(c, p.state, p.n);
         const long nq = (p.n + 3) / 4;
         for (long q = (long)blockIdx.x * blockDim.x + threadIdx.x; q < nq; q += (long)gridDim.x * blockDim.x) {
+            float mm[4]; eps_quad(p.m, p.parts, q, p.n, mm);
 #pragma unroll
             for (int e = 0; e < 4; ++e) {
                 const long i = 4 * q + e;
                 if (i >= p.n) break;
-                pndm_element<PRED>(c, s, p.x, p.m[i], i);
+                pndm_element<PRED>(c, s, p.x, mm[e], i);
             }
         }
     }
diff --git a/include/ldm3d.h b/include/ldm3d.h
--- a/include/ldm3d.h
+++ b/include/ldm3d.h
@@ -146,6 +146,8 @@
 int ldm_sampler_reset(ldm_sampler* sp, float* tbuf, int B, void* stream);
 int ldm_sampler_step(ldm_sampler* sp, const float* eps, float* x, float* x0_out, int64_t n, float* tbuf, int B, void* stream);
 int ldm_sampler_noise(const ldm_sampler* sp, int step, float* out, int64_t n, void* stream);
+int ldm_op_sampler_step_parts(ldm_sampler* sp, const float* partial, int chunks, int64_t stride, const float* bias, int cout, int dhw,
+                              float* x, float* x0_out, int64_t n, float* tbuf, int B, void* stream);
 int ldm_unet_denoise_step(ldm_model* m, ldm_sampler* sp, float* x, int x_channels, const float* cond, int cond_channels,
                           float* tbuf, float* eps_scratch, int B, int D, int H, int W,
                           void* workspace, size_t workspace_bytes, void* stream);
@@ -165,6 +167,8 @@
                   const float* temb, int temb_stride, const void* residual, void* out_bf16, float* out_f32,
                   int N, int Din, int Hin, int Win, int ksize, int stride, int pad, int ups,
                   int cout, int cout_pad, int wgn, int splitk, void* scratch, size_t scratch_bytes, void* stream);
+int ldm_op_conv3d_thin(const void* x, int cin, const void* w, const float* bias, float* out, int cout_pad, int cout_real,
+                       int N, int D, int H, int W, int split, void* stream);
 int ldm_op_conv3d_block_stats_rows(int D, int H, int W, int th);
 int ldm_op_conv3d_block128(const void* x, int cin, const void* w, const float* bias, const float* temb, int temb_stride, const void* residual,
                            void* out, float* stats, int N, int D, int H, int W, void* stream);
@@ -201,6 +205,9 @@
 int ldm_op_gemm_wgrad_f32(const float* dy, int cdy, const float* x, int K, float* dw, int cout, int64_t M, int ksplit, void* stream);
 int ldm_op_linear_f32x3(const float* xa, int ca, const float* xb, int cb, const float* w, const float* bias, const float* residual, float* out,
                         float* stats, int64_t M, int cout_pad, int couts, int big, void* stream);
+int ldm_op_conv_in_im2col(const float* x, int cx, const float* cond, int cc, const void* w2, const float* bias, void* out, float* stats,
+                          int N, int D, int H, int W, int Kp, int cout_pad, int couts, int big, int fused, void* patch,
+                          const ldm_sampler* sp, const float* tab, float* temb_out, int rows, int B, void* stream);
 int ldm_op_linear_bf16(const void* xa, int ca, const void* xb, int cb, const void* w, const float* bias, const void* residual, void* out,
                        float* stats, int64_t M, int cout_pad, int couts, int big, int kernel,
                        const float* gn_slabs, int gn_nrb, int gn_dhw, const float* gamma, const float* beta, int groups, float eps, int fold,
```

Result: no change. 534.1 (median of 6 runs) (+0.4%).
